# brown-ivl/manus

Hardware: AMD Instinct MI355X
Metric: train iters/sec (fwd+bwd) 300k Gaussians @1080p, 8 views; PSNR parity (higher is better)
Workload: dtype f32

## Files before the change

### include/manus_hip.h

```cpp
#ifndef MANUS_HIP_H
#define MANUS_HIP_H

#include <stddef.h>
#include <stdint.h>

#ifdef __cplusplus
extern "C" {
#endif

#define MGR_VERSION 100
#define MGR_CAM_FLOATS 40
#define MGR_TILE 16
#define MGR_MAX_BONES 32

enum {
    MGR_OK = 0,
    MGR_EINVAL = -1,
    MGR_ENOMEM = -2,
    MGR_EHIP = -3,
    MGR_EOVERFLOW = -4,
    MGR_ECUT = -6,
    MGR_ETIER = -7,
    MGR_ESTATE = -8
};

#define MGR_FWD_CHECK 1
#define MGR_FWD_NO_BLEND 2
#define MGR_FWD_BLEND_ONLY 4
#define MGR_FWD_DEPTH_CUT 8
#define MGR_FWD_SKIP_BOX_LARGE 16
#define MGR_FWD_SKIP_BOX_MID 32
#define MGR_FWD_SKIP_SORT_BEHIND 128
#define MGR_FWD_RANK_LARGE 256
#define MGR_FWD_IMAGE_KEPT 1024
#define MGR_FWD_REPAIR 2048
#define MGR_FWD_SPREAD 4096

#define MGR_BWD_CHECK 1
#define MGR_BWD_OUTPUTS_KEPT 512

#define MGR_OVF_PAIRS 1u
#define MGR_OVF_CUT 2u
#define MGR_OVF_TIER 4u
#define MGR_OVF_FLAGS_MASK 0xFFFF
#define MGR_OVF_REPAIRED_SHIFT 16

#define MGR_TIERS_BOX_LARGE 1
#define MGR_TIERS_BOX_MID 2
#define MGR_TIERS_WIDE_RECT 4
#define MGR_TIERS_NEAR_SMALL_SHIFT 8
#define MGR_TIERS_NEAR_LARGE_SHIFT 16
#define MGR_TIERS_NEAR_MASK 0xFF
#define MGR_TIERS_BEYOND_SMALL_SHIFT 24
#define MGR_TIERS_BEYOND_SMALL_MASK 0x7F

int mgr_version(void);
int mgr_build_variant(void);
int mgr_raster_repair_max_tiles(void);
const char* mgr_last_error(void);


size_t mgr_raster_workspace_bytes(int V, int N, int W, int H, int64_t pair_capacity);

int mgr_raster_forward(int V, int N, int W, int H, const float* cams, const float* bg,
                       const float* means3D, int64_t stride_means3D, const float* cov3D,
                       int64_t stride_cov3D, const float* colors, int64_t stride_colors,
                       const float* opacity, int64_t stride_opacity, float* out_color,
                       int32_t* radii, void* workspace, size_t workspace_bytes,
                       int64_t pair_capacity, int flags, void* stream);

int mgr_raster_backward(int V, int N, int W, int H, const float* cams, const float* bg,
                        const float* means3D, int64_t stride_means3D, const float* cov3D,
                        int64_t stride_cov3D, const float* colors, int64_t stride_colors,
                        const float* opacity, int64_t stride_opacity, const float* out_color,
                        const float* dL_dcolor, float* dL_dmeans3D, float* dL_dmeans2D, float* dL_dcolors,
                        float* dL_dopacity, float* dL_dcov3D, void* workspace,
                        size_t workspace_bytes, int64_t pair_capacity, int flags, void* stream);

int mgr_raster_blend_features(int V, int N, int C, int W, int H, const float* features, int64_t stride_features,
                              const float* bg_feat, int with_depth, float* out_feat, float* out_alpha,
                              const void* workspace, size_t workspace_bytes, int64_t pair_capacity, void* stream);

size_t mgr_raster_feat_backward_workspace_bytes(int V, int N, int C, int W, int H, int64_t pair_capacity);
int mgr_raster_blend_features_backward(int V, int N, int C, int W, int H, const float* cams, const float* means3D,
                                       int64_t stride_means3D, const float* cov3D, int64_t stride_cov3D, const float* features,
                                       int64_t stride_features, const float* bg_feat, int with_depth, const float* out_feat,
                                       const float* out_alpha, const float* dL_dout_feat, const float* dL_dalpha,
                                       float* dL_dmeans3D, float* dL_dmeans2D, float* dL_dopacity, float* dL_dcov3D,
                                       float* dL_dfeatures, const void* workspace, size_t workspace_bytes, int64_t pair_capacity,
                                       void* scratch, size_t scratch_bytes, int flags, void* stream);

int mgr_raster_forward_seq_sync(const void* workspace, uint32_t* seq, void* stream);

int mgr_views_forward(int V, int N, int B, int n_articulated, int sh_half, int W, int H, const float* cams, const float* bg,
                      const float* xyz, const float* log_scale, const float* rot,
                      const float* opacity_logit, const float* f_dc, const float* f_rest,
                      const float* skin_w, const float* transforms, float* out_color, int32_t* radii,
                      void* workspace, size_t workspace_bytes, int64_t pair_capacity, int flags,
                      void* stream);
int mgr_views_backward(int V, int N, int B, int n_articulated, int sh_half, int W, int H, const float* cams, const float* bg,
                       const float* xyz, const float* log_scale, const float* rot,
                       const float* opacity_logit, const float* f_dc, const float* f_rest,
                       const float* skin_w, const float* transforms, const int32_t* radii,
                       const float* out_color, const float* dL_dcolor, float grad2d_scale, float* d_xyz,
                       float* d_log_scale, float* d_rot, float* d_opacity_logit, float* d_f_dc,
                       float* d_f_rest, float* d_skin_w, float* stat_grad2d, float* stat_vis,
                       int32_t* stat_radii, void* workspace, size_t workspace_bytes,
                       int64_t pair_capacity, int flags, void* stream);



size_t mgr_views_pose_workspace_bytes(int V, int N, int B);
int mgr_views_backward_pose(int V, int N, int B, int n_articulated, int sh_half, int W, int H, const float* cams, const float* bg,
                            const float* xyz, const float* log_scale, const float* rot,
                            const float* opacity_logit, const float* f_dc, const float* f_rest,
                            const float* skin_w, const float* transforms, const int32_t* radii,
                            const float* out_color, const float* dL_dcolor, float grad2d_scale, float* d_xyz,
                            float* d_log_scale, float* d_rot, float* d_opacity_logit, float* d_f_dc,
                            float* d_f_rest, float* d_skin_w, float* stat_grad2d, float* stat_vis,
                            int32_t* stat_radii, void* workspace, size_t workspace_bytes,
                            int64_t pair_capacity, int flags, float* d_transforms, void* pose_workspace,
                            size_t pose_workspace_bytes, void* stream);

size_t mgr_views_maps_backward_workspace_bytes(int V, int N, int W, int H, int64_t pair_capacity);
int mgr_views_maps_backward(int V, int N, int B, int n_articulated, int W, int H, const float* cams, const float* xyz,
                            const float* log_scale, const float* rot, const float* opacity_logit, const float* skin_w,
                            const float* transforms, const float* out_alpha, const float* out_depth, const float* dL_dalpha,
                            const float* dL_ddepth, int accumulate, float* d_xyz, float* d_log_scale, float* d_rot,
                            float* d_opacity_logit, float* d_skin_w, const void* workspace, size_t workspace_bytes,
                            int64_t pair_capacity, void* scratch, size_t scratch_bytes, int flags, void* stream);

size_t mgr_views_maps_pose_workspace_bytes(int V, int N, int B);
int mgr_views_maps_backward_pose(int V, int N, int B, int n_articulated, int W, int H, const float* cams, const float* xyz,
                                 const float* log_scale, const float* rot, const float* opacity_logit, const float* skin_w,
                                 const float* transforms, const float* out_alpha, const float* out_depth, const float* dL_dalpha,
                                 const float* dL_ddepth, int accumulate, float* d_xyz, float* d_log_scale, float* d_rot,
                                 float* d_opacity_logit, float* d_skin_w, const void* workspace, size_t workspace_bytes,
                                 int64_t pair_capacity, void* scratch, size_t scratch_bytes, int flags, int accumulate_pose,
                                 float* d_transforms, void* pose_workspace, size_t pose_workspace_bytes, void* stream);

int mgr_views_active_list(void* workspace, int V, int N, int W, int H, int64_t pair_capacity, const uint32_t** list,
                          const uint32_t** count);

int mgr_views_backward_run_lists(int on);

int mgr_sh_to_half(int N, const float* f_rest, void* out_half, void* stream);

int mgr_raster_layout(int V, int N, int W, int H, int64_t pair_capacity, size_t* out, int n_out);
int mgr_raster_record_bytes(void);

int mgr_raster_set_cut_margin(float frac_entries, int min_entries, float depth_range_frac, float depth_rel, int interior_only);
int mgr_raster_set_cut_penalty(int forwards);
int mgr_raster_set_status_mirror(const void* workspace, void* host_words);
int mgr_raster_status_tiers_sync(const void* workspace, int64_t* num_pairs, int32_t* overflow, int32_t* tiers,
                                 void* stream);
int mgr_raster_status_sync(const void* workspace, int64_t* num_pairs, int32_t* overflow,
                           void* stream);

int mgr_raster_debug_binning_sync(const void* workspace, int V, int N, int W, int H,
                                  int64_t pair_capacity, int view, int32_t* tile_ranges_host,
                                  int32_t* point_list_host, int64_t max_pairs, void* stream);

int mgr_debug_pair_alpha(int n, const float* rec, const int32_t* px, const int32_t* py, float* alpha, int32_t* valid,
                         void* stream);


int mgr_skin_weights_fwd(int N, const float* xyz, const float* grid, int D, int H, int W, int B,
                         int grid_stride, const float* center3, const float* scale3, float* out_w,
                         void* stream);
int mgr_skin_weights_bwd(int N, const float* xyz, const float* grid, int D, int H, int W, int B,
                         int grid_stride, const float* center3, const float* scale3,
                         const float* dL_dw, float* dL_dxyz, int accumulate, void* stream);
int mgr_skin_weights_bwd_indexed(int N, const float* xyz, const float* grid, int D, int H, int W, int B,
                                 int grid_stride, const float* center3, const float* scale3, const float* dL_dw,
                                 float* dL_dxyz, const uint32_t* index, const uint32_t* index_count, int max_count,
                                 void* stream);

size_t mgr_skin_grid_bwd_workspace_bytes(int D, int H, int W, int max_count);
int mgr_skin_grid_bwd(int N, const float* xyz, const float* grid, int D, int H, int W, int B, int grid_stride,
                      const float* center3, const float* scale3, const float* dL_dw,
                      const uint32_t* index, const uint32_t* index_count, int max_count,
                      int32_t* out_voxel, float* out_grad, uint32_t* out_count, int capacity,
                      void* workspace, size_t workspace_bytes, void* stream);
int mgr_skin_grid_adam(const int32_t* voxel, const float* grad, const uint32_t* count, int capacity,
                       float* grid, int grid_stride, int B, float* exp_avg, float* exp_avg_sq,
                       double lr, double beta1, double beta2, double eps, int step, int clamp, float clamp_min,
                       void* stream);
int mgr_skin_rows_mask(int n, int B, const float* dL_dw, uint8_t* mask, void* stream);

int mgr_lbs_cov_fwd(int P, int N, int B, const float* xyz, const float* log_scale,
                    const float* rot, const float* skin_w, const float* transforms,
                    float* posed_xyz, float* posed_cov, float* tf, void* stream);
int mgr_lbs_cov_bwd(int P, int N, int B, const float* xyz, const float* log_scale,
                    const float* rot, const float* skin_w, const float* transforms,
                    const float* dL_dposed_xyz, const float* dL_dposed_cov, const float* dL_dtf,
                    float* dL_dxyz, float* dL_dlog_scale, float* dL_drot, float* dL_dw,
                    void* stream);

int mgr_sh_color_fwd(int V, int N, const float* sh, const float* xyz, int64_t stride_xyz,
                     const float* tf, int64_t stride_tf, const float* cams, float* colors,
                     void* stream);
int mgr_sh_color_bwd(int V, int N, const float* sh, const float* xyz, int64_t stride_xyz,
                     const float* tf, int64_t stride_tf, const float* cams,
                     const float* dL_dcolors, float* dL_dsh, float* dL_dxyz, float* dL_dtf,
                     void* stream);

int mgr_lbs_cov_fwd_rows(int P, int N, int B, const float* xyz, const float* log_scale,
                         const float* rot, const float* skin_w, const float* transforms,
                         float* posed_xyz, float* posed_cov, float* tf, int tf_row_floats, void* stream);
int mgr_lbs_cov_bwd_rows(int P, int N, int B, const float* xyz, const float* log_scale,
                         const float* rot, const float* skin_w, const float* transforms,
                         const float* dL_dposed_xyz, const float* dL_dposed_cov, const float* dL_dtf, int tf_row_floats,
                         float* dL_dxyz, float* dL_dlog_scale, float* dL_drot, float* dL_dw, void* stream);
size_t mgr_lbs_pose_workspace_bytes(int P, int N, int B);
int mgr_lbs_pose_bwd(int P, int N, int B, const float* xyz, const float* log_scale, const float* rot,
                     const float* skin_w, const float* transforms, const float* dL_dposed_xyz,
                     const float* dL_dposed_cov, const float* dL_dtf, int tf_row_floats, float* dL_dtransforms,
                     void* workspace, size_t workspace_bytes, void* stream);
int mgr_sh_color_fwd_rows(int V, int N, const float* sh, const float* xyz, int64_t stride_xyz,
                          const float* tf, int64_t stride_tf, int tf_row_floats, const float* cams, float* colors,
                          void* stream);
int mgr_sh_color_bwd_rows(int V, int N, const float* sh, const float* xyz, int64_t stride_xyz,
                          const float* tf, int64_t stride_tf, int tf_row_floats, const float* cams,
                          const float* dL_dcolors, float* dL_dsh, float* dL_dxyz, float* dL_dtf,
                          void* stream);

int mgr_pack_camera(float tanfovx, float tanfovy, const float* view16, const float* proj16, const float* campos3,
                    float* out40, void* stream);
int mgr_bone_transforms(int B, int background, const float* posed, const float* rest, float* out, void* stream);

int mgr_project_points(int N, const float* xyz, const float* K9, const float* E12, float* uv,
// ... 135 lines not shown
```

### manus_amd/_lib.py

```python
import ctypes
import os

import weakref

import torch

_HERE = os.path.dirname(os.path.abspath(__file__))
_VARIANT = os.environ.get("MANUS_HIP_VARIANT", "")
LIB_PATH = os.path.join(_HERE, "libmanus_hip%s.so" % ("_" + _VARIANT if _VARIANT else ""))
_LIB = None

MGR_CAM_FLOATS = 40
MGR_MAX_BONES = 32
MGR_FRAMES_MAX_VIEWS = 16

MGR_OK, MGR_EINVAL, MGR_ENOMEM, MGR_EHIP, MGR_EOVERFLOW, MGR_ECUT, MGR_ETIER, MGR_ESTATE = 0, -1, -2, -3, -4, -6, -7, -8
MGR_FWD_CHECK, MGR_FWD_NO_BLEND, MGR_FWD_BLEND_ONLY, MGR_FWD_DEPTH_CUT = 1, 2, 4, 8
MGR_FWD_SKIP_BOX_LARGE, MGR_FWD_SKIP_BOX_MID, MGR_FWD_SKIP_SORT_BEHIND, MGR_FWD_RANK_LARGE = 16, 32, 128, 256
MGR_FWD_IMAGE_KEPT, MGR_FWD_REPAIR, MGR_FWD_SPREAD = 1024, 2048, 4096
MGR_BWD_CHECK, MGR_BWD_OUTPUTS_KEPT = 1, 512
MGR_OVF_PAIRS, MGR_OVF_CUT, MGR_OVF_TIER, MGR_OVF_FLAGS_MASK, MGR_OVF_REPAIRED_SHIFT = 1, 2, 4, 0xFFFF, 16
MGR_TIERS_BOX_LARGE, MGR_TIERS_BOX_MID, MGR_TIERS_WIDE_RECT = 1, 2, 4
MGR_TIERS_NEAR_SMALL_SHIFT, MGR_TIERS_NEAR_LARGE_SHIFT, MGR_TIERS_NEAR_MASK = 8, 16, 0xFF
MGR_TIERS_BEYOND_SMALL_SHIFT, MGR_TIERS_BEYOND_SMALL_MASK = 24, 0x7F

c_int, c_i64, c_f32, c_vp, c_sz = ctypes.c_int, ctypes.c_int64, ctypes.c_float, ctypes.c_void_p, ctypes.c_size_t


class MgrFrameView(ctypes.Structure):
    _fields_ = [("offset", ctypes.c_int64), ("x0", ctypes.c_int32), ("y0", ctypes.c_int32), ("x1", ctypes.c_int32), ("y1", ctypes.c_int32),
                ("rx0", ctypes.c_int32), ("ry0", ctypes.c_int32), ("rx1", ctypes.c_int32), ("ry1", ctypes.c_int32),
                ("bg", ctypes.c_float * 3), ("slot", ctypes.c_int32)]


SIGNATURES = {
    "mgr_version": (c_int, []),
    "mgr_build_variant": (c_int, []),
    "mgr_raster_repair_max_tiles": (c_int, []),
    "mgr_last_error": (ctypes.c_char_p, []),
    "mgr_raster_workspace_bytes": (c_sz, [c_int, c_int, c_int, c_int, c_i64]),
    "mgr_raster_forward": (c_int, [c_int, c_int, c_int, c_int, c_vp, c_vp, c_vp, c_i64, c_vp, c_i64, c_vp,
                                   c_i64, c_vp, c_i64, c_vp, c_vp, c_vp, c_sz, c_i64, c_int, c_vp]),
    "mgr_raster_backward": (c_int, [c_int, c_int, c_int, c_int, c_vp, c_vp, c_vp, c_i64, c_vp, c_i64, c_vp,
                                    c_i64, c_vp, c_i64, c_vp, c_vp, c_vp, c_vp, c_vp, c_vp, c_vp, c_vp, c_sz,
                                    c_i64, c_int, c_vp]),
    "mgr_raster_blend_features": (c_int, [c_int, c_int, c_int, c_int, c_int, c_vp, c_i64, c_vp, c_int, c_vp, c_vp, c_vp, c_sz,
                                          c_i64, c_vp]),
    "mgr_raster_feat_backward_workspace_bytes": (c_sz, [c_int, c_int, c_int, c_int, c_int, c_i64]),
    "mgr_raster_blend_features_backward": (c_int, [c_int] * 5 + [c_vp, c_vp, c_i64, c_vp, c_i64, c_vp, c_i64, c_vp, c_int] + [c_vp] * 9
                                           + [c_vp, c_sz, c_i64, c_vp, c_sz, c_int, c_vp]),
    "mgr_raster_forward_seq_sync": (c_int, [c_vp, ctypes.POINTER(ctypes.c_uint32), c_vp]),
    "mgr_sh_to_half": (c_int, [c_int, c_vp, c_vp, c_vp]),
    "mgr_views_forward": (c_int, [c_int] * 7 + [c_vp] * 12 + [c_vp, c_sz, c_i64, c_int, c_vp]),
    "mgr_views_backward": (c_int, [c_int] * 7 + [c_vp] * 13 + [c_f32] + [c_vp] * 10 + [c_vp, c_sz, c_i64, c_int, c_vp]),
    "mgr_views_pose_workspace_bytes": (c_sz, [c_int, c_int, c_int]),
    "mgr_views_backward_pose": (c_int, [c_int] * 7 + [c_vp] * 13 + [c_f32] + [c_vp] * 10 + [c_vp, c_sz, c_i64, c_int, c_vp, c_vp, c_sz,
                                        c_vp]),
    "mgr_views_maps_backward_workspace_bytes": (c_sz, [c_int, c_int, c_int, c_int, c_i64]),
    "mgr_views_maps_backward": (c_int, [c_int] * 6 + [c_vp] * 11 + [c_int] + [c_vp] * 5 + [c_vp, c_sz, c_i64, c_vp, c_sz, c_int, c_vp]),
    "mgr_views_maps_pose_workspace_bytes": (c_sz, [c_int, c_int, c_int]),
    "mgr_views_maps_backward_pose": (c_int, [c_int] * 6 + [c_vp] * 11 + [c_int] + [c_vp] * 5 + [c_vp, c_sz, c_i64, c_vp, c_sz, c_int] +
                                     [c_int, c_vp, c_vp, c_sz, c_vp]),
    "mgr_raster_record_bytes": (c_int, []),
    "mgr_raster_layout": (c_int, [c_int, c_int, c_int, c_int, c_i64, ctypes.POINTER(c_sz), c_int]),
    "mgr_raster_status_sync": (c_int, [c_vp, ctypes.POINTER(c_i64), ctypes.POINTER(ctypes.c_int32), c_vp]),
    "mgr_raster_set_status_mirror": (c_int, [c_vp, c_vp]),
    "mgr_raster_set_cut_margin": (c_int, [c_f32, c_int, c_f32, c_f32, c_int]),
    "mgr_raster_set_cut_penalty": (c_int, [c_int]),
    "mgr_raster_status_tiers_sync": (c_int, [c_vp, ctypes.POINTER(c_i64), ctypes.POINTER(ctypes.c_int32),
                                             ctypes.POINTER(ctypes.c_int32), c_vp]),
    "mgr_debug_pair_alpha": (c_int, [c_int, c_vp, c_vp, c_vp, c_vp, c_vp, c_vp]),
    "mgr_raster_debug_binning_sync": (c_int, [c_vp, c_int, c_int, c_int, c_int, c_i64, c_int, c_vp, c_vp,
                                              c_i64, c_vp]),
    "mgr_skin_weights_fwd": (c_int, [c_int, c_vp, c_vp, c_int, c_int, c_int, c_int, c_int, c_vp, c_vp, c_vp,
                                     c_vp]),
    "mgr_skin_weights_bwd": (c_int, [c_int, c_vp, c_vp, c_int, c_int, c_int, c_int, c_int, c_vp, c_vp, c_vp,
                                     c_vp, c_int, c_vp]),
    "mgr_skin_weights_bwd_indexed": (c_int, [c_int, c_vp, c_vp, c_int, c_int, c_int, c_int, c_int, c_vp, c_vp, c_vp,
                                             c_vp, c_vp, c_vp, c_int, c_vp]),
    "mgr_skin_grid_bwd_workspace_bytes": (c_sz, [c_int, c_int, c_int, c_int]),
    "mgr_skin_grid_bwd": (c_int, [c_int, c_vp, c_vp, c_int, c_int, c_int, c_int, c_int, c_vp, c_vp, c_vp, c_vp, c_vp, c_int,
                                  c_vp, c_vp, c_vp, c_int, c_vp, c_sz, c_vp]),
    "mgr_skin_grid_adam": (c_int, [c_vp, c_vp, c_vp, c_int, c_vp, c_int, c_int, c_vp, c_vp, ctypes.c_double, ctypes.c_double, ctypes.c_double,
                                   ctypes.c_double, c_int, c_int, c_f32, c_vp]),
    "mgr_skin_rows_mask": (c_int, [c_int, c_int, c_vp, c_vp, c_vp]),
    "mgr_views_backward_run_lists": (c_int, [c_int]),
    "mgr_views_active_list": (c_int, [c_vp, c_int, c_int, c_int, c_int, c_i64, ctypes.POINTER(c_vp), ctypes.POINTER(c_vp)]),
    "mgr_lbs_cov_fwd": (c_int, [c_int, c_int, c_int, c_vp, c_vp, c_vp, c_vp, c_vp, c_vp, c_vp, c_vp, c_vp]),
    "mgr_lbs_cov_bwd": (c_int, [c_int, c_int, c_int, c_vp, c_vp, c_vp, c_vp, c_vp, c_vp, c_vp, c_vp, c_vp,
                                c_vp, c_vp, c_vp, c_vp]),
    "mgr_lbs_cov_fwd_rows": (c_int, [c_int, c_int, c_int, c_vp, c_vp, c_vp, c_vp, c_vp, c_vp, c_vp, c_vp, c_int, c_vp]),
    "mgr_lbs_cov_bwd_rows": (c_int, [c_int, c_int, c_int, c_vp, c_vp, c_vp, c_vp, c_vp, c_vp, c_vp, c_vp, c_int, c_vp,
                                     c_vp, c_vp, c_vp, c_vp]),
    "mgr_lbs_pose_workspace_bytes": (c_sz, [c_int, c_int, c_int]),
    "mgr_lbs_pose_bwd": (c_int, [c_int, c_int, c_int, c_vp, c_vp, c_vp, c_vp, c_vp, c_vp, c_vp, c_vp, c_int, c_vp, c_vp, c_sz, c_vp]),
    "mgr_sh_color_fwd_rows": (c_int, [c_int, c_int, c_vp, c_vp, c_i64, c_vp, c_i64, c_int, c_vp, c_vp, c_vp]),
    "mgr_sh_color_bwd_rows": (c_int, [c_int, c_int, c_vp, c_vp, c_i64, c_vp, c_i64, c_int, c_vp, c_vp, c_vp, c_vp, c_vp,
                                      c_vp]),
    "mgr_sh_color_fwd": (c_int, [c_int, c_int, c_vp, c_vp, c_i64, c_vp, c_i64, c_vp, c_vp, c_vp]),
    "mgr_sh_color_bwd": (c_int, [c_int, c_int, c_vp, c_vp, c_i64, c_vp, c_i64, c_vp, c_vp, c_vp, c_vp, c_vp,
                                 c_vp]),
    "mgr_pack_camera": (c_int, [c_f32, c_f32, c_vp, c_vp, c_vp, c_vp, c_vp]),
    "mgr_bone_transforms": (c_int, [c_int, c_int, c_vp, c_vp, c_vp, c_vp]),
    "mgr_project_points": (c_int, [c_int, c_vp, c_vp, c_vp, c_vp, c_vp]),
    "mgr_dilate_mask": (c_int, [c_int, c_int, c_int, c_vp, c_vp, c_vp, c_vp]),
    "mgr_points_outside_mask": (c_int, [c_int, c_vp, c_vp, c_vp, c_int, c_int, c_vp, c_int, c_vp, c_vp, c_vp]),
    "mgr_keypoint_far_mask": (c_int, [c_int, c_vp, c_int, c_vp, c_f32, c_vp, c_vp]),
    "mgr_knn3_workspace_bytes": (c_sz, [c_int]),
    "mgr_knn3_mean_dist2": (c_int, [c_int, c_vp, c_vp, c_vp, c_sz, c_vp]),
    "mgr_exchange_mask": (c_int, [c_int, c_vp, c_int, ctypes.POINTER(c_i64), ctypes.POINTER(c_int), c_i64, c_vp, c_vp, c_vp, c_vp]),
    "mgr_exchange_index_workspace_bytes": (c_sz, [c_int]),
    "mgr_exchange_index": (c_int, [c_int, c_vp, c_vp, c_vp, c_vp, c_sz, c_vp]),
    "mgr_exchange_pack": (c_int, [c_int, c_int, c_vp, c_vp, c_int, ctypes.POINTER(c_i64), ctypes.POINTER(c_int), c_i64, c_vp, c_vp]),
    "mgr_exchange_unpack": (c_int, [c_int, c_int, c_vp, c_vp, c_int, ctypes.POINTER(c_i64), ctypes.POINTER(c_int), c_i64, c_vp, c_vp,
                                    c_i64, c_vp]),
    "mgr_exchange_pack_rows": (c_int, [c_int, c_int, c_vp, c_vp, c_vp, c_int, ctypes.POINTER(c_i64), ctypes.POINTER(c_int), c_i64, c_vp, c_vp]),
    "mgr_exchange_unpack_rows": (c_int, [c_int, c_int, c_vp, c_vp, c_vp, c_int, ctypes.POINTER(c_i64), ctypes.POINTER(c_int), c_i64, c_vp, c_vp,
                                         c_i64, c_vp]),
    "mgr_l1_loss_grad": (c_int, [c_i64, c_vp, c_vp, c_f32, c_vp, c_vp, c_vp]),
    "mgr_image_loss_workspace_bytes": (c_sz, [c_int, c_int, c_int]),
    "mgr_image_loss": (c_int, [c_int, c_int, c_int, c_vp, c_vp, c_f32, c_f32, c_f32, c_f32, c_vp, c_vp, c_vp, c_sz, c_vp]),
    "mgr_image_loss_tiles": (c_int, [c_int, c_int, c_int, c_vp, c_vp, c_vp, c_vp, c_f32, c_f32, c_f32, c_f32, c_vp, c_vp, c_vp, c_sz,
                                     c_vp]),
    "mgr_image_loss_target_map_words": (c_sz, [c_int, c_int, c_int]),
    "mgr_image_loss_target_map": (c_int, [c_int, c_int, c_int, c_vp, c_vp, c_vp, c_vp]),
    "mgr_image_loss_tiles_list_mapped": (c_int, [c_int, c_int, c_int, c_vp, c_vp, c_vp, c_vp, c_sz, c_int, c_vp]),
    "mgr_views_forward_attach_loss_list": (c_int, [c_vp, c_int, c_int, c_int, c_vp, c_vp, c_sz]),
    "mgr_image_loss_tiles_list": (c_int, [c_int, c_int, c_int, c_vp, c_vp, c_vp, c_vp, c_sz, c_vp]),
    "mgr_image_loss_tiles_finish": (c_int, [c_int, c_int, c_int, c_vp, c_vp, c_f32, c_f32, c_f32, c_f32, c_vp, c_vp, c_vp, c_sz,
                                            c_vp]),
    "mgr_map_loss_workspace_bytes": (c_sz, [c_int, c_int, c_int]),
    "mgr_map_loss": (c_int, [c_int, c_int, c_int, c_vp, c_vp, c_vp, c_vp, c_f32, c_f32, c_f32, c_vp, c_vp, c_vp, c_vp, c_sz, c_vp]),
    "mgr_frames_decode": (c_int, [c_int, c_int, c_int, c_int, c_vp, c_i64, ctypes.POINTER(MgrFrameView), c_vp, c_vp, c_i64, c_vp]),
    "mgr_eval_workspace_bytes": (c_sz, [c_int, c_int, c_int]),
    "mgr_eval_views": (c_int, [c_int, c_int, c_int, c_vp, c_vp, c_vp, c_vp, c_vp, c_vp, c_vp, c_vp, c_sz, c_vp]),
    "mgr_eval_triptych": (c_int, [c_int, c_int, c_int, c_vp, c_vp, c_vp, c_vp, c_vp, c_vp]),
    "mgr_ceval_workspace_bytes": (c_sz, [c_int, c_int, c_int]),
    "mgr_ceval_masks": (c_int, [c_int, c_int, c_int, c_vp, c_int, c_vp, c_vp, c_vp, c_vp, c_vp, c_vp, c_vp]),
    "mgr_ceval_labels": (c_int, [c_int, c_int, c_int, c_vp, c_int, c_vp, c_vp, c_vp, c_sz, c_vp]),
    "mgr_ceval_fill": (c_int, [c_int, c_int, c_int, c_vp, c_vp, c_vp, c_sz, c_vp]),
    "mgr_ceval_counts": (c_int, [c_int, c_int, c_int, c_vp, c_vp, c_vp, c_vp, c_vp, c_sz, c_vp]),
    "mgr_ceval_collage": (c_int, [c_int, c_int, c_int, c_int, c_vp, c_vp, c_vp, c_vp, c_vp]),
    "mgr_adam_step": (c_int, [c_int, c_vp, c_vp, c_vp, c_vp, c_vp, c_vp, c_i64, ctypes.c_double, ctypes.c_double,
                               ctypes.c_double, c_vp]),
    "mgr_reset_opacity": (c_int, [c_int, c_vp, c_vp, c_vp, c_vp]),
    "mgr_add_densification_stats": (c_int, [c_int, c_vp, c_vp, c_vp, c_vp, c_vp, c_vp, c_vp]),
# ... 145 lines not shown
```

### manus_amd/csrc/instance_math.h

```cpp
#pragma once
#include <hip/hip_fp16.h>

#include "mgr_common.h"

#ifdef __HIPCC__

struct GaussCano {
    float x, y, z;
    float q[4], nrm, R[9], s[3];
};

__device__ __forceinline__ void quat_rot(const float q[4], float R[9]) {
#pragma clang fp contract(off)
    const float r = q[0], x = q[1], y = q[2], z = q[3];
    R[0] = 1.f - 2.f * (y * y + z * z); R[1] = 2.f * (x * y - r * z); R[2] = 2.f * (x * z + r * y);
    R[3] = 2.f * (x * y + r * z); R[4] = 1.f - 2.f * (x * x + z * z); R[5] = 2.f * (y * z - r * x);
    R[6] = 2.f * (x * z - r * y); R[7] = 2.f * (y * z + r * x); R[8] = 1.f - 2.f * (x * x + y * y);
}

typedef float mgr_f4u __attribute__((ext_vector_type(4), aligned(4)));
typedef float mgr_f3u __attribute__((ext_vector_type(3), aligned(4)));

__device__ __forceinline__ void cano_load(const float* __restrict__ xyz, const float* __restrict__ log_scale,
                                          const float* __restrict__ rot, int i, GaussCano& g) {
// ... 297 lines not shown
    const float b = M0[0] * S1[0] + M0[1] * S1[1] + M0[2] * S1[2];
    const float c = M1[0] * S1[0] + M1[1] * S1[1] + M1[2] * S1[2] + 0.3f;
    const float dA = acc[2], dB = acc[3], dC = acc[4];
    const float den = a * c - b * b;
    const float k2 = 1.0f / (den * den + 0.0000001f);
    float da = 0.f, db = 0.f, dc = 0.f;
#pragma unroll
    for (int j = 0; j < 6; ++j) dc6[j] = 0.f;
    if (k2 != 0.0f) {
        da = k2 * (-c * c * dA + 2.0f * b * c * dB + (den - a * c) * dC);
        dc = k2 * (-a * a * dC + 2.0f * a * b * dB + (den - a * c) * dA);
        db = k2 * 2.0f * (b * c * dA - (den + 2.0f * b * b) * dB + a * b * dC);
        dc6[0] = M0[0] * M0[0] * da + M0[0] * M1[0] * db + M1[0] * M1[0] * dc;
        dc6[3] = M0[1] * M0[1] * da + M0[1] * M1[1] * db + M1[1] * M1[1] * dc;
        dc6[5] = M0[2] * M0[2] * da + M0[2] * M1[2] * db + M1[2] * M1[2] * dc;
        dc6[1] = 2.0f * M0[0] * M0[1] * da + (M0[0] * M1[1] + M0[1] * M1[0]) * db + 2.0f * M1[0] * M1[1] * dc;
        dc6[2] = 2.0f * M0[0] * M0[2] * da + (M0[0] * M1[2] + M0[2] * M1[0]) * db + 2.0f * M1[0] * M1[2] * dc;
        dc6[4] = 2.0f * M0[2] * M0[1] * da + (M0[1] * M1[2] + M0[2] * M1[1]) * db + 2.0f * M1[1] * M1[2] * dc;
    }
    float dM0[3], dM1[3];
#pragma unroll
    for (int j = 0; j < 3; ++j) {
        dM0[j] = 2.0f * S0[j] * da + S1[j] * db;
        dM1[j] = 2.0f * S1[j] * dc + S0[j] * db;
    }
    const float dJ00 = vm[0] * dM0[0] + vm[4] * dM0[1] + vm[8] * dM0[2];
    const float dJ02 = vm[2] * dM0[0] + vm[6] * dM0[1] + vm[10] * dM0[2];
    const float dJ11 = vm[1] * dM1[0] + vm[5] * dM1[1] + vm[9] * dM1[2];
    const float dJ12 = vm[2] * dM1[0] + vm[6] * dM1[1] + vm[10] * dM1[2];
    const float tz = 1.0f / t[2], tz2 = tz * tz, tz3 = tz2 * tz;
    const float dtx = xm * -fx * tz2 * dJ02;
    const float dty = ym * -fy * tz2 * dJ12;
    const float dtz = -fx * tz2 * dJ00 - fy * tz2 * dJ11 + (2.0f * fx * t[0]) * tz3 * dJ02 +
                      (2.0f * fy * t[1]) * tz3 * dJ12;
    dm[0] = vm[0] * dtx + vm[1] * dty + vm[2] * dtz;
    dm[1] = vm[4] * dtx + vm[5] * dty + vm[6] * dtz;
    dm[2] = vm[8] * dtx + vm[9] * dty + vm[10] * dtz;
    const float* pm = cam.proj;
    const float hw = pm[3] * p[0] + pm[7] * p[1] + pm[11] * p[2] + pm[15];
    const float mw = 1.0f / (hw + 0.0000001f);
    const float mul1 = (pm[0] * p[0] + pm[4] * p[1] + pm[8] * p[2] + pm[12]) * mw * mw;
    const float mul2 = (pm[1] * p[0] + pm[5] * p[1] + pm[9] * p[2] + pm[13]) * mw * mw;
    const float gx2 = acc[0], gy2 = acc[1];
    dm[0] += (pm[0] * mw - pm[3] * mul1) * gx2 + (pm[1] * mw - pm[3] * mul2) * gy2;
    dm[1] += (pm[4] * mw - pm[7] * mul1) * gx2 + (pm[5] * mw - pm[7] * mul2) * gy2;
    dm[2] += (pm[8] * mw - pm[11] * mul1) * gx2 + (pm[9] * mw - pm[11] * mul2) * gy2;
}

typedef uint32_t mgr_u4u __attribute__((ext_vector_type(4), aligned(4)));

__device__ __forceinline__ void gather_pair_grads(uint32_t off, uint32_t cnt, const uint32_t* __restrict__ pair_tag,
                                                  const float4* __restrict__ pair_grad, uint32_t cap, uint32_t epoch,
                                                  float acc[9]) {
#pragma unroll
    for (int k = 0; k < 9; ++k) acc[k] = 0.f;
    if (off >= cap) return;
    cnt = min(cnt, cap - off);
    for (uint32_t base = 0; base < cnt; base += 64) {
        const uint32_t n = min(64u, cnt - base);
        unsigned long long hit = 0ull;
        for (uint32_t k = 0; k < n; k += 16) {
            const mgr_u4u* tp = (const mgr_u4u*)(pair_tag + off + base + k);
            const mgr_u4u t0 = tp[0], t1 = tp[1], t2 = tp[2], t3 = tp[3];
            const uint32_t tg[16] = {t0.x, t0.y, t0.z, t0.w, t1.x, t1.y, t1.z, t1.w,
                                     t2.x, t2.y, t2.z, t2.w, t3.x, t3.y, t3.z, t3.w};
            uint32_t m16 = 0;
#pragma unroll
            for (int j = 0; j < 16; ++j) m16 |= (tg[j] == epoch ? 1u : 0u) << j;
            hit |= (unsigned long long)m16 << k;
        }
        if (n < 64) hit &= (1ull << n) - 1ull;
        while (hit) {
            const int j = __builtin_ctzll(hit);
            hit &= hit - 1;
            const float4* r = pair_grad + (size_t)(off + base + (uint32_t)j) * 3;
            const float4 a = r[0], b = r[1], c = r[2];
            acc[0] += a.x; acc[1] += a.y; acc[2] += a.z; acc[3] += a.w;
            acc[4] += b.x; acc[5] += b.y; acc[6] += b.z; acc[7] += b.w;
            acc[8] += c.x;
        }
    }
}

#define MGR_POSE_REC 13
#define MGR_POSE_MAX_WG 1024

__device__ __forceinline__ int pose_segments(int NT, int nvb) {
    int s = 1;
    while (s < 8 && 2 * s * nvb <= NT) s *= 2;
    return s;
}

template <int NT>
__device__ __forceinline__ void pose_wg_lists(int tid, int NV, int pv, unsigned char* s_lst, int* s_cnt, int* s_wc) {
    static_assert(NT <= 256 && NT % 64 == 0, "lane ids are kept in a byte");
    constexpr int NW = NT / 64;
    const int lane = tid & 63, wv = tid >> 6;
    int rank = 0;
    for (int v = 0; v < NV; ++v) {
        const unsigned long long m = __ballot(pv == v);
        if (pv == v) rank = __popcll(m & ((1ull << lane) - 1ull));
        if (lane == 0) s_wc[v * NW + wv] = __popcll(m);
    }
    __syncthreads();
    if (pv >= 0) {
        int base = 0;
        for (int w = 0; w < wv; ++w) base += s_wc[pv * NW + w];
        s_lst[pv * NT + base + rank] = (unsigned char)tid;
    }
    if (tid < NV) {
        int c = 0;
        for (int w = 0; w < NW; ++w) c += s_wc[tid * NW + w];
        s_cnt[tid] = c;
    }
    __syncthreads();
}

template <int NT>
__device__ __forceinline__ void pose_wg_accumulate(int tid, int NV, int B, const float* s_rec, const unsigned char* s_lst,
                                                   const int* s_cnt, const float* __restrict__ skin_w, float pacc[12]) {
    const int nvb = NV * B, S = pose_segments(NT, nvb);
    const int seg = tid / nvb, o = tid - seg * nvb;
    if (seg >= S) return;
    const int v = o / B, b = o - v * B;
    const int cnt = s_cnt[v], per = (cnt + S - 1) / S;
    const int j1 = min(cnt, (seg + 1) * per);
    const unsigned char* lst = s_lst + v * NT;
#pragma unroll 4
    for (int j = seg * per; j < j1; ++j) {
        const float* r = s_rec + (int)lst[j] * MGR_POSE_REC;
        const float w = skin_w[(size_t)__float_as_int(r[12]) * B + b];
#pragma unroll
        for (int k = 0; k < 12; ++k) pacc[k] = __builtin_fmaf(w, r[k], pacc[k]);
    }
}

template <int NT>
__device__ __forceinline__ void pose_wg_store(int tid, int NV, int B, float* s_scratch, const float pacc[12],
                                              float* __restrict__ slot) {
    const int nvb = NV * B, S = pose_segments(NT, nvb);
    const int seg = tid / nvb, o = tid - seg * nvb;
    if (S > 1) {
        __syncthreads();
        if (seg > 0 && seg < S) {
#pragma unroll
            for (int k = 0; k < 12; ++k) s_scratch[(seg * nvb + o) * 12 + k] = pacc[k];
        }
        __syncthreads();
    }
    if (seg != 0) return;
    float a[12];
#pragma unroll
    for (int k = 0; k < 12; ++k) a[k] = pacc[k];
    for (int s = 1; s < S; ++s) {
#pragma unroll
        for (int k = 0; k < 12; ++k) a[k] += s_scratch[(s * nvb + o) * 12 + k];
    }
#pragma unroll
    for (int k = 0; k < 12; ++k) slot[o * 12 + k] = a[k];
}

#endif

int mgr_pose_fold(int v_first, int v_count, int NV, int B, const float* part, int n_slots, float* d_transforms,
                  hipStream_t stream);
int mgr_pose_fold_acc(int v_first, int v_count, int NV, int B, const float* part, int n_slots, int accumulate, float* d_transforms,
// ... 2 lines not shown
```

### manus_amd/csrc/mgr_common.h

```cpp
#pragma once
#include <hip/hip_runtime.h>
#include <stdint.h>
#include <stdio.h>
#include <string.h>

#include "../../include/manus_hip.h"

#define MGR_WAVE 64

extern thread_local char g_mgr_err[512];

static inline int mgr_fail(int code, const char* fmt, const char* a = "", const char* b = "") {
    snprintf(g_mgr_err, sizeof(g_mgr_err), fmt, a, b);
    return code;
}

#define MGR_HIP(call)                                                                      \
    do {                                                                                   \
        hipError_t e_ = (call);                                                            \
        if (e_ != hipSuccess) return mgr_fail(MGR_EHIP, "%s: %s", #call, hipGetErrorString(e_)); \
    } while (0)

#define MGR_LAUNCH_CHECK(name, stream, debug)                                              \
    do {                                                                                   \
// ... 30 lines not shown
#define MGR_REP_CAND 8192
#define MGR_REP_TARGET 3072
#define MGR_REP_VIEW_TILES 256
#define MGR_REP_MAX_TILES 65536
struct __attribute__((aligned(16))) MgrRepUnit {
    uint32_t vt, quad, nlist, start;
    uint32_t ck0, done_lo, done_hi, ntail;
    uint32_t ov_start, ov_ck0, p0, ck_first;
    uint32_t beyond;
    uint32_t pad[3];
};
struct __attribute__((aligned(16))) MgrRepTile {
    uint32_t tile, unit, zc, zw;
};
struct MgrRepView {
    uint32_t n, x0, y0, x1, y1, pad[3];
    MgrRepTile t[MGR_REP_VIEW_TILES];
};
struct MgrRep {
    MgrRepUnit* unit;
    float4* state;
    uint32_t* last;
    uint32_t* cnt;
    uint32_t* tile_rep;
    unsigned long long* cand;
    MgrRepView* view;
    uint32_t max_units, list_cap, ck_cap, list_base, ck_base;
};
struct MgrHeader {
    uint32_t total_pairs;
    uint32_t overflow;
    uint32_t epoch;
    uint32_t queue_len;
    uint32_t queue_head;
    uint32_t queue_head2;
    uint32_t n_items;
    uint32_t item_head;
    uint32_t queue_small;
    uint32_t queue_head3;
    uint32_t n_active;
    uint32_t queue_len_i;
    uint32_t acc_pairs, acc_flags;
    uint32_t tiers;
    uint32_t sort_big;
    uint32_t n_runs[4];
    uint32_t bwd_seq, rows_seq, rows_pending;
    uint32_t rows_owner[2];
    uint32_t fwd_seq, img_seq, img_owner[2], img_bg[3];
    uint32_t n_rep_units, rep_list_used, rep_ck_used;
    uint32_t rep_why;
    MgrRep rep;
    uint32_t sort_huge;
    uint32_t sort_large;
    uint32_t sort_near_large;
    uint32_t feat_seq, feat_dims[5], feat_flags;
    uint32_t spare[45 - 7 - sizeof(MgrRep) / 4];
    uint32_t queue_giant;
    uint32_t n_groups;
    uint32_t split_head, group_head;
    uint32_t pad2[56 - 8 - 68 + 64 - 4];
    uint32_t qctr[16 * 64];
    uint32_t qctr_f[16 * 64];
};
#define MGR_NCTR 16
#define MGR_HOLE 0xFFFFFFFEu
#define MGR_FEAT_CUT 1u
struct MgrFeatStamp {
    uint32_t dims[5], flags;
};
#define MGR_SKIP_BOX_LARGE 1
#define MGR_SKIP_BOX_MID 2
#define MGR_SKIP_SORT_BEHIND 4
#define MGR_SKIP_RANK_LARGE 8

#ifndef MGR_GREC_BYTES
#define MGR_GREC_BYTES 64
#endif
struct __attribute__((aligned(MGR_GREC_BYTES == 64 ? 64 : 16))) MgrGRec {
    float x, y, ca, cb;
    float cc, op, r, g;
    float b;
    int32_t slot_base;
    int32_t rect_w;
    int32_t pad;
#if MGR_GREC_BYTES == 64
    int32_t pad64[4];
#endif
};

#define MGR_CHUNK 64

static inline uint32_t mgr_rep_units(int64_t cap) { int64_t u = cap / 16384; return (uint32_t)(u < 64 ? 64 : (u > 1024 ? 1024 : u)); }
static inline uint32_t mgr_rep_list(int64_t cap) { int64_t n = cap / 8; return (uint32_t)(n < (1 << 16) ? (1 << 16) : (n > (2 << 20) ? (2 << 20) : n)); }
static inline uint32_t mgr_rep_ck(int64_t cap) { return mgr_rep_list(cap) / MGR_CHUNK + mgr_rep_units(cap); }

struct MgrLayout {
    size_t header, scan_part, scan_cls, scan_box, grec, depth, rect, alive, pair_off, tile_count, tile_start, tile_cursor, tile_done, tile_qdone,
        tile_zcut, tile_zused, tile_qend, tile_bgok, tile_queue, tile_qrec, chunk_start, items, ckpt, keys, keys2, groups, sorted_gid, final_T, n_contrib, pair_tag, pair_grad, inst_grad, inst_tag,
        db_count, db_cursor, db_start, db_nvis, db_bbox, db_keys, db_order, db_rec, bin_mat, tile_rep, rep_unit, rep_state, rep_last, rep_cnt, rep_cand, rep_view, tile_zwin, db_zrange, db_item, total;
};

#ifndef MGR_DB_BUCKETS
#define MGR_DB_BUCKETS 1024
#endif
#ifndef MGR_DB_ITEM
#define MGR_DB_ITEM 768
#endif
#define MGR_DB_RANK_MAX 2048
#define MGR_DB_RANK_LARGE 3072
#ifndef MGR_BIN_BLOCK
#define MGR_BIN_BLOCK 1024
#endif
static inline int mgr_bin_block(int V, int N) { return (long long)V * (long long)N >= 500000ll ? MGR_BIN_BLOCK : 256; }

static inline size_t mgr_align(size_t x) { return (x + 255) & ~(size_t)255; }

static inline MgrLayout mgr_layout(int V, int N, int W, int H, int64_t cap) {
    MgrLayout L;
    size_t VN = (size_t)V * (size_t)(N > 0 ? N : 1);
    size_t gx = (W + MGR_TILE - 1) / MGR_TILE, gy = (H + MGR_TILE - 1) / MGR_TILE;
    size_t VT = (size_t)V * gx * gy, VP = (size_t)V * W * H;
    size_t c = (size_t)(cap > 0 ? cap : 1);
    size_t o = 0;
    L.header = o;      o += mgr_align(sizeof(MgrHeader));
    const size_t scan_blocks = (size_t)V * ((gx * gy + 1023) / 1024);
    L.scan_part = o;   o += mgr_align((scan_blocks + 1) * 8);
    L.scan_cls = o;    o += mgr_align(scan_blocks * 34 * 4);
    L.scan_box = o;    o += mgr_align(scan_blocks * 16);
    L.grec = o;        o += mgr_align(VN * sizeof(MgrGRec));
    L.depth = o;       o += mgr_align(VN * 4);
    L.rect = o;        o += mgr_align(VN * 8);
    L.alive = o;       o += mgr_align(VN * 8);
    L.pair_off = o;    o += mgr_align(VN * 4);
    L.tile_count = o;  o += mgr_align(VT * 4);
    L.tile_start = o;  o += mgr_align((VT + 1) * 4);
    L.tile_cursor = o; o += mgr_align(VT * 4);
    L.tile_done = o;   o += mgr_align(VT * 4);
    L.tile_qdone = o;  o += mgr_align(VT * 16);
    L.tile_zcut = o;   o += mgr_align(VT * 4);
    L.tile_zused = o;  o += mgr_align(VT * 4);
    L.tile_qend = o;   o += mgr_align(VT * 4);
    L.tile_queue = o;  o += mgr_align(VT * 4);
    L.tile_qrec = o;   o += mgr_align(VT * 16);
    L.chunk_start = o; o += mgr_align((VT + 1) * 4);
    const size_t rep_u = mgr_rep_units(cap), rep_l = mgr_rep_list(cap), rep_c = mgr_rep_ck(cap);
    L.items = o;       o += mgr_align((c / MGR_CHUNK + VT + 1 + rep_c) * 32);
    L.ckpt = o;        o += mgr_align((c / MGR_CHUNK + 1 + rep_c) * 256 * 16);
    L.keys = o;        o += mgr_align(c * 8);
    L.keys2 = o;       o += mgr_align(c * 8);
    L.groups = o;      o += mgr_align((c / 4096 + 64) * 16);
    L.sorted_gid = o;  o += mgr_align((c + rep_l) * 4);
    L.final_T = o;     o += mgr_align(VP * 4);
    L.n_contrib = o;   o += mgr_align(VP * 4);
    L.pair_tag = o;    o += mgr_align(c * 4 + 64);
    L.pair_grad = o;   o += mgr_align(c * 48);
    L.inst_tag = o;    o += mgr_align(VN * 4);
    L.inst_grad = o;   o += mgr_align(VN * 128);
    {
        const size_t VB = (size_t)V * MGR_DB_BUCKETS, bb = (size_t)mgr_bin_block(V, N), nblk = ((size_t)(N > 0 ? N : 1) + bb - 1) / bb;
        L.db_count = o;  o += mgr_align(VB * 4);
        L.db_cursor = o; o += mgr_align(VB * 4);
        L.db_start = o;  o += mgr_align((VB + 1) * 4);
        L.db_nvis = o;   o += mgr_align((size_t)V * 4);
        L.db_bbox = o;   o += mgr_align((size_t)V * 8);
        L.db_keys = o;   o += mgr_align(VN * 8);
        L.db_order = o;  o += mgr_align(VN * 4);
        L.db_rec = o;    o += mgr_align(VN * 16);
        L.bin_mat = o;   o += mgr_align((size_t)V * nblk * gx * gy * 4);
    }
    L.tile_bgok = o; o += mgr_align((size_t)V * gx * gy);
    L.tile_rep = o;  o += mgr_align(VT * 4);
    L.rep_unit = o;  o += mgr_align(rep_u * sizeof(MgrRepUnit));
    L.rep_state = o; o += mgr_align(rep_u * 64 * 16);
    L.rep_last = o;  o += mgr_align(rep_u * 64 * 4);
    L.rep_cnt = o;   o += mgr_align(rep_u * 4);
    L.rep_cand = o;  o += mgr_align(rep_u * (size_t)MGR_REP_CAND * 8);
    L.rep_view = o;  o += mgr_align((size_t)V * sizeof(MgrRepView));
    L.tile_zwin = o; o += mgr_align(VT * 4);
    L.db_zrange = o; o += mgr_align((size_t)V * (((size_t)(N > 0 ? N : 1) + 511) / 512) * 2 * 4);
    L.db_item = o;   o += mgr_align((size_t)V * (((size_t)(N > 0 ? N : 1) + MGR_DB_ITEM - 1) / MGR_DB_ITEM + 1) * 2 * 4);
    L.total = o;
    return L;
}

#ifdef __HIPCC__

struct MgrCam {
    float tanfovx, tanfovy;
    float view[16], proj[16];
    float campos[3];
};

__device__ __forceinline__ void mgr_load_cam(const float* __restrict__ cams, int v, MgrCam& c) {
    const float* p = cams + (size_t)v * MGR_CAM_FLOATS;
    c.tanfovx = p[0];
    c.tanfovy = p[1];
#pragma unroll
    for (int i = 0; i < 16; ++i) {
        c.view[i] = p[2 + i];
        c.proj[i] = p[18 + i];
    }
    c.campos[0] = p[34];
    c.campos[1] = p[35];
    c.campos[2] = p[36];
}

template <int CTRL, int ROW_MASK = 0xf, int BANK_MASK = 0xf>
__device__ __forceinline__ float mgr_dpp(float v) {
    return __builtin_bit_cast(
        float, __builtin_amdgcn_update_dpp(0, __builtin_bit_cast(int, v), CTRL, ROW_MASK, BANK_MASK, false));
}

template <int CTRL, int ROW_MASK = 0xf>
__device__ __forceinline__ uint32_t mgr_dpp_u(uint32_t v) {
    return (uint32_t)__builtin_amdgcn_update_dpp(0, (int)v, CTRL, ROW_MASK, 0xf, false);
}
__device__ __forceinline__ uint32_t mgr_wave_incl_scan_u32(uint32_t v) {
    v += mgr_dpp_u<0x111>(v);
    v += mgr_dpp_u<0x112>(v);
    v += mgr_dpp_u<0x114>(v);
    v += mgr_dpp_u<0x118>(v);
    v += mgr_dpp_u<0x142, 0xa>(v);
    v += mgr_dpp_u<0x143, 0xc>(v);
    return v;
}

__device__ __forceinline__ uint32_t mgr_wave_max_u32(uint32_t v) {
    v = max(v, mgr_dpp_u<0xb1>(v));
    v = max(v, mgr_dpp_u<0x4e>(v));
    v = max(v, mgr_dpp_u<0x141>(v));
    v = max(v, mgr_dpp_u<0x140>(v));
    const uint32_t a = (uint32_t)__builtin_amdgcn_readlane((int)v, 0), b = (uint32_t)__builtin_amdgcn_readlane((int)v, 16),
                   c = (uint32_t)__builtin_amdgcn_readlane((int)v, 32), d = (uint32_t)__builtin_amdgcn_readlane((int)v, 48);
    return max(max(a, b), max(c, d));
}

__device__ __forceinline__ float mgr_wave_sum63(float v) {
    v += mgr_dpp<0xb1>(v);
    v += mgr_dpp<0x4e>(v);
    v += mgr_dpp<0x114>(v);
    v += mgr_dpp<0x118>(v);
    v += mgr_dpp<0x142, 0xa>(v);
    v += mgr_dpp<0x143, 0xc>(v);
    return v;
}

#define MGR_DPP9(ctrl)                                                                              \
    asm volatile("s_nop 1\n"                                                                        \
                 "v_add_f32_dpp %0, %0, %0 " ctrl "\n v_add_f32_dpp %1, %1, %1 " ctrl "\n"          \
                 "v_add_f32_dpp %2, %2, %2 " ctrl "\n v_add_f32_dpp %3, %3, %3 " ctrl "\n"          \
                 "v_add_f32_dpp %4, %4, %4 " ctrl "\n v_add_f32_dpp %5, %5, %5 " ctrl "\n"          \
                 "v_add_f32_dpp %6, %6, %6 " ctrl "\n v_add_f32_dpp %7, %7, %7 " ctrl "\n"          \
                 "v_add_f32_dpp %8, %8, %8 " ctrl "\n"                                              \
                 : "+v"(a0), "+v"(a1), "+v"(a2), "+v"(a3), "+v"(a4), "+v"(a5), "+v"(a6), "+v"(a7), "+v"(a8))

__device__ __forceinline__ void mgr_wave_sum63_x9(float& a0, float& a1, float& a2, float& a3, float& a4,
                                                  float& a5, float& a6, float& a7, float& a8) {
    MGR_DPP9("quad_perm:[1,0,3,2] row_mask:0xf bank_mask:0xf");
    MGR_DPP9("quad_perm:[2,3,0,1] row_mask:0xf bank_mask:0xf");
    MGR_DPP9("row_shr:4 row_mask:0xf bank_mask:0xf");
    MGR_DPP9("row_shr:8 row_mask:0xf bank_mask:0xf");
    MGR_DPP9("row_bcast:15 row_mask:0xa bank_mask:0xf");
    MGR_DPP9("row_bcast:31 row_mask:0xc bank_mask:0xf");
// ... 241 lines not shown
```

### manus_amd/csrc/raster_bwd.hip

```cpp
#include <atomic>

#include "instance_math.h"

#ifdef MGR_STATS
__device__ unsigned long long g_stats[16];
extern "C" int mgr_debug_stats(unsigned long long* dst) {
    return (int)hipMemcpyFromSymbol(dst, HIP_SYMBOL(g_stats), sizeof(unsigned long long) * 16);
}
__device__ unsigned long long g_bhist[3][65];
extern "C" int mgr_debug_bhist(unsigned long long* dst) {
    return (int)hipMemcpyFromSymbol(dst, HIP_SYMBOL(g_bhist), sizeof(unsigned long long) * 3 * 65);
}
#define BH(r, c, v) do { const int c_ = (c); const unsigned long long v_ = (unsigned long long)(v); if (lane == 0) atomicAdd(&g_bhist[r][c_], v_); } while (0)
#define MGR_STAT(i, v) do { const unsigned long long v_ = (unsigned long long)(v); if (lane == 0) atomicAdd(&g_stats[i], v_); } while (0)
#else
#define MGR_STAT(i, v)
#endif

#ifdef BWD_PROF
__device__ unsigned long long g_bprof[8];
extern "C" int mgr_debug_bprof(unsigned long long* dst) {
    return (int)hipMemcpyFromSymbol(dst, HIP_SYMBOL(g_bprof), sizeof(unsigned long long) * 8);
}
#define BP(k) { const long long now_ = wall_clock64(); acc_[k] += now_ - tp_; tp_ = now_; }
#else
#define BP(k)
#endif

__device__ __forceinline__ uint32_t mgr_any64(unsigned long long m) {
    uint32_t r;
    asm("s_cmp_lg_u64 %1, 0\n\ts_cselect_b32 %0, 1, 0" : "=s"(r) : "s"(m) : "scc");
    return r;
}

#define BWD_BATCH MGR_CHUNK
#ifndef BWD_KO
#define BWD_KO 0
#endif
int mgr_bwd_variant_bits(void) {
    int bits = 0;
    if (BWD_KO != 0) bits |= 1;
#if defined(MGR_STATS) || defined(BWD_PROF)
    bits |= 2;
#endif
#ifdef BWD_WLAST_REDUCE
    bits |= 4;
#endif
#if defined(MGR_GATHER_PRELOAD)
    if (MGR_GATHER_PRELOAD != 1) bits |= 4;
#endif
    return bits;
}
#define MGR_LDS_VOLATILE_F32 volatile const __attribute__((address_space(3))) float*
#define BWD_ROW 288
#define BWD_PLANE_W 64
#define BWD_PLANE_B 128
#ifndef BWD_WAVES
#define BWD_WAVES 4
#endif

__global__ __launch_bounds__(256) __attribute__((amdgpu_waves_per_eu(BWD_WAVES, BWD_WAVES))) void k_blend_bwd(
    int N, int W, int H, int gx, int gy, const uint32_t* __restrict__ sorted_gid, const MgrGRec* __restrict__ grec,
    const uint32_t* __restrict__ n_contrib, const float4* __restrict__ ckpt, const uint4* __restrict__ items,
    MgrHeader* hdr, const float* __restrict__ out_color, const float* __restrict__ dL_dpix,
    uint32_t* __restrict__ pair_tag, float4* __restrict__ pair_grad, uint32_t* __restrict__ inst_tag, uint32_t cap,
    uint32_t epoch) {
    __shared__ __align__(16) float s_pair[4][32][MGR_PAIR_FLOATS];
    __shared__ __align__(16) float s_xch[4][4 * BWD_ROW];
    __shared__ float s_acc[4][BWD_BATCH][9];
    __shared__ uint32_t s_flag[4][BWD_BATCH];

    const int tid = threadIdx.x, wave = tid >> 6, lane = tid & 63;
    const int T = gx * gy;
    const uint32_t n_items = hdr->n_items;
    if (blockIdx.x == 0 && tid < 4) (tid == 3 ? hdr->n_active : hdr->n_runs[tid]) = 0;
    if (blockIdx.x == 0 && tid == 4) hdr->bwd_seq += 1u;
    const size_t P = (size_t)W * H;
    const unsigned long long lt = (1ull << lane) - 1ull;
    float* const slab = &s_pair[wave][0][0];
    float* const xch = &s_xch[wave][0];
    float* const acc = &s_acc[wave][0][0];
    uint32_t* const flag = &s_flag[wave][0];
    const int e2 = lane >> 3, pc = lane & 7;
#ifdef BWD_PROF
    long long acc_[6] = {0, 0, 0, 0, 0, 0}, tp_ = wall_clock64(), nit_ = 0;
#endif

    MgrQueue queue;
    queue.init(hdr->qctr, n_items, (int)blockIdx.x);
    uint32_t item = queue.resolve(queue.issue(lane), lane);
    while (item != 0xFFFFFFFFu) {
        const uint32_t next_raw = queue.issue(lane);
        const uint4 recA = items[2 * (size_t)item], recB = items[2 * (size_t)item + 1];
        const uint32_t vt = recA.x, chunk = recA.y;
        const uint32_t mxq[4] = {recB.x, recB.y, recB.z, recB.w};
        const int v = (int)(vt / (uint32_t)T), t = (int)(vt % (uint32_t)T);
        const int bx = t % gx, by = t / gx;
        const uint32_t first = chunk * BWD_BATCH;
        const uint32_t tmax = max(max(mxq[0], mxq[1]), max(mxq[2], mxq[3]));
        const int cnt = (int)min((uint32_t)BWD_BATCH, tmax - first);
        const MgrGRec* const gv = grec + (size_t)v * N;
#ifdef BWD_PROF
        ++nit_;
#endif
        BP(0);
#if BWD_KO & 1024
        const uint32_t gid = sorted_gid[recA.z] + 0u * (uint32_t)lane;
#else
        const uint32_t gid = sorted_gid[recA.z + (uint32_t)min(lane, cnt - 1)];
#endif
        float4 ra, rb, rcz;
        {
            const MgrGRec* r = gv + gid;
            ra = *(const float4*)r;
            rb = *((const float4*)r + 1);
            rcz = *((const float4*)r + 2);
        }
#pragma unroll
        for (int k = 0; k < 9; ++k) acc[k * 64 + lane] = 0.f;
        flag[lane] = 0u;
        const int32_t slot = __float_as_int(rcz.y) + by * __float_as_int(rcz.z) + bx;
        const float qmax_e = mgr_qmax(rb.y);
        BP(1);

        uint32_t qmask = (mxq[0] > first ? 1u : 0u) | (mxq[1] > first ? 2u : 0u) | (mxq[2] > first ? 4u : 0u) | (mxq[3] > first ? 8u : 0u);
        struct PxState {
            uint32_t nc;
            float t0, t1, t2, o0, o1, o2;
            float4 ck;
        };
        auto load_px = [&](int quad, PxState& q) {
            const int px = bx * 16 + (quad & 1) * 8 + (lane & 7);
            const int py = by * 16 + (quad >> 1) * 8 + (lane >> 3);
            const size_t pixc = (size_t)min(py, H - 1) * W + min(px, W - 1);
#if BWD_KO & 512
            q.nc = tmax; q.t0 = 0.001f * (float)pixc; q.t1 = 0.5f; q.t2 = 0.25f; q.o0 = 0.3f; q.o1 = 0.2f; q.o2 = 0.1f;
            q.ck = make_float4(0.1f, 0.1f, 0.1f, 0.5f);
#else
            q.nc = n_contrib[(size_t)v * P + pixc];
            const float* gp = dL_dpix + (size_t)v * 3 * P + pixc;
            const float* op = out_color + (size_t)v * 3 * P + pixc;
            q.t0 = gp[0]; q.t1 = gp[P]; q.t2 = gp[2 * P];
            q.o0 = op[0]; q.o1 = op[P]; q.o2 = op[2 * P];
            q.ck = ckpt[(size_t)recA.w * 256 + ((quad << 6) | lane)];
#endif
        };
        PxState pxn;
        load_px(qmask ? __builtin_ctz(qmask) : 0, pxn);
#pragma unroll 1
// ... 156 lines not shown
                    const float xe = pbs[0 + h], ye = pbs[2 + h];
                    const uint32_t pos = __float_as_uint(*(MGR_LDS_VOLATILE_F32)(pbs + 18 + h));
                    const float dxc = xe - fx_col, dy0 = ye - qy0;
                    const float* src = xch + (e2 >> 1) * BWD_ROW + h * BWD_PLANE_B + 4 * pc;
#if !(BWD_KO & 128)
                    const bool on2 = (tmask >> e2) & 1u;
                    float* const accp = acc + (on2 ? (int)((pos - 1u - first) & 63u) : 0) * 9;
                    const float old_t = *(MGR_LDS_VOLATILE_F32)(accp + pc), old_9 = *(MGR_LDS_VOLATILE_F32)(accp + 8);
#endif
                    mgr_v2f DY = {dy0, dy0 - 1.0f};
                    mgr_v2f B0 = {0.f, 0.f}, B1 = {0.f, 0.f}, B2 = {0.f, 0.f}, Cr = {0.f, 0.f}, Cg = {0.f, 0.f}, Cb = {0.f, 0.f};
#pragma unroll
                    for (int j = 0; j < 2; ++j) {
                        const float4 v4 = *(const float4*)(src + 32 * j), w4 = *(const float4*)(src + BWD_PLANE_W + 32 * j);
#pragma unroll
                        for (int q = 0; q < 2; ++q) {
                            const int k = 2 * j + q;
                            const mgr_v2f vv = q ? mgr_v2f{v4.z, v4.w} : mgr_v2f{v4.x, v4.y};
                            const mgr_v2f ww = q ? mgr_v2f{w4.z, w4.w} : mgr_v2f{w4.x, w4.y};
                            const mgr_v2f t1 = vv * DY;
                            B0 += vv;
                            B1 += t1;
                            B2 += t1 * DY;
                            Cr += ww * gr0[k];
                            Cg += ww * gr1[k];
                            Cb += ww * gr2[k];
                            DY -= 2.0f;
                        }
                    }
                    const float A0 = B0.x + B0.y, A1 = B1.x + B1.y, A2 = B2.x + B2.y;
                    const float sr = Cr.x + Cr.y, sgn = Cg.x + Cg.y, sb = Cb.x + Cb.y;
                    const float Sx = dxc * A0;
                    const float x8[8] = {Sx, A1, Sx * dxc, dxc * A1, A2, A0, sr, sgn};
                    const float tot = grp8_reduce_scatter(x8, pc);
                    const float b9 = grp_sum<8>(sb);
                    if ((tmask >> e2) & 1u) {
                        const int ja = (int)(pos - 1u - first);
#if BWD_KO & 8
                        acc[ja * 9 + pc] = tot;
                        if (pc == 0) {
                            acc[ja * 9 + 8] = b9;
                            flag[ja] = 1u;
                        }
#elif BWD_KO & 128
                        __hip_atomic_fetch_add(acc + ja * 9 + pc, tot, __ATOMIC_RELAXED, __HIP_MEMORY_SCOPE_WAVEFRONT);
                        if (pc == 0) {
                            __hip_atomic_fetch_add(acc + ja * 9 + 8, b9, __ATOMIC_RELAXED, __HIP_MEMORY_SCOPE_WAVEFRONT);
                            flag[ja] = 1u;
                        }
#else
                        accp[pc] = old_t + tot;
                        if (pc == 0) {
                            accp[8] = old_9 + b9;
                            flag[ja] = 1u;
                        }
#endif
                    }
                }
                __builtin_amdgcn_wave_barrier();
            }
#ifdef MGR_STATS
            MGR_STAT(10, (max(max(nblk_[0], nblk_[1]), max(nblk_[2], nblk_[3])) + 1u) >> 1);
            MGR_STAT(11, (nblk_[0] + nblk_[1] + nblk_[2] + nblk_[3] + 7u) >> 3);
#endif
            BP(3);
        }
        __builtin_amdgcn_wave_barrier();
        if (lane < cnt && flag[lane] != 0u && slot >= 0 && (uint32_t)slot < cap) {
            float r[9];
#pragma unroll
            for (int c = 0; c < 9; ++c) r[c] = acc[lane * 9 + c];
#pragma unroll
            for (int c = 0; c < 5; ++c) r[c] *= rb.y;
            const float cA = ra.z, cB = ra.w, cC = rb.x;
            const float mx = (-0.5f * (float)W) * (cA * r[0] + cB * r[1]);
            const float my = (-0.5f * (float)H) * (cC * r[1] + cB * r[0]);
#if BWD_KO & 256
            if (mx + my + r[2] + r[3] + r[4] + r[5] + r[6] + r[7] + r[8] == 12345.678f) pair_tag[slot] = epoch;
#else
            float4* o = pair_grad + (size_t)slot * 3;
            o[0] = make_float4(mx, my, -0.5f * r[2], -0.5f * r[3]);
            o[1] = make_float4(-0.5f * r[4], r[5], r[6], r[7]);
            o[2] = make_float4(r[8], 0.f, 0.f, 0.f);
            pair_tag[slot] = epoch;
            inst_tag[(size_t)v * N + gid] = epoch;
#endif
        }
        __builtin_amdgcn_wave_barrier();
        BP(5);
        item = queue.resolve(next_raw, lane);
    }
#ifdef BWD_PROF
    if (lane == 0) {
        for (int k = 0; k < 6; ++k) atomicAdd(&g_bprof[k], (unsigned long long)acc_[k]);
        atomicAdd(&g_bprof[6], (unsigned long long)nit_);
        atomicAdd(&g_bprof[7], 1ull);
    }
#endif
}

__global__ __launch_bounds__(256) void k_preprocess_bwd(
    int N, int W, int H, const float* __restrict__ cams, const float* __restrict__ means3D,
    int64_t s_means, const float* __restrict__ cov3D, int64_t s_cov,
    const int32_t* __restrict__ radii_ws, const ushort4* __restrict__ rect,
    const uint32_t* __restrict__ pair_off, const uint32_t* __restrict__ pair_tag,
    const float4* __restrict__ pair_grad, float* __restrict__ dL_dmeans3D,
    float* __restrict__ dL_dmeans2D, float* __restrict__ dL_dcolors,
    float* __restrict__ dL_dopacity, float* __restrict__ dL_dcov3D, const uint32_t* __restrict__ inst_tag,
    uint32_t cap, uint32_t epoch, MgrHeader* hdr) {
    if (blockIdx.x == 0 && blockIdx.y == 0 && threadIdx.x < MGR_NCTR) hdr->qctr[threadIdx.x * 64] = 0u;
    const int v = blockIdx.y;
    const int i = blockIdx.x * 256 + threadIdx.x;
    if (i >= N) return;
    const size_t vi = (size_t)v * N + i;
    const ushort4 rc = rect[vi];
    const uint32_t cnt = (uint32_t)((rc.z - rc.x) * (rc.w - rc.y));
    float acc[9] = {0.f, 0.f, 0.f, 0.f, 0.f, 0.f, 0.f, 0.f, 0.f};
    float dm[3] = {0.f, 0.f, 0.f}, dc6[6] = {0.f, 0.f, 0.f, 0.f, 0.f, 0.f};
    if (cnt > 0 && inst_tag[vi] == epoch) {
        gather_pair_grads(pair_off[vi], cnt, pair_tag, pair_grad, cap, epoch, acc);
        MgrCam cam;
        mgr_load_cam(cams, v, cam);
        const float* mp = means3D + (size_t)v * s_means + (size_t)i * 3;
        const float p[3] = {mp[0], mp[1], mp[2]};
        const float* cp = cov3D + (size_t)v * s_cov + (size_t)i * 6;
        const float c6[6] = {cp[0], cp[1], cp[2], cp[3], cp[4], cp[5]};
        project_backward(cam, W, H, p, c6, acc, dm, dc6);
    }
    float* o3 = dL_dmeans3D + vi * 3;
    o3[0] = dm[0]; o3[1] = dm[1]; o3[2] = dm[2];
    float* o2 = dL_dmeans2D + vi * 3;
    o2[0] = acc[0]; o2[1] = acc[1]; o2[2] = 0.f;
    float* oc = dL_dcolors + vi * 3;
    oc[0] = acc[6]; oc[1] = acc[7]; oc[2] = acc[8];
    dL_dopacity[vi] = acc[5];
    float* ov = dL_dcov3D + vi * 6;
#pragma unroll
    for (int j = 0; j < 6; ++j) ov[j] = dc6[j];
}


typedef float mgr_f2u __attribute__((ext_vector_type(2), aligned(4)));
template <int G>
__device__ __forceinline__ void grp_store_span(const float t[8], int vl, bool ok, float* __restrict__ dst, int n, bool accumulate) {
    constexpr int PER = 8 / G;
    float mine[PER];
#pragma unroll
    for (int j = 0; j < PER; ++j) {
        mine[j] = t[j];
#pragma unroll
        for (int r = 1; r < G; ++r) mine[j] = vl == r ? t[r * PER + j] : mine[j];
    }
    const int e0 = vl * PER;
    if (!ok || e0 >= n) return;
    float* d = dst + e0;
    if (e0 + PER <= n) {
        if (PER == 2) {
            mgr_f2u v = {mine[0], mine[1]};
            if (accumulate) v += *(const mgr_f2u*)d;
            *(mgr_f2u*)d = v;
        } else if (PER == 4) {
            mgr_f4u v = {mine[0], mine[1], mine[2], mine[3]};
            if (accumulate) v += *(const mgr_f4u*)d;
            *(mgr_f4u*)d = v;
        } else {
#pragma unroll
            for (int h = 0; h < PER / 4; ++h) {
                mgr_f4u v = {mine[4 * h], mine[4 * h + 1], mine[4 * h + 2], mine[4 * h + 3]};
                if (accumulate) v += *(const mgr_f4u*)(d + 4 * h);
                *(mgr_f4u*)(d + 4 * h) = v;
            }
        }
    } else {
#pragma unroll
        for (int j = 0; j < PER; ++j)
            if (e0 + j < n) d[j] = accumulate ? d[j] + mine[j] : mine[j];
    }
}

template <int G>
__device__ __forceinline__ void grp_store8(const float x[8], int vl, bool ok, float* __restrict__ dst, int n,
                                           bool accumulate) {
    if (G == 8) {
        const float t = grp8_reduce_scatter(x, vl);
        if (ok && vl < n) dst[vl] = accumulate ? dst[vl] + t : t;
    } else {
        float t[8];
#pragma unroll
        for (int k = 0; k < 8; ++k) t[k] = grp_sum<G>(x[k]);
        grp_store_span<G>(t, vl, ok, dst, n, accumulate);
    }
}

#ifndef IB_THREADS
#define IB_THREADS 256
#endif
#ifndef MGR_IB_WAVES
#define MGR_IB_WAVES 2
#endif
#ifndef IG_ROUNDS
#define IG_ROUNDS 8
#endif
#define IB_TSTRIDE(B) ((B) * 16 + 4)

template <int G>
__global__ __launch_bounds__(256) void k_inst_gather(
    int v_first, int v_count, int N, int B, int n_art, const int32_t* __restrict__ radii, const ushort4* __restrict__ rect,
    const uint32_t* __restrict__ pair_off, const uint32_t* __restrict__ pair_tag,
    const float4* __restrict__ pair_grad, const uint32_t* __restrict__ inst_tag, uint32_t cap, uint32_t epoch,
    int accumulate, int rounds, float4* __restrict__ iacc,
    uint32_t* __restrict__ active_list, MgrHeader* hdr, float* __restrict__ d_xyz, float* __restrict__ d_ls,
    float* __restrict__ d_rot, float* __restrict__ d_op, float* __restrict__ d_fdc, float* __restrict__ d_frest,
    float* __restrict__ d_w, float* __restrict__ st_grad2d, float* __restrict__ st_vis,
    int32_t* __restrict__ st_radii, uint32_t* __restrict__ run_list) {
    constexpr int IPB = 256 / G;
    __shared__ uint32_t s_list[IPB * IG_ROUNDS];
    __shared__ uint32_t s_cnt, s_base;
    constexpr int RL = G == 8 ? IPB * IG_ROUNDS : 1;
    __shared__ uint32_t s_rl[3][RL];
    __shared__ uint32_t s_rc[3], s_rb[3];
    const bool runs = G == 8 && run_list != nullptr;
    const int tid = threadIdx.x, vl = tid & (G - 1), il = tid / G, lane = tid & 63;
    if (blockIdx.x == 0 && tid < MGR_NCTR && v_first == 0) hdr->qctr[tid * 64] = 0u;
    if (tid == 0) s_cnt = 0;
    if (tid < 3) s_rc[tid] = 0;
    __syncthreads();
    const bool acc_out = accumulate != 0;
#pragma unroll 1
    for (int rnd = 0; rnd < rounds; ++rnd) {
        const int i_raw = (blockIdx.x * rounds + rnd) * IPB + il;
        const int i = min(i_raw, N - 1);
        const bool ok = i_raw < N, mine = ok && vl < v_count;
        const int v = v_first + vl;
        float acc[9];
#pragma unroll
        for (int k = 0; k < 9; ++k) acc[k] = 0.f;
        int rad = 0;
        bool any = false;
        {
            const size_t vi = (size_t)min(v, v_first + v_count - 1) * N + i;
            const int rd = radii[vi];
            const uint32_t tg = inst_tag[vi];
            const ushort4 rc = rect[vi];
            const uint32_t po = pair_off[vi];
            rad = mine ? rd : 0;
            if (rad > 0 && tg == epoch) {
                gather_pair_grads(po, (uint32_t)((rc.z - rc.x) * (rc.w - rc.y)), pair_tag, pair_grad, cap, epoch, acc);
#pragma unroll
                for (int k = 0; k < 9; ++k) any = any || (acc[k] != 0.f);
            }
        }
        const bool grp_any = grp_sum<G>(any ? 1.0f : 0.0f) > 0.0f;
        const float vis = grp_sum<G>(rad > 0 ? 1.0f : 0.0f);
        int maxrad = rad;
        if (G >= 2) maxrad = max(maxrad, __builtin_amdgcn_update_dpp(0, maxrad, 0xb1, 0xf, 0xf, false));
        if (G >= 4) maxrad = max(maxrad, __builtin_amdgcn_update_dpp(0, maxrad, 0x4e, 0xf, 0xf, false));
        if (G >= 8) maxrad = max(maxrad, __builtin_amdgcn_update_dpp(0, maxrad, 0x141, 0xf, 0xf, false));
        if (runs) {
            const uint32_t m8 = (uint32_t)(__ballot(any) >> (lane & 56)) & 0xFFu;
            if (ok && vl == 0 && m8) {
                const int nv = __popc(m8), c = nv > 4 ? 0 : nv > 2 ? 1 : 2;
                s_rl[c][atomicAdd(&s_rc[c], 1u)] = (uint32_t)i | (m8 << 24);
            }
        }
        if (ok && (runs ? any : grp_any)) {
            float4* o = iacc + ((size_t)i * G + vl) * 3;
            o[0] = make_float4(acc[0], acc[1], acc[2], acc[3]);
            o[1] = make_float4(acc[4], acc[5], acc[6], acc[7]);
            o[2] = make_float4(acc[8], 0.f, 0.f, 0.f);
        }
        {
            const bool lead = ok && grp_any && vl == 0;
            const unsigned long long m = __ballot(lead);
            if (m) {
                const int first = __builtin_ctzll(m);
                uint32_t base = 0;
                if (lane == first) base = atomicAdd(&s_cnt, (uint32_t)__popcll(m));
                base = (uint32_t)__shfl((int)base, first, 64);
                if (lead) s_list[base + (uint32_t)__popcll(m & ((1ull << lane) - 1ull))] = (uint32_t)i;
            }
        }
        if (ok && vl == 0) {
            if (st_vis) st_vis[i] = acc_out ? st_vis[i] + vis : vis;
            if (st_radii) st_radii[i] = acc_out ? max(st_radii[i], maxrad) : maxrad;
        }
    }
    if (!acc_out) {
        const size_t i_lo = (size_t)blockIdx.x * rounds * IPB;
        const size_t i_hi = min((size_t)N, i_lo + (size_t)rounds * IPB);
        if (i_hi > i_lo) {
            const size_t n = i_hi - i_lo;
            for (size_t k = tid; k < n * 3; k += 256) { d_xyz[i_lo * 3 + k] = 0.f; d_ls[i_lo * 3 + k] = 0.f; d_fdc[i_lo * 3 + k] = 0.f; }
            for (size_t k = tid; k < n * 4; k += 256) d_rot[i_lo * 4 + k] = 0.f;
            for (size_t k = tid; k < n * 45; k += 256) d_frest[i_lo * 45 + k] = 0.f;
            if (d_w && i_lo < (size_t)n_art) {
                const size_t na = min(i_hi, (size_t)n_art) - i_lo;
                for (size_t k = tid; k < na * (size_t)B; k += 256) d_w[i_lo * B + k] = 0.f;
            }
            for (size_t k = tid; k < n; k += 256) {
                d_op[i_lo + k] = 0.f;
                if (st_grad2d) st_grad2d[i_lo + k] = 0.f;
            }
        }
    }
    __syncthreads();
    const uint32_t cnt = s_cnt;
    if (tid == 0 && cnt) s_base = atomicAdd(&hdr->n_active, cnt);
    __syncthreads();
    for (uint32_t k = tid; k < cnt; k += 256) active_list[s_base + k] = s_list[k];
    if (runs) {
        if (tid < 3) s_rb[tid] = s_rc[tid] ? atomicAdd(&hdr->n_runs[tid], s_rc[tid]) : 0u;
        __syncthreads();
#pragma unroll
        for (int c = 0; c < 3; ++c)
            for (uint32_t k = tid; k < s_rc[c]; k += 256) run_list[(size_t)c * N + s_rb[c] + k] = s_rl[c][k];
    }
}

template <int G>
__global__ __launch_bounds__(256) void k_inst_gather_runs(
    int v_first, int v_count, int N, int B, int n_art, const int32_t* __restrict__ radii, const ushort4* __restrict__ rect,
    const uint32_t* __restrict__ pair_off, const uint32_t* __restrict__ pair_tag,
    const float4* __restrict__ pair_grad, const uint32_t* __restrict__ inst_tag, uint32_t cap, uint32_t epoch,
    int accumulate, int rounds, float4* __restrict__ iacc,
    uint32_t* __restrict__ active_list, MgrHeader* hdr, float* __restrict__ d_xyz, float* __restrict__ d_ls,
    float* __restrict__ d_rot, float* __restrict__ d_op, float* __restrict__ d_fdc, float* __restrict__ d_frest,
    float* __restrict__ d_w, float* __restrict__ st_grad2d, float* __restrict__ st_vis,
    int32_t* __restrict__ st_radii, uint32_t* __restrict__ run_list, unsigned char* __restrict__ row_state, int kept) {
    constexpr int IPB = 256 / G, NG = 256;
    __shared__ uint32_t s_wi[NG * G], s_wo[NG * G], s_wc[NG * G];
    __shared__ uint32_t s_mask[NG];
    __shared__ uint32_t s_list[NG], s_rl[3][NG];
    __shared__ uint32_t s_nw, s_cnt, s_base, s_rc[3], s_rb[3];
    const int tid = threadIdx.x, vl = tid & (G - 1), il = tid / G, lane = tid & 63;
    if (blockIdx.x == 0 && tid < MGR_NCTR && v_first == 0) hdr->qctr[tid * 64] = 0u;
    if (tid == 0) { s_nw = 0; s_cnt = 0; }
    if (tid < 3) s_rc[tid] = 0;
    s_mask[tid] = 0u;
    __syncthreads();
    const bool acc_out = accumulate != 0;
    const int i_base = blockIdx.x * rounds * IPB;
    const unsigned long long owner = (unsigned long long)(uintptr_t)d_xyz;
    const bool kept_ok = kept && row_state && hdr->rows_seq != 0u && hdr->rows_seq + 1u == hdr->bwd_seq &&
                         hdr->rows_owner[0] == (uint32_t)owner && hdr->rows_owner[1] == (uint32_t)(owner >> 32);
    int rd_r[G];
    uint32_t tg_r[G], po_r[G];
    ushort4 rc_r[G];
#ifndef MGR_GATHER_PRELOAD
#define MGR_GATHER_PRELOAD 1
#endif
#if MGR_GATHER_PRELOAD
#pragma unroll
    for (int rnd = 0; rnd < G; ++rnd) {
        const int i = min(i_base + min(rnd, rounds - 1) * IPB + il, N - 1);
        const size_t vi = (size_t)min(v_first + vl, v_first + v_count - 1) * N + i;
        rd_r[rnd] = radii[vi];
        tg_r[rnd] = inst_tag[vi];
        rc_r[rnd] = rect[vi];
        po_r[rnd] = pair_off[vi];
    }
#pragma unroll
#else
#pragma unroll 1
#endif
    for (int rnd = 0; rnd < G; ++rnd) {
        if (rnd >= rounds) break;
        const int i_raw = i_base + rnd * IPB + il;
        const int i = min(i_raw, N - 1);
        const bool ok = i_raw < N, mine = ok && vl < v_count;
#if MGR_GATHER_PRELOAD
        const int rd = rd_r[rnd];
        const uint32_t tg = tg_r[rnd];
        const ushort4 rc = rc_r[rnd];
        const uint32_t po = po_r[rnd];
#else
        const size_t vi = (size_t)min(v_first + vl, v_first + v_count - 1) * N + i;
        const int rd = radii[vi];
        const uint32_t tg = inst_tag[vi];
        const ushort4 rc = rect[vi];
        const uint32_t po = pair_off[vi];
        (void)rd_r; (void)tg_r; (void)rc_r; (void)po_r;
#endif
        const int rad = mine ? rd : 0;
        const bool act = rad > 0 && tg == epoch;
        const float vis = grp_sum<G>(rad > 0 ? 1.0f : 0.0f);
        int maxrad = rad;
        if (G >= 2) maxrad = max(maxrad, __builtin_amdgcn_update_dpp(0, maxrad, 0xb1, 0xf, 0xf, false));
        if (G >= 4) maxrad = max(maxrad, __builtin_amdgcn_update_dpp(0, maxrad, 0x4e, 0xf, 0xf, false));
        if (G >= 8) maxrad = max(maxrad, __builtin_amdgcn_update_dpp(0, maxrad, 0x141, 0xf, 0xf, false));
        const unsigned long long m = __ballot(act);
        if (m) {
            const int first = __builtin_ctzll(m);
            uint32_t base = 0;
            if (lane == first) base = atomicAdd(&s_nw, (uint32_t)__popcll(m));
            base = (uint32_t)__shfl((int)base, first, 64);
            if (act) {
                const uint32_t pos = base + (uint32_t)__popcll(m & ((1ull << lane) - 1ull));
                s_wi[pos] = ((uint32_t)(rnd * IPB + il) << 3) | (uint32_t)vl;
                s_wo[pos] = po;
                s_wc[pos] = (uint32_t)((rc.z - rc.x) * (rc.w - rc.y));
            }
        }
        if (ok && vl == 0) {
            if (st_vis) st_vis[i] = acc_out ? st_vis[i] + vis : vis;
            if (st_radii) st_radii[i] = acc_out ? max(st_radii[i], maxrad) : maxrad;
        }
    }
    __syncthreads();
    const uint32_t n_work = s_nw;
    for (uint32_t k = (uint32_t)tid; k < n_work; k += 256u) {
        const uint32_t w = s_wi[k];
        float acc[9];
        gather_pair_grads(s_wo[k], s_wc[k], pair_tag, pair_grad, cap, epoch, acc);
        bool any = false;
#pragma unroll
        for (int q = 0; q < 9; ++q) any = any || (acc[q] != 0.f);
        {
            float4* o = iacc + ((size_t)(i_base + (int)(w >> 3)) * G + (w & 7u)) * 3;
            o[0] = make_float4(acc[0], acc[1], acc[2], acc[3]);
            o[1] = make_float4(acc[4], acc[5], acc[6], acc[7]);
            o[2] = make_float4(acc[8], 0.f, 0.f, 0.f);
        }
        if (any) atomicOr(&s_mask[w >> 3], 1u << (w & 7u));
    }
    if (!acc_out && !kept_ok) {
        const size_t i_lo = (size_t)i_base;
        const size_t i_hi = min((size_t)N, i_lo + (size_t)rounds * IPB);
        if (i_hi > i_lo) {
            const size_t n = i_hi - i_lo;
            for (size_t k = tid; k < n * 3; k += 256) { d_xyz[i_lo * 3 + k] = 0.f; d_ls[i_lo * 3 + k] = 0.f; d_fdc[i_lo * 3 + k] = 0.f; }
            for (size_t k = tid; k < n * 4; k += 256) d_rot[i_lo * 4 + k] = 0.f;
            for (size_t k = tid; k < n * 45; k += 256) d_frest[i_lo * 45 + k] = 0.f;
            if (d_w && i_lo < (size_t)n_art) {
                const size_t na = min(i_hi, (size_t)n_art) - i_lo;
                for (size_t k = tid; k < na * (size_t)B; k += 256) d_w[i_lo * B + k] = 0.f;
            }
            for (size_t k = tid; k < n; k += 256) {
                d_op[i_lo + k] = 0.f;
                if (st_grad2d) st_grad2d[i_lo + k] = 0.f;
            }
        }
    }
    __syncthreads();
    if (row_state && tid < rounds * IPB && i_base + tid < N) {
        const int i = i_base + tid;
        if (kept_ok && row_state[i] && s_mask[tid] == 0u) {
            for (int k = 0; k < 3; ++k) { d_xyz[3 * i + k] = 0.f; d_ls[3 * i + k] = 0.f; d_fdc[3 * i + k] = 0.f; }
            for (int k = 0; k < 4; ++k) d_rot[4 * i + k] = 0.f;
            for (int k = 0; k < 45; ++k) d_frest[(size_t)i * 45 + k] = 0.f;
            if (d_w && i < n_art)
                for (int k = 0; k < B; ++k) d_w[(size_t)i * B + k] = 0.f;
            d_op[i] = 0.f;
            if (st_grad2d) st_grad2d[i] = 0.f;
        }
        row_state[i] = s_mask[tid] != 0u ? 1 : 0;
    }
    if (blockIdx.x == 0 && tid == 0) hdr->rows_pending = row_state ? hdr->bwd_seq : 0u;
    {
        const uint32_t m8 = tid < rounds * IPB ? s_mask[tid] : 0u;
        if (m8) {
            const uint32_t i = (uint32_t)(i_base + tid);
            s_list[atomicAdd(&s_cnt, 1u)] = i;
            if (G >= 2) {
                const int nv = __popc(m8), c = nv > 4 ? 0 : nv > 2 ? 1 : 2;
                s_rl[c][atomicAdd(&s_rc[c], 1u)] = i | (m8 << 24);
            }
        }
    }
    __syncthreads();
    const uint32_t cnt = s_cnt;
    if (tid == 0 && cnt) s_base = atomicAdd(&hdr->n_active, cnt);
    if (G >= 2 && tid < 3) s_rb[tid] = s_rc[tid] ? atomicAdd(&hdr->n_runs[tid], s_rc[tid]) : 0u;
    __syncthreads();
    for (uint32_t k = tid; k < cnt; k += 256) active_list[s_base + k] = s_list[k];
    if (G >= 2) {
#pragma unroll
        for (int c = 0; c < 3; ++c)
            for (uint32_t k = tid; k < s_rc[c]; k += 256) run_list[(size_t)c * N + s_rb[c] + k] = s_rl[c][k];
    }
}

template <int G, int BMAX, bool MIXED, bool SH_HALF, bool RUNS, int NVV = 8, bool POSE = false>
__device__ __forceinline__ void inst_bwd_body(
    int blk, int n_active, const uint32_t* __restrict__ active_list,
    int v_first, int v_count, int N, int B, int n_art, int W, int H, const float* __restrict__ cams,
    const float* __restrict__ xyz, const float* __restrict__ log_scale, const float* __restrict__ rot,
    const float* __restrict__ op_logit, const float* __restrict__ f_dc, const float* __restrict__ f_rest,
    const float* __restrict__ skin_w, const float* __restrict__ transforms, const float4* __restrict__ iacc,
    float grad2d_scale, int accumulate,
    float* __restrict__ d_xyz, float* __restrict__ d_ls, float* __restrict__ d_rot, float* __restrict__ d_op,
    float* __restrict__ d_fdc, float* __restrict__ d_frest, float* __restrict__ d_w, float* __restrict__ st_grad2d,
    unsigned char* __restrict__ pose_valid = nullptr) {
    constexpr int IPB = IB_THREADS / G;
    constexpr int NV = RUNS ? NVV : G;
    extern __shared__ __align__(16) float s_view[];
    if (blk * IPB >= n_active) return;
// ... 193 lines not shown
        h->rows_seq = hdr->bwd_seq;
        h->rows_owner[0] = (uint32_t)owner;
        h->rows_owner[1] = (uint32_t)(owner >> 32);
    }
    const int b8 = (n8 + IB_THREADS / 8 - 1) / (IB_THREADS / 8), b4 = (n4 + IB_THREADS / 4 - 1) / (IB_THREADS / 4);
    if constexpr (NVV >= 8) {
        if (blk < b8) { inst_bwd_body<8, BMAX, MIXED, SH_HALF, true, NVV, POSE>(blk, n8, active_list, MGR_IB_ARGS, pose_valid); return; }
    }
    blk -= b8;
    if constexpr (NVV >= 4) {
        if (blk < b4) { inst_bwd_body<4, BMAX, MIXED, SH_HALF, true, NVV, POSE>(blk, n4, active_list + (size_t)N, MGR_IB_ARGS, pose_valid); return; }
    }
    blk -= b4;
    inst_bwd_body<2, BMAX, MIXED, SH_HALF, true, NVV, POSE>(blk, n2, active_list + 2 * (size_t)N, MGR_IB_ARGS, pose_valid);
}
template <int NVV, int BMAX, bool MIXED, bool SH_HALF>
__global__ __launch_bounds__(IB_THREADS) __attribute__((amdgpu_waves_per_eu(MGR_IB_WAVES, MGR_IB_WAVES))) void k_inst_bwd_runs(MGR_IB_PARAMS) {
    inst_bwd_runs<NVV, BMAX, MIXED, SH_HALF, false>(MGR_IB_ALL, nullptr);
}

template <int G, int BMAX, bool MIXED, bool SH_HALF>
__global__ __launch_bounds__(IB_THREADS) __attribute__((amdgpu_waves_per_eu(MGR_IB_WAVES, MGR_IB_WAVES))) void k_inst_bwd_pose(MGR_IB_PARAMS, unsigned char* __restrict__ pose_valid) {
    inst_bwd_body<G, BMAX, MIXED, SH_HALF, false, 8, true>((int)blockIdx.x, (int)hdr->n_active, active_list, MGR_IB_ARGS, pose_valid);
}
template <int NVV, int BMAX, bool MIXED, bool SH_HALF>
__global__ __launch_bounds__(IB_THREADS) __attribute__((amdgpu_waves_per_eu(MGR_IB_WAVES, MGR_IB_WAVES))) void k_inst_bwd_runs_pose(MGR_IB_PARAMS, unsigned char* __restrict__ pose_valid) {
    inst_bwd_runs<NVV, BMAX, MIXED, SH_HALF, true>(MGR_IB_ALL, pose_valid);
}

template <int NV>
__global__ __launch_bounds__(256) void k_pose_part_views(int n_art, int B, int n_chunks, const float4* __restrict__ iacc,
                                                         const unsigned char* __restrict__ valid,
                                                         const float* __restrict__ skin_w, float* __restrict__ part) {
    constexpr int IPB = 256 / NV;
    __shared__ float s_rec[256 * MGR_POSE_REC];
    __shared__ unsigned char s_lst[NV * 256];
    __shared__ int s_cnt[8], s_wc[8 * 4];
    const int tid = threadIdx.x, vl = tid & (NV - 1), il = tid / NV;
    float pacc[12];
#pragma unroll
    for (int k = 0; k < 12; ++k) pacc[k] = 0.f;
    for (int c = blockIdx.x; c < n_chunks; c += gridDim.x) {
        const int i = c * IPB + il;
        const bool on = i < n_art && valid[(size_t)i * NV + vl] != 0;
        if (on) {
            const float4* o = iacc + ((size_t)i * NV + vl) * 3;
            const float4 a = o[0], b = o[1], d = o[2];
            float* r = s_rec + tid * MGR_POSE_REC;
            r[0] = a.x; r[1] = a.y; r[2] = a.z; r[3] = a.w; r[4] = b.x; r[5] = b.y; r[6] = b.z; r[7] = b.w;
            r[8] = d.x; r[9] = d.y; r[10] = d.z; r[11] = d.w;
            r[12] = __int_as_float(i);
        }
        pose_wg_lists<256>(tid, NV, on ? vl : -1, s_lst, s_cnt, s_wc);
        pose_wg_accumulate<256>(tid, NV, B, s_rec, s_lst, s_cnt, skin_w, pacc);
        __syncthreads();
    }
    pose_wg_store<256>(tid, NV, B, s_rec, pacc, part + (size_t)blockIdx.x * NV * B * 12);
}

static std::atomic<int> g_inst_runs{[] { const char* e = getenv("MANUS_INST_RUNS"); return e ? atoi(e) : 1; }()};
extern "C" int mgr_views_backward_run_lists(int on) { return g_inst_runs.exchange(on); }

struct CanonGrads {
    int B, n_art, sh_half;
    const float *xyz, *log_scale, *rot, *op_logit, *f_dc, *f_rest, *skin_w, *transforms;
    const int32_t* radii;
    float grad2d_scale;
    float *d_xyz, *d_ls, *d_rot, *d_op, *d_fdc, *d_frest, *d_w, *st_grad2d, *st_vis;
    int32_t* st_radii;
    float *d_T, *pose_part;
};

static int pose_view_slots(int n_art, int Gv) {
    const int ipb = 256 / Gv, chunks = (n_art + ipb - 1) / ipb;
    return chunks < MGR_POSE_MAX_WG ? chunks : MGR_POSE_MAX_WG;
}
static size_t pose_part_bytes(int N, int B, int Gv) { return ((size_t)pose_view_slots(N, Gv) * Gv * B * 12 * sizeof(float) + 255) & ~(size_t)255; }
extern "C" size_t mgr_views_pose_workspace_bytes(int V, int N, int B) {
    if (V <= 0 || N <= 0 || B <= 0) return 0;
    const int Gv = V <= 1 ? 1 : V <= 2 ? 2 : V <= 4 ? 4 : 8;
    return pose_part_bytes(N, B, Gv) + (size_t)N * Gv;
}

static int raster_backward_impl(int V, int N, int W, int H, const float* cams, const float* bg,
                                   const float* means3D, int64_t s_means, const float* cov3D,
                                   int64_t s_cov, const float* colors, int64_t s_col,
                                   const float* opacity, int64_t s_op, const float* out_color,
                                   const float* dL_dcolor, float* dL_dmeans3D, float* dL_dmeans2D, float* dL_dcolors,
                                   float* dL_dopacity, float* dL_dcov3D, const CanonGrads* canon, void* workspace,
                                   size_t workspace_bytes, int64_t cap, int flags, void* stream_) {
    (void)colors; (void)s_col; (void)opacity; (void)s_op;
    hipStream_t stream = (hipStream_t)stream_;
    if (V <= 0 || N < 0 || W <= 0 || H <= 0 || cap < 0)
        return mgr_fail(MGR_EINVAL, "mgr_raster_backward: bad sizes");
    if (!cams || !bg || !dL_dcolor || !out_color || !workspace)
        return mgr_fail(MGR_EINVAL, "mgr_raster_backward: null pointer");
    if (N == 0) return MGR_OK;
    if (!canon && (!means3D || !cov3D || !dL_dmeans3D || !dL_dmeans2D || !dL_dcolors || !dL_dopacity || !dL_dcov3D))
        return mgr_fail(MGR_EINVAL, "mgr_raster_backward: null pointer");
    const int gx = (W + 15) / 16, gy = (H + 15) / 16;
    const MgrLayout L = mgr_layout(V, N, W, H, cap);
    if (workspace_bytes < L.total) return mgr_fail(MGR_ENOMEM, "mgr_raster_backward: workspace too small");
    char* ws = (char*)workspace;
    MgrHeader* hdr = (MgrHeader*)(ws + L.header);
    static std::atomic<uint32_t> g_epoch{0};
    uint32_t epoch = g_epoch.fetch_add(1) + 1;
    if (epoch == 0) epoch = g_epoch.fetch_add(1) + 1;

    { MGR_PROF("k_blend_bwd", stream); hipLaunchKernelGGL(k_blend_bwd, dim3(256 * BWD_WAVES), dim3(256), 0, stream, N, W, H, gx, gy,
                       (const uint32_t*)(ws + L.sorted_gid), (const MgrGRec*)(ws + L.grec), (const uint32_t*)(ws + L.n_contrib),
                       (const float4*)(ws + L.ckpt), (const uint4*)(ws + L.items), hdr, out_color,
                       dL_dcolor, (uint32_t*)(ws + L.pair_tag), (float4*)(ws + L.pair_grad),
                       (uint32_t*)(ws + L.inst_tag), (uint32_t)cap, epoch); }
    MGR_LAUNCH_CHECK("k_blend_bwd", stream, flags & MGR_BWD_CHECK);
    if (canon) {
        const int Gv = V <= 1 ? 1 : V <= 2 ? 2 : V <= 4 ? 4 : 8;
        const int ipb = 256 / Gv;
        const size_t lds = (size_t)Gv * (MGR_CAM_FLOATS + (canon->skin_w ? IB_TSTRIDE(canon->B) : 0)) * sizeof(float);
        float4* iacc = (float4*)(ws + L.inst_grad);
        uint32_t* alist = (uint32_t*)(ws + L.inst_grad + (size_t)N * Gv * 48);
        const int ipb2 = IB_THREADS / Gv;
        const bool mixed = canon->skin_w && canon->n_art < N;
        int rounds = (int)((long long)N / ((long long)ipb * 1024));
        rounds = rounds < 1 ? 1 : (rounds > IG_ROUNDS ? IG_ROUNDS : rounds);
        const dim3 grid((N + ipb2 - 1) / ipb2), grid_g((N + ipb * rounds - 1) / (ipb * rounds));
        for (int v0 = 0; v0 < V; v0 += Gv) {
            const int vc = V - v0 < Gv ? V - v0 : Gv;
            const int accm = v0 > 0 ? 1 : 0;
            if (v0 > 0) {
                MGR_HIP(hipMemsetAsync(&hdr->n_active, 0, 4, stream));
                MGR_HIP(hipMemsetAsync(&hdr->n_runs[0], 0, 12, stream));
            }
            const bool runs = g_inst_runs.load(std::memory_order_relaxed) != 0 && Gv >= 4 && canon->B <= 24 && N < (1 << 24);
            const int rounds_r = rounds < Gv ? rounds : Gv;
            const dim3 grid_gr((N + ipb * rounds_r - 1) / (ipb * rounds_r));
            uint32_t* rlist = alist + (size_t)N;
            unsigned char* row_state = V <= Gv ? (unsigned char*)(rlist + 3 * (size_t)N) : nullptr;
            const int kept = (flags & MGR_BWD_OUTPUTS_KEPT) && V <= Gv ? 1 : 0;
#define MGR_IG_LAUNCH(GG)                                                                                             \
    hipLaunchKernelGGL((k_inst_gather<GG>), grid_g, dim3(256), 0, stream, v0, vc, N, canon->B, canon->n_art, canon->radii, \
                       (const ushort4*)(ws + L.rect), (const uint32_t*)(ws + L.pair_off),                             \
                       (const uint32_t*)(ws + L.pair_tag), (const float4*)(ws + L.pair_grad),                        \
                       (const uint32_t*)(ws + L.inst_tag), (uint32_t)cap, epoch, accm, rounds, iacc, alist, hdr, canon->d_xyz, canon->d_ls, canon->d_rot, canon->d_op, canon->d_fdc,    \
                       canon->d_frest, canon->d_w, canon->st_grad2d, canon->st_vis, canon->st_radii, runs && GG == 8 ? rlist : (uint32_t*)nullptr)
#define MGR_IB_LAUNCH(GG, BB)                                                                                         \
    if (mixed && canon->sh_half) MGR_IB_LAUNCH2(GG, BB, true, true);                                                  \
    else if (mixed) MGR_IB_LAUNCH2(GG, BB, true, false);                                                              \
    else if (canon->sh_half) MGR_IB_LAUNCH2(GG, BB, false, true);                                                     \
    else MGR_IB_LAUNCH2(GG, BB, false, false)
#define MGR_IB_LAUNCH2(GG, BB, MX, HF)                                                                                \
    hipLaunchKernelGGL((k_inst_bwd<GG, BB, MX, HF>), grid, dim3(IB_THREADS), lds, stream, v0, vc, N, canon->B, canon->n_art, W, H, cams, canon->xyz, \
                       canon->log_scale, canon->rot, canon->op_logit, canon->f_dc, canon->f_rest, canon->skin_w,      \
                       canon->transforms, (const float4*)iacc, (const uint32_t*)alist, (const MgrHeader*)hdr,         \
                       canon->grad2d_scale, accm, canon->d_xyz, canon->d_ls, canon->d_rot, canon->d_op, canon->d_fdc, \
                       canon->d_frest, canon->d_w, canon->st_grad2d)
            {
                MGR_PROF("k_inst_gather", stream);
#define MGR_IGR_LAUNCH(GG)                                                                                            \
    hipLaunchKernelGGL((k_inst_gather_runs<GG>), grid_gr, dim3(256), 0, stream, v0, vc, N, canon->B, canon->n_art, canon->radii, \
                       (const ushort4*)(ws + L.rect), (const uint32_t*)(ws + L.pair_off),                             \
                       (const uint32_t*)(ws + L.pair_tag), (const float4*)(ws + L.pair_grad),                        \
                       (const uint32_t*)(ws + L.inst_tag), (uint32_t)cap, epoch, accm, rounds_r, iacc, alist, hdr, canon->d_xyz, canon->d_ls, canon->d_rot, canon->d_op, canon->d_fdc, \
                       canon->d_frest, canon->d_w, canon->st_grad2d, canon->st_vis, canon->st_radii, rlist, row_state, kept)
                const bool old_gather = g_inst_runs.load(std::memory_order_relaxed) == 2 && Gv == 8;
                if (runs && !old_gather) {
                    if (Gv == 8) MGR_IGR_LAUNCH(8);
                    else if (Gv == 4) MGR_IGR_LAUNCH(4);
                    else if (Gv == 2) MGR_IGR_LAUNCH(2);
                    else MGR_IGR_LAUNCH(1);
                }
#undef MGR_IGR_LAUNCH
                else if (Gv == 8) MGR_IG_LAUNCH(8);
                else if (Gv == 4) MGR_IG_LAUNCH(4);
                else if (Gv == 2) MGR_IG_LAUNCH(2);
                else MGR_IG_LAUNCH(1);
            }
            MgrProfScope prof_ib(canon->d_T ? "k_inst_bwd_pose" : "k_inst_bwd", stream);
#define MGR_IBR_LAUNCH(MX, HF)                                                                                        \
    if (Gv == 8) MGR_IBR_LAUNCH2(8, MX, HF); else if (Gv == 4) MGR_IBR_LAUNCH2(4, MX, HF); else MGR_IBR_LAUNCH2(2, MX, HF)
#define MGR_IBR_LAUNCH2(NN, MX, HF)                                                                                   \
    hipLaunchKernelGGL((k_inst_bwd_runs<NN, 24, MX, HF>), dim3(grid.x + 3), dim3(IB_THREADS), lds, stream, v0, vc, N, canon->B, canon->n_art, W, H, cams, canon->xyz, \
                       canon->log_scale, canon->rot, canon->op_logit, canon->f_dc, canon->f_rest, canon->skin_w,      \
                       canon->transforms, (const float4*)iacc, (const uint32_t*)rlist, (const MgrHeader*)hdr,         \
                       canon->grad2d_scale, accm, canon->d_xyz, canon->d_ls, canon->d_rot, canon->d_op, canon->d_fdc, \
                       canon->d_frest, canon->d_w, canon->st_grad2d)
            if (canon->d_T) {
                const int slots = pose_view_slots(canon->n_art, Gv);
                unsigned char* pvalid = (unsigned char*)canon->pose_part + pose_part_bytes(N, canon->B, Gv);
                MGR_HIP(hipMemsetAsync(pvalid, 0, (size_t)canon->n_art * Gv, stream));
#define MGR_IP_ARGS                                                                                                   \
    v0, vc, N, canon->B, canon->n_art, W, H, cams, canon->xyz, canon->log_scale, canon->rot, canon->op_logit, canon->f_dc,  \
        canon->f_rest, canon->skin_w, canon->transforms, (const float4*)iacc, (const uint32_t*)(runs && Gv >= 2 ? rlist : alist), \
        (const MgrHeader*)hdr, canon->grad2d_scale, accm, canon->d_xyz, canon->d_ls, canon->d_rot, canon->d_op,          \
        canon->d_fdc, canon->d_frest, canon->d_w, canon->st_grad2d, pvalid
#define MGR_IP_LAUNCH(KERNEL) hipLaunchKernelGGL(KERNEL, dim3(runs && Gv >= 2 ? grid.x + 3 : grid.x), dim3(IB_THREADS), lds, stream, MGR_IP_ARGS)
#define MGR_IP_FLAGS(K, GG, BB)                                                                                       \
    if (mixed && canon->sh_half) MGR_IP_LAUNCH((K<GG, BB, true, true>));                                               \
    else if (mixed) MGR_IP_LAUNCH((K<GG, BB, true, false>));                                                           \
    else if (canon->sh_half) MGR_IP_LAUNCH((K<GG, BB, false, true>));                                                  \
    else MGR_IP_LAUNCH((K<GG, BB, false, false>))
#define MGR_IP_VIEWS(K, BB)                                                                                           \
    if (Gv == 8) { MGR_IP_FLAGS(K, 8, BB); } else if (Gv == 4) { MGR_IP_FLAGS(K, 4, BB); } else if (Gv == 2) { MGR_IP_FLAGS(K, 2, BB); }
                if (runs && Gv >= 2) { MGR_IP_VIEWS(k_inst_bwd_runs_pose, 24) }
                else if (canon->B <= 24) { MGR_IP_VIEWS(k_inst_bwd_pose, 24) else { MGR_IP_FLAGS(k_inst_bwd_pose, 1, 24); } }
                else { MGR_IP_VIEWS(k_inst_bwd_pose, MGR_MAX_BONES) else { MGR_IP_FLAGS(k_inst_bwd_pose, 1, MGR_MAX_BONES); } }
#undef MGR_IP_VIEWS
#undef MGR_IP_FLAGS
#undef MGR_IP_LAUNCH
#undef MGR_IP_ARGS
                MGR_LAUNCH_CHECK("k_inst_bwd_pose", stream, flags & MGR_BWD_CHECK);
                if (prof_ib.on) { mgr_prof_end(stream); prof_ib.on = false; }
                {
                    MGR_PROF("k_pose_part_views", stream);
                    const int n_chunks = (canon->n_art + 256 / Gv - 1) / (256 / Gv);
#define MGR_PP_LAUNCH(NN) hipLaunchKernelGGL((k_pose_part_views<NN>), dim3(slots), dim3(256), 0, stream, canon->n_art, canon->B, n_chunks, \
                                             (const float4*)iacc, (const unsigned char*)pvalid, canon->skin_w, canon->pose_part)
                    if (Gv == 8) MGR_PP_LAUNCH(8); else if (Gv == 4) MGR_PP_LAUNCH(4); else if (Gv == 2) MGR_PP_LAUNCH(2); else MGR_PP_LAUNCH(1);
#undef MGR_PP_LAUNCH
                    MGR_LAUNCH_CHECK("k_pose_part_views", stream, flags & MGR_BWD_CHECK);
                }
                const int rc = mgr_pose_fold(v0, vc, Gv, canon->B, canon->pose_part, slots, canon->d_T, stream);
                if (rc != MGR_OK) return rc;
            } else
            if (runs && Gv >= 2) {
                if (mixed && canon->sh_half) MGR_IBR_LAUNCH(true, true);
                else if (mixed) MGR_IBR_LAUNCH(true, false);
                else if (canon->sh_half) MGR_IBR_LAUNCH(false, true);
                else MGR_IBR_LAUNCH(false, false);
            } else
#undef MGR_IBR_LAUNCH
#undef MGR_IBR_LAUNCH2
            if (canon->B <= 24) {
                if (Gv == 8) MGR_IB_LAUNCH(8, 24);
                else if (Gv == 4) MGR_IB_LAUNCH(4, 24);
                else if (Gv == 2) MGR_IB_LAUNCH(2, 24);
                else MGR_IB_LAUNCH(1, 24);
            } else {
                if (Gv == 8) MGR_IB_LAUNCH(8, MGR_MAX_BONES);
                else if (Gv == 4) MGR_IB_LAUNCH(4, MGR_MAX_BONES);
                else if (Gv == 2) MGR_IB_LAUNCH(2, MGR_MAX_BONES);
                else MGR_IB_LAUNCH(1, MGR_MAX_BONES);
            }
#undef MGR_IB_LAUNCH
#undef MGR_IB_LAUNCH2
#undef MGR_IG_LAUNCH
        }
    } else
    { MGR_PROF("k_preprocess_bwd", stream); hipLaunchKernelGGL(k_preprocess_bwd, dim3((N + 255) / 256, V), dim3(256), 0, stream, N, W, H, cams,
                       means3D, s_means, cov3D, s_cov, (const int32_t*)nullptr,
                       (const ushort4*)(ws + L.rect), (const uint32_t*)(ws + L.pair_off),
                       (const uint32_t*)(ws + L.pair_tag), (const float4*)(ws + L.pair_grad),
                       dL_dmeans3D, dL_dmeans2D, dL_dcolors, dL_dopacity, dL_dcov3D,
                       (const uint32_t*)(ws + L.inst_tag), (uint32_t)cap, epoch, hdr); }
    MGR_LAUNCH_CHECK("k_preprocess_bwd", stream, flags & MGR_BWD_CHECK);
    return MGR_OK;
}

extern "C" int mgr_views_active_list(void* workspace, int V, int N, int W, int H, int64_t cap, const uint32_t** list,
                                     const uint32_t** count) {
    if (!workspace || !list || !count || V <= 0 || N <= 0) return mgr_fail(MGR_EINVAL, "mgr_views_active_list: bad arguments");
    if (V > 8) return mgr_fail(MGR_EINVAL, "mgr_views_active_list: only defined for up to 8 views (one lane group)");
    const MgrLayout L = mgr_layout(V, N, W, H, cap);
    const int Gv = V <= 1 ? 1 : V <= 2 ? 2 : V <= 4 ? 4 : 8;
    char* ws = (char*)workspace;
    *list = (const uint32_t*)(ws + L.inst_grad + (size_t)N * Gv * 48);
    *count = &((const MgrHeader*)(ws + L.header))->n_active;
    return MGR_OK;
}

extern "C" int mgr_raster_backward(int V, int N, int W, int H, const float* cams, const float* bg,
                                   const float* means3D, int64_t s_means, const float* cov3D,
                                   int64_t s_cov, const float* colors, int64_t s_col,
                                   const float* opacity, int64_t s_op, const float* out_color,
                                   const float* dL_dcolor, float* dL_dmeans3D, float* dL_dmeans2D, float* dL_dcolors,
                                   float* dL_dopacity, float* dL_dcov3D, void* workspace,
                                   size_t workspace_bytes, int64_t cap, int flags, void* stream_) {
    return raster_backward_impl(V, N, W, H, cams, bg, means3D, s_means, cov3D, s_cov, colors, s_col, opacity, s_op,
                                out_color, dL_dcolor, dL_dmeans3D, dL_dmeans2D, dL_dcolors, dL_dopacity, dL_dcov3D,
                                nullptr, workspace, workspace_bytes, cap, flags, stream_);
}

extern "C" int mgr_views_backward(int V, int N, int B, int n_articulated, int sh_half, int W, int H, const float* cams, const float* bg,
                                  const float* xyz, const float* log_scale, const float* rot,
                                  const float* opacity_logit, const float* f_dc, const float* f_rest,
                                  const float* skin_w, const float* transforms, const int32_t* radii,
                                  const float* out_color, const float* dL_dcolor, float grad2d_scale,
                                  float* d_xyz, float* d_log_scale, float* d_rot, float* d_opacity_logit,
                                  float* d_f_dc, float* d_f_rest, float* d_skin_w, float* stat_grad2d,
                                  float* stat_vis, int32_t* stat_radii, void* workspace, size_t workspace_bytes,
                                  int64_t cap, int flags, void* stream_) {
    if (N > 0 && (!xyz || !log_scale || !rot || !opacity_logit || !f_dc || !f_rest || !radii || !d_xyz ||
                  !d_log_scale || !d_rot || !d_opacity_logit || !d_f_dc || !d_f_rest ||
                  (skin_w && (!transforms || !d_skin_w))))
        return mgr_fail(MGR_EINVAL, "mgr_views_backward: null pointer");
    if (skin_w && (B <= 0 || B > MGR_MAX_BONES)) return mgr_fail(MGR_EINVAL, "mgr_views_backward: bad B");
    if (skin_w && (n_articulated < 0 || n_articulated > N)) return mgr_fail(MGR_EINVAL, "mgr_views_backward: bad n_articulated");
    const CanonGrads cg = {B, skin_w ? n_articulated : 0, sh_half ? 1 : 0, xyz, log_scale, rot, opacity_logit, f_dc, f_rest, skin_w, transforms, radii,
                           grad2d_scale, d_xyz, d_log_scale, d_rot, d_opacity_logit, d_f_dc, d_f_rest, d_skin_w,
                           stat_grad2d, stat_vis, stat_radii};
    return raster_backward_impl(V, N, W, H, cams, bg, nullptr, 0, nullptr, 0, nullptr, 0, nullptr, 0, out_color,
                                dL_dcolor, nullptr, nullptr, nullptr, nullptr, nullptr, &cg, workspace, workspace_bytes,
                                cap, flags, stream_);
}

extern "C" int mgr_views_backward_pose(int V, int N, int B, int n_articulated, int sh_half, int W, int H, const float* cams, const float* bg,
                                       const float* xyz, const float* log_scale, const float* rot,
                                       const float* opacity_logit, const float* f_dc, const float* f_rest,
                                       const float* skin_w, const float* transforms, const int32_t* radii,
                                       const float* out_color, const float* dL_dcolor, float grad2d_scale,
                                       float* d_xyz, float* d_log_scale, float* d_rot, float* d_opacity_logit,
                                       float* d_f_dc, float* d_f_rest, float* d_skin_w, float* stat_grad2d,
                                       float* stat_vis, int32_t* stat_radii, void* workspace, size_t workspace_bytes,
                                       int64_t cap, int flags, float* d_transforms, void* pose_workspace,
                                       size_t pose_workspace_bytes, void* stream_) {
    if (!skin_w || !transforms || n_articulated <= 0)
        return mgr_fail(MGR_EINVAL, "mgr_views_backward_pose: no articulated Gaussians (a static object has no transforms)");
    if (B <= 0 || B > MGR_MAX_BONES || V <= 0 || N <= 0 || n_articulated > N) return mgr_fail(MGR_EINVAL, "mgr_views_backward_pose: bad sizes");
    if (!xyz || !log_scale || !rot || !opacity_logit || !f_dc || !f_rest || !radii || !d_xyz || !d_log_scale || !d_rot ||
        !d_opacity_logit || !d_f_dc || !d_f_rest || !d_skin_w || !d_transforms)
        return mgr_fail(MGR_EINVAL, "mgr_views_backward_pose: null pointer");
    if (!pose_workspace || pose_workspace_bytes < mgr_views_pose_workspace_bytes(V, N, B))
        return mgr_fail(MGR_ENOMEM, "mgr_views_backward_pose: pose workspace too small");
    const CanonGrads cg = {B, n_articulated, sh_half ? 1 : 0, xyz, log_scale, rot, opacity_logit, f_dc, f_rest, skin_w, transforms, radii,
                           grad2d_scale, d_xyz, d_log_scale, d_rot, d_opacity_logit, d_f_dc, d_f_rest, d_skin_w,
                           stat_grad2d, stat_vis, stat_radii, d_transforms, (float*)pose_workspace};
    return raster_backward_impl(V, N, W, H, cams, bg, nullptr, 0, nullptr, 0, nullptr, 0, nullptr, 0, out_color,
                                dL_dcolor, nullptr, nullptr, nullptr, nullptr, nullptr, &cg, workspace, workspace_bytes,
                                cap, flags, stream_);
}
```

### manus_amd/csrc/raster_fwd.hip

```cpp
#include <atomic>
#include <mutex>

#include "instance_math.h"
#include "il_list.h"

#include <cstdlib>
#include <cstring>
#include <map>
#include <string>
#include <vector>

thread_local char g_mgr_err[512] = {0};

int g_mgr_prof_on = 0;
namespace {
struct ProfRec { const char* name; hipEvent_t a, b; };
std::vector<ProfRec> g_prof_recs;
std::vector<hipEvent_t> g_prof_pool;
hipEvent_t prof_event() {
    if (!g_prof_pool.empty()) { hipEvent_t e = g_prof_pool.back(); g_prof_pool.pop_back(); return e; }
    hipEvent_t e;
    if (hipEventCreate(&e) != hipSuccess) return nullptr;
    return e;
}
// ... 129 lines not shown
    r.zmin = __uint_as_float(~lo_c);
    const float ext = __uint_as_float(hi) - r.zmin;
    r.scale = (hi != 0u && ext > 0.0f) ? (float)(MGR_DB_BUCKETS - 1) / ext : 0.0f;
    return r;
}
__device__ __forceinline__ uint32_t db_bucket(float z, const DbRange r) {
    const float f = (z - r.zmin) * r.scale;
    return f > 0.0f ? min((uint32_t)f, (uint32_t)MGR_DB_BUCKETS - 1u) : 0u;
}
__device__ __forceinline__ bool db_takes_part(int radius, ushort4 rc, unsigned long long am) {
    const uint32_t tiles = (uint32_t)((rc.z - rc.x) * (rc.w - rc.y));
    return radius > 0 && tiles > 0u && (tiles > 64u || am != 0ull);
}

__device__ __forceinline__ void pre_tail(int N, int gx, int gy, int v, int i, const ProjOut& po, float op_i,
                                         const float col[3], uint32_t* s_scan, uint32_t* s_hist, int lds_hist,
                                         MgrGRec* __restrict__ grec, float* __restrict__ depth,
                                         ushort4* __restrict__ rect, unsigned long long* __restrict__ alive,
                                         uint32_t* __restrict__ pair_off, uint32_t* __restrict__ tile_count,
                                         int32_t* __restrict__ radii, MgrHeader* hdr, uint32_t* __restrict__ zr_slot,
                                         const uint32_t* __restrict__ zcut_v = nullptr) {
    const int tid = threadIdx.x, T = gx * gy;
    const int radius = po.radius, x0 = po.x0, y0 = po.y0, x1 = po.x1, y1 = po.y1;
    const uint32_t tiles = (uint32_t)((x1 - x0) * (y1 - y0));
    {
        const uint32_t zb = (radius > 0 && tiles > 0u) ? __float_as_uint(po.zv) : 0u;
        const uint32_t wmax = mgr_wave_max_u32(zb), wminc = mgr_wave_max_u32(zb ? ~zb : 0u);
        if ((tid & 63) == 0 && wmax) { atomicMax(&s_scan[23], wmax); atomicMax(&s_scan[22], wminc); }
    }
    unsigned long long amask = ~0ull;
    if (radius > 0 && !(zcut_v && tiles <= 64)) {
        const bool small = tiles <= 64;
        const MgrCull cull = mgr_cull_init(po.px, po.py, po.ca, po.cb, po.cc, mgr_qmax(op_i));
        if (small) amask = 0ull;
        int k = 0;
        for (int y = y0; y < y1; ++y) {
            float dy_lo, dy_hi, dxo;
            mgr_cull_row(cull, 16.0f * y, 16.0f * y + 15.0f, dy_lo, dy_hi, dxo);
            for (int x = x0; x < x1; ++x, ++k) {
                if (small) {
                    if (mgr_cull_dead(cull, dy_lo, dy_hi, dxo, 16.0f * x, 16.0f * x + 15.0f)) continue;
                    amask |= 1ull << k;
                }
                if (lds_hist) atomicAdd(&s_hist[y * gx + x], 1u);
                else atomicAdd(&tile_count[(size_t)v * T + y * gx + x], 1u);
            }
        }
    } else if (radius > 0) {
        const MgrCull cull = mgr_cull_init(po.px, po.py, po.ca, po.cb, po.cc, mgr_qmax(op_i));
        const uint32_t zbits = __float_as_uint(po.zv);
        amask = 0ull;
        int k = 0;
        uint32_t zc = tiles ? zcut_v[y0 * gx + x0] : 0u;
        for (int y = y0; y < y1; ++y) {
            float dy_lo, dy_hi, dxo;
            mgr_cull_row(cull, 16.0f * y, 16.0f * y + 15.0f, dy_lo, dy_hi, dxo);
            for (int x = x0; x < x1; ++x, ++k) {
                const bool wrap = x + 1 == x1;
                const int nx = wrap ? x0 : x + 1, ny = wrap ? y + 1 : y;
                const uint32_t zn = zcut_v[min(ny, y1 - 1) * gx + nx];
                const bool dead = mgr_cull_dead(cull, dy_lo, dy_hi, dxo, 16.0f * x, 16.0f * x + 15.0f);
                if (!dead && zbits <= ~zc) {
                    amask |= 1ull << k;
                    if (lds_hist) atomicAdd(&s_hist[y * gx + x], 1u);
                    else atomicAdd(&tile_count[(size_t)v * T + y * gx + x], 1u);
                }
                zc = zn;
            }
        }
    }
    uint32_t block_total;
    const uint32_t local = block_excl_scan(tiles, s_scan, block_total);
    if (tid == 0) s_scan[20] = block_total ? atomicAdd(&hdr->acc_pairs, block_total) : 0u;
    __syncthreads();
    const uint32_t off = s_scan[20] + local;
    if (i < N) {
        const size_t vi = (size_t)v * N + i;
        MgrGRec r;
        r.x = po.px; r.y = po.py; r.ca = po.ca; r.cb = po.cb; r.cc = po.cc;
        r.op = op_i;
        r.r = col[0]; r.g = col[1]; r.b = col[2];
        r.rect_w = x1 - x0;
        r.slot_base = (int32_t)off - y0 * (x1 - x0) - x0;
        r.pad = 0;
        grec[vi] = r;
        depth[vi] = po.zv;
        rect[vi] = make_ushort4((unsigned short)x0, (unsigned short)y0, (unsigned short)x1, (unsigned short)y1);
        alive[vi] = amask;
        pair_off[vi] = off;
        radii[vi] = radius;
    }
    if (lds_hist) {
        __syncthreads();
        for (int k = tid; k < T; k += PRE_THREADS) {
            const uint32_t c = s_hist[k];
            if (c) atomicAdd(&tile_count[(size_t)v * T + k], c);
        }
    }
    if (tid == 0) { zr_slot[0] = s_scan[22]; zr_slot[1] = s_scan[23]; }
}

__global__ __launch_bounds__(PRE_THREADS) void k_preprocess(
    int N, int W, int H, int gx, int gy, const float* __restrict__ cams,
    const float* __restrict__ means3D, int64_t s_means, const float* __restrict__ cov3D,
    int64_t s_cov, const float* __restrict__ colors, int64_t s_col,
    const float* __restrict__ opacity, int64_t s_op, MgrGRec* __restrict__ grec,
    float* __restrict__ depth, ushort4* __restrict__ rect, unsigned long long* __restrict__ alive,
    uint32_t* __restrict__ pair_off, uint32_t* __restrict__ tile_count, int32_t* __restrict__ radii,
    MgrHeader* hdr, int lds_hist, uint32_t* __restrict__ db_zrange) {
    extern __shared__ uint32_t s_mem[];
    uint32_t* s_scan = s_mem;
    uint32_t* s_hist = s_mem + 32;
    const int v = blockIdx.y, tid = threadIdx.x;
    const int i = blockIdx.x * PRE_THREADS + tid;
    const int T = gx * gy;
    if (lds_hist) {
        for (int k = tid; k < T; k += PRE_THREADS) s_hist[k] = 0;
    }
    if (tid < 2) s_scan[22 + tid] = 0u;
    __syncthreads();

    MgrCam cam;
    mgr_load_cam(cams, v, cam);

    ProjOut po;
    po.radius = 0; po.x0 = po.y0 = po.x1 = po.y1 = 0;
    po.px = po.py = po.ca = po.cb = po.cc = po.zv = 0.f;
    if (i < N) {
        const float* mp = means3D + (size_t)v * s_means + (size_t)i * 3;
        const float p[3] = {mp[0], mp[1], mp[2]};
        const float* cp = cov3D + (size_t)v * s_cov + (size_t)i * 6;
        const float c6[6] = {cp[0], cp[1], cp[2], cp[3], cp[4], cp[5]};
        project_gaussian(cam, W, H, gx, gy, p, c6, po);
    }
    const float op_i = (i < N) ? opacity[(size_t)v * s_op + i] : 0.0f;
    float col[3] = {0.f, 0.f, 0.f};
    if (i < N) {
        const float* cp = colors + (size_t)v * s_col + (size_t)i * 3;
        col[0] = cp[0]; col[1] = cp[1]; col[2] = cp[2];
    }
    pre_tail(N, gx, gy, v, i, po, op_i, col, s_scan, s_hist, lds_hist, grec, depth, rect, alive, pair_off, tile_count,
             radii, hdr, db_zrange + 2 * ((size_t)v * gridDim.x + blockIdx.x));
}

template <bool MIXED, bool SH_HALF>
__global__ __launch_bounds__(PRE_THREADS) void k_inst_fwd(
    int N, int B, int n_art, int W, int H, int gx, int gy, const float* __restrict__ cams,
    const float* __restrict__ xyz, const float* __restrict__ log_scale, const float* __restrict__ rot,
    const float* __restrict__ op_logit, const float* __restrict__ f_dc, const float* __restrict__ f_rest,
    const float* __restrict__ skin_w, const float* __restrict__ transforms, MgrGRec* __restrict__ grec,
    float* __restrict__ depth, ushort4* __restrict__ rect, unsigned long long* __restrict__ alive,
    uint32_t* __restrict__ pair_off, uint32_t* __restrict__ tile_count, int32_t* __restrict__ radii,
    MgrHeader* hdr, int lds_hist, int V, const uint32_t* __restrict__ tile_zcut, uint32_t* __restrict__ db_zrange) {
    extern __shared__ uint32_t s_mem[];
    uint32_t* s_scan = s_mem;
    uint32_t* s_hist = s_mem + 32;
    const int tid = threadIdx.x;
    const int nrange = (N + PRE_THREADS - 1) / PRE_THREADS;
    const int xcd = blockIdx.x & 7, k = blockIdx.x >> 3;
    const int range = (k / V) * 8 + xcd, v = k % V;
    if (range >= nrange) return;
    const int i = range * PRE_THREADS + tid;
    const int T = gx * gy;
    if (lds_hist) {
        for (int k2 = tid; k2 < T; k2 += PRE_THREADS) s_hist[k2] = 0;
    }
    if (tid < 2) s_scan[22 + tid] = 0u;
// ... 2322 lines not shown

struct MgrSideStream {
    hipStream_t stream = nullptr;
    hipEvent_t fork = nullptr, join = nullptr;
    hipError_t init() {
        if (stream) return hipSuccess;
        hipError_t e = hipStreamCreateWithFlags(&stream, hipStreamNonBlocking);
        if (e != hipSuccess) return e;
        e = hipEventCreateWithFlags(&fork, hipEventDisableTiming);
        if (e != hipSuccess) return e;
        return hipEventCreateWithFlags(&join, hipEventDisableTiming);
    }
};
#define MGR_MAX_DEVICES 64
static MgrSideStream& mgr_side_stream(int device) {
    static thread_local MgrSideStream s[MGR_MAX_DEVICES];
    return s[device];
}

static std::mutex g_slot_mu;
template <typename T>
struct MgrSlots {
    struct { const void* ws; T v; } slot[64];
    bool set(const void* workspace, const T* v) {
        std::lock_guard<std::mutex> lk(g_slot_mu);
        int k_free = -1;
        for (int k = 0; k < 64; ++k) {
            if (slot[k].ws == workspace) { k_free = k; break; }
            if (!slot[k].ws && k_free < 0) k_free = k;
        }
        if (k_free < 0) return false;
        if (v) { slot[k_free].ws = workspace; slot[k_free].v = *v; }
        else if (slot[k_free].ws == workspace) slot[k_free].ws = nullptr;
        return true;
    }
    T take(const void* workspace) {
        std::lock_guard<std::mutex> lk(g_slot_mu);
        for (auto& m : slot)
            if (m.ws == workspace) { m.ws = nullptr; return m.v; }
        return T();
    }
};
static MgrSlots<uint32_t*> g_mirror;
static MgrSlots<IlListArgs> g_loss_list;

extern "C" int mgr_views_forward_attach_loss_list(const void* workspace, int V, int H, int W, const uint32_t* target_map,
                                                  void* loss_workspace, size_t loss_workspace_bytes) {
    if (!workspace) return mgr_fail(MGR_EINVAL, "mgr_views_forward_attach_loss_list: null workspace");
    if (!target_map) { g_loss_list.set(workspace, nullptr); return MGR_OK; }
    if (V <= 0 || H <= 0 || W <= 0 || W > ILS_MAXW || !loss_workspace) return mgr_fail(MGR_EINVAL, "mgr_views_forward_attach_loss_list: bad arguments");
    if (loss_workspace_bytes < (size_t)il_blocks(V, H, W) * 12 + 256) return mgr_fail(MGR_ENOMEM, "mgr_views_forward_attach_loss_list: loss workspace too small");
    const IlListArgs a = il_list_args(V, H, W, target_map, nullptr, loss_workspace);
    if (!g_loss_list.set(workspace, &a)) return mgr_fail(MGR_ENOMEM, "mgr_views_forward_attach_loss_list: too many pending lists");
    return MGR_OK;
}

extern "C" int mgr_raster_set_status_mirror(const void* workspace, void* host_words) {
    if (!workspace) return mgr_fail(MGR_EINVAL, "mgr_raster_set_status_mirror: null workspace");
    void* dev = nullptr;
    if (host_words) MGR_HIP(hipHostGetDevicePointer(&dev, host_words, 0));
    uint32_t* const words = (uint32_t*)dev;
    if (!g_mirror.set(workspace, host_words ? &words : nullptr))
        return mgr_fail(MGR_EINVAL, "mgr_raster_set_status_mirror: too many workspaces with a pending mirror");
    return MGR_OK;
}

static int raster_forward_impl(int V, int N, int W, int H, const float* cams, const float* bg,
                               const float* means3D, int64_t s_means, const float* cov3D,
                               int64_t s_cov, const float* colors, int64_t s_col,
                               const float* opacity, int64_t s_op, const CanonInputs* canon, float* out_color,
                               int32_t* radii, void* workspace, size_t workspace_bytes,
                               int64_t cap, int flags, void* stream_) {
    hipStream_t stream = (hipStream_t)stream_;
    const bool do_bin = !(flags & MGR_FWD_BLEND_ONLY), do_blend = !(flags & MGR_FWD_NO_BLEND), use_cut = (flags & MGR_FWD_DEPTH_CUT) && canon != nullptr;
    static const bool bg_fill_on = [] { const char* e = getenv("MANUS_BG_FILL"); return !(e && e[0] == 'b'); }();
    bool bg_filled = false;
    const int skip_tiers = ((flags & MGR_FWD_SKIP_BOX_LARGE) ? MGR_SKIP_BOX_LARGE : 0) | ((flags & MGR_FWD_SKIP_BOX_MID) ? MGR_SKIP_BOX_MID : 0) |
                           ((flags & MGR_FWD_SKIP_SORT_BEHIND) ? MGR_SKIP_SORT_BEHIND : 0) | ((flags & MGR_FWD_RANK_LARGE) ? MGR_SKIP_RANK_LARGE : 0);
    const int img_kept = (flags & MGR_FWD_IMAGE_KEPT) ? 1 : 0;
    const bool spread = (flags & MGR_FWD_SPREAD) != 0;
    const bool repair = use_cut && (flags & MGR_FWD_REPAIR) && W < 65536 && H < 65536 &&
                        (int64_t)((W + 15) / 16) * ((H + 15) / 16) <= (int64_t)MGR_REP_MAX_TILES;
    const int debug = flags & MGR_FWD_CHECK;
    if (V <= 0 || N < 0 || W <= 0 || H <= 0 || cap < 0 || cap > 0xFFFFFFF0ll)
        return mgr_fail(MGR_EINVAL, "mgr_raster_forward: bad sizes");
    if (!cams || !bg || !out_color || !workspace ||
        (N > 0 && !canon && (!means3D || !cov3D || !colors || !opacity)) || (N > 0 && !radii))
        return mgr_fail(MGR_EINVAL, "mgr_raster_forward: null pointer");
    const int gx = (W + 15) / 16, gy = (H + 15) / 16, T = gx * gy;
    if (gx > 65535 || gy > 65535) return mgr_fail(MGR_EINVAL, "mgr_raster_forward: image too large");
    const MgrLayout L = mgr_layout(V, N, W, H, cap);
    if (workspace_bytes < L.total) return mgr_fail(MGR_ENOMEM, "mgr_raster_forward: workspace too small");
    char* ws = (char*)workspace;
    MgrHeader* hdr = (MgrHeader*)(ws + L.header);
    uint32_t* tile_count = (uint32_t*)(ws + L.tile_count);
    uint32_t* tile_start = (uint32_t*)(ws + L.tile_start);
    const int VT = V * T;
    MgrRep rep_all;
    rep_all.unit = (MgrRepUnit*)(ws + L.rep_unit); rep_all.state = (float4*)(ws + L.rep_state); rep_all.last = (uint32_t*)(ws + L.rep_last);
    rep_all.cnt = (uint32_t*)(ws + L.rep_cnt); rep_all.tile_rep = (uint32_t*)(ws + L.tile_rep); rep_all.cand = (unsigned long long*)(ws + L.rep_cand);
    rep_all.view = (MgrRepView*)(ws + L.rep_view);
    rep_all.max_units = repair ? mgr_rep_units(cap) : 0u;
    rep_all.list_cap = mgr_rep_list(cap); rep_all.ck_cap = mgr_rep_ck(cap);
    rep_all.list_base = (uint32_t)cap; rep_all.ck_base = (uint32_t)(cap / MGR_CHUNK + 1);

    static std::atomic<bool> attr_set[MGR_MAX_DEVICES];
    int device = 0;
    MGR_HIP(hipGetDevice(&device));
    if (device < 0 || device >= MGR_MAX_DEVICES) return mgr_fail(MGR_EINVAL, "mgr_raster_forward: device index out of range");
    if (!attr_set[device].load(std::memory_order_acquire)) {
        MGR_HIP(hipFuncSetAttribute((const void*)k_tile_sort, hipFuncAttributeMaxDynamicSharedMemorySize,
                                    SORT_LDS_KEYS * 8 + RS_WAVES * 256 * 4 + 256));
        MGR_HIP(hipFuncSetAttribute((const void*)k_preprocess, hipFuncAttributeMaxDynamicSharedMemorySize,
                                    152 * 1024));
        MGR_HIP(hipFuncSetAttribute((const void*)k_emit, hipFuncAttributeMaxDynamicSharedMemorySize,
                                    152 * 1024));
        MGR_HIP(hipFuncSetAttribute((const void*)k_inst_fwd<false, false>, hipFuncAttributeMaxDynamicSharedMemorySize, 152 * 1024));
        MGR_HIP(hipFuncSetAttribute((const void*)k_inst_fwd<true, false>, hipFuncAttributeMaxDynamicSharedMemorySize, 152 * 1024));
        MGR_HIP(hipFuncSetAttribute((const void*)k_inst_fwd<false, true>, hipFuncAttributeMaxDynamicSharedMemorySize, 152 * 1024));
        MGR_HIP(hipFuncSetAttribute((const void*)k_inst_fwd<true, true>, hipFuncAttributeMaxDynamicSharedMemorySize, 152 * 1024));
        MGR_HIP(hipFuncSetAttribute((const void*)k_dbin_sort<SORT_LDS_KEYS>, hipFuncAttributeMaxDynamicSharedMemorySize,
                                    SORT_LDS_KEYS * 8 + RS_WAVES * 256 * 4 + 256));
        MGR_HIP(hipFuncSetAttribute((const void*)k_bin_count<false>, hipFuncAttributeMaxDynamicSharedMemorySize, 152 * 1024));
        MGR_HIP(hipFuncSetAttribute((const void*)k_bin_scatter<0, false>, hipFuncAttributeMaxDynamicSharedMemorySize, 152 * 1024));
        MGR_HIP(hipFuncSetAttribute((const void*)k_bin_scatter<0, true>, hipFuncAttributeMaxDynamicSharedMemorySize, 152 * 1024));
        MGR_HIP(hipFuncSetAttribute((const void*)k_repair_blend, hipFuncAttributeMaxDynamicSharedMemorySize, REP_BLEND_LDS));
        attr_set[device].store(true, std::memory_order_release);
    }

    const int lds_hist = ((size_t)T * 4 + 128 <= 150 * 1024) ? 1 : 0;
    const char* binning_env = getenv("MGR_BINNING");
    const bool ordered_env = !(binning_env && strcmp(binning_env, "sorted") == 0);
    const bool ordered = ordered_env && lds_hist && T <= 65535 && (size_t)T * 4 + BIN_SC_FIXED_BYTES <= 150 * 1024;
    const size_t hist_bytes = lds_hist ? (size_t)T * 4 : 0;
    if (do_bin) {

    if (N > 0) {
        dim3 grid((N + PRE_THREADS - 1) / PRE_THREADS, V);
        if (canon) {
            MGR_PROF("k_inst_fwd", stream);
            const bool mixed = canon->skin_w && canon->n_art < N;
#define MGR_IF_LAUNCH(MX, HF)                                                                                           \
    hipLaunchKernelGGL((k_inst_fwd<MX, HF>), dim3(8 * ((grid.x + 7) / 8) * V), dim3(PRE_THREADS), 128 + hist_bytes, stream, N, canon->B, canon->n_art, W, H, \
                       gx, gy, cams, canon->xyz, canon->log_scale, canon->rot, canon->op_logit, canon->f_dc,            \
                       canon->f_rest, canon->skin_w, canon->transforms, (MgrGRec*)(ws + L.grec),                        \
                       (float*)(ws + L.depth), (ushort4*)(ws + L.rect), (unsigned long long*)(ws + L.alive),            \
                       (uint32_t*)(ws + L.pair_off), tile_count, radii, hdr, lds_hist, V,                                  \
                       use_cut ? (const uint32_t*)(ws + L.tile_zcut) : (const uint32_t*)nullptr, (uint32_t*)(ws + L.db_zrange))
            if (mixed && canon->sh_half) MGR_IF_LAUNCH(true, true);
            else if (mixed) MGR_IF_LAUNCH(true, false);
            else if (canon->sh_half) MGR_IF_LAUNCH(false, true);
            else MGR_IF_LAUNCH(false, false);
#undef MGR_IF_LAUNCH
        } else
        { MGR_PROF("k_preprocess", stream); hipLaunchKernelGGL(k_preprocess, grid, dim3(PRE_THREADS), 128 + hist_bytes, stream, N, W, H, gx,
                           gy, cams, means3D, s_means, cov3D, s_cov, colors, s_col, opacity, s_op,
                           (MgrGRec*)(ws + L.grec), (float*)(ws + L.depth), (ushort4*)(ws + L.rect),
                           (unsigned long long*)(ws + L.alive), (uint32_t*)(ws + L.pair_off), tile_count, radii,
                           hdr, lds_hist, (uint32_t*)(ws + L.db_zrange)); }
        MGR_LAUNCH_CHECK("k_preprocess", stream, debug);
    }
    {
        const int nbT = (T + 1023) / 1024, nblk = V * nbT;
        uint2* part = (uint2*)(ws + L.scan_part);
        uint32_t* blk_cls = (uint32_t*)(ws + L.scan_cls);
        const int use_hint = ordered ? 1 : 0;
        const bool dbin = ordered && N > 0;
        const int n_bx = (N + 1024 * DB_PER - 1) / (1024 * DB_PER);
// ... 96 lines not shown
                           tile_start, (const uint32_t*)(ws + L.tile_queue), (unsigned long long*)(ws + L.keys),
                           (unsigned long long*)(ws + L.keys2), (uint4*)(ws + L.groups),
                           (uint32_t*)(ws + L.sorted_gid), hdr, (uint32_t)cap); }
        { MGR_PROF("k_tile_sort_small", side.stream); hipLaunchKernelGGL(k_tile_sort_small, dim3(256 * 8), dim3(256), 0, side.stream,
                           tile_start, (const uint32_t*)(ws + L.tile_queue),
                           (const unsigned long long*)(ws + L.keys), (uint32_t*)(ws + L.sorted_gid), hdr,
                           (uint32_t)cap); }
        MGR_HIP(hipEventRecord(side.join, side.stream));
        { MGR_PROF("k_tile_sort", stream); hipLaunchKernelGGL(k_tile_sort, dim3(512), dim3(RS_THREADS), SORT_LDS_KEYS * 8 + RS_WAVES * 256 * 4 + 256, stream,
                           tile_start, (const uint32_t*)(ws + L.tile_queue),
                           (const unsigned long long*)(ws + L.keys), (const unsigned long long*)(ws + L.keys2),
                           (const uint4*)(ws + L.groups), (uint32_t*)(ws + L.sorted_gid), hdr, (uint32_t)cap); }
        MGR_HIP(hipStreamWaitEvent(stream, side.join, 0));
        MGR_LAUNCH_CHECK("k_tile_sort", stream, debug);
    }
    }
    if (!do_blend) return MGR_OK;
    { MGR_PROF("k_blend_fwd", stream); hipLaunchKernelGGL(k_blend_fwd, dim3(MGR_FWD_GRID), dim3(256), 0, stream, N, W, H, gx, gy, VT, bg,
                       (const uint32_t*)(ws + L.tile_queue), (const uint4*)(ws + L.tile_qrec), (const uint32_t*)(ws + L.sorted_gid), (const MgrGRec*)(ws + L.grec), out_color,
                       (uint32_t*)(ws + L.n_contrib), (uint32_t*)(ws + L.tile_done), (uint32_t*)(ws + L.tile_qdone),
                       (float4*)(ws + L.ckpt), hdr, (const uint32_t*)(ws + L.tile_zused), (uint32_t*)(ws + L.tile_qend), bg_filled ? 1 : 0); }
    if (repair && N > 0) {
        { MGR_PROF("k_repair_scan", stream);
          hipLaunchKernelGGL(k_repair_prep, dim3(V), dim3(256), 0, stream, T, gx, hdr, rep_all, (const uint32_t*)(ws + L.tile_zused),
                             (const uint32_t*)(ws + L.tile_zwin));
          hipLaunchKernelGGL(k_repair_scan, dim3(REP_SCAN_SEGS, V), dim3(REP_SCAN_THREADS), 0, stream, N, T, gx, hdr, rep_all, (const int32_t*)radii,
                             (const ushort4*)(ws + L.rect), (const float*)(ws + L.depth), (const MgrGRec*)(ws + L.grec)); }
        { MGR_PROF("k_repair_blend", stream);
          hipLaunchKernelGGL(k_repair_blend, dim3(128), dim3(RS_THREADS), REP_BLEND_LDS, stream, N, W, H, gx, T, hdr, rep_all, bg,
                             (uint32_t*)(ws + L.sorted_gid), (const MgrGRec*)(ws + L.grec), out_color, (uint32_t*)(ws + L.n_contrib),
                             (uint32_t*)(ws + L.tile_qdone), (float4*)(ws + L.ckpt)); }
        MGR_LAUNCH_CHECK("k_repair_blend", stream, debug);
    }
    IlListArgs ll = g_loss_list.take(workspace);
    if (ll.nbx) {
        if (ll.H != H || ll.W != W || ll.list_views != V) return mgr_fail(MGR_EINVAL, "attached loss list: views or image size differ from the forward's");
        ll.tile_start = tile_start;
    }
    const int n_item_blocks = (VT + 255) / 256;
    const MgrFeatStamp stamp = {{(uint32_t)V, (uint32_t)N, (uint32_t)W, (uint32_t)H, (uint32_t)cap}, use_cut ? MGR_FEAT_CUT : 0u};
    { MGR_PROF("k_fwd_items", stream); hipLaunchKernelGGL(k_fwd_items, dim3((unsigned)(n_item_blocks + ll.nbx * V)), dim3(256), 0, stream, (const uint4*)(ws + L.tile_qrec),
                       (const uint32_t*)(ws + L.tile_qdone), (uint32_t*)(ws + L.tile_done), (uint4*)(ws + L.items), hdr,
                       N, T, (const uint32_t*)(ws + L.sorted_gid), (const float*)(ws + L.depth), (const uint32_t*)(ws + L.tile_zused),
                       (const uint32_t*)(ws + L.tile_qend), (uint32_t*)(ws + L.tile_zcut), g_mirror.take(workspace),
                       g_cut_frac, (uint32_t)g_cut_min, g_cut_range, g_cut_rel, gx, g_cut_interior,
                       (const uint32_t*)(ws + L.tile_queue), VT, (unsigned char*)(ws + L.tile_bgok), (const float*)out_color, bg, rep_all,
                       (uint32_t)g_cut_penalty, (uint32_t*)(ws + L.tile_zwin), ll, n_item_blocks, stamp); }
    MGR_LAUNCH_CHECK("k_blend_fwd", stream, debug);
    return MGR_OK;
}

extern "C" int mgr_raster_forward(int V, int N, int W, int H, const float* cams, const float* bg,
                                  const float* means3D, int64_t s_means, const float* cov3D,
                                  int64_t s_cov, const float* colors, int64_t s_col,
                                  const float* opacity, int64_t s_op, float* out_color,
                                  int32_t* radii, void* workspace, size_t workspace_bytes,
                                  int64_t cap, int flags, void* stream_) {
    return raster_forward_impl(V, N, W, H, cams, bg, means3D, s_means, cov3D, s_cov, colors, s_col, opacity, s_op,
                               nullptr, out_color, radii, workspace, workspace_bytes, cap, flags, stream_);
}

extern "C" int mgr_views_forward(int V, int N, int B, int n_articulated, int sh_half, int W, int H, const float* cams, const float* bg,
                                 const float* xyz, const float* log_scale, const float* rot,
                                 const float* opacity_logit, const float* f_dc, const float* f_rest,
                                 const float* skin_w, const float* transforms, float* out_color,
                                 int32_t* radii, void* workspace, size_t workspace_bytes, int64_t cap,
                                 int flags, void* stream_) {
    if (N > 0 && (!xyz || !log_scale || !rot || !opacity_logit || !f_dc || !f_rest || (skin_w && !transforms)))
        return mgr_fail(MGR_EINVAL, "mgr_views_forward: null pointer");
    if (skin_w && (B <= 0 || B > MGR_MAX_BONES)) return mgr_fail(MGR_EINVAL, "mgr_views_forward: bad B");
    if (skin_w && (n_articulated < 0 || n_articulated > N)) return mgr_fail(MGR_EINVAL, "mgr_views_forward: bad n_articulated");
    if (sh_half && ((uintptr_t)f_rest & 15)) return mgr_fail(MGR_EINVAL, "mgr_views_forward: fp16 f_rest must be 16-byte aligned");
    const CanonInputs ci = {B, skin_w ? n_articulated : 0, sh_half ? 1 : 0, xyz, log_scale, rot, opacity_logit, f_dc, f_rest, skin_w, transforms};
    return raster_forward_impl(V, N, W, H, cams, bg, nullptr, 0, nullptr, 0, nullptr, 0, nullptr, 0, &ci, out_color,
                               radii, workspace, workspace_bytes, cap, flags, stream_);
}

#ifdef BIN_PROF
extern "C" int mgr_binprof(unsigned long long* out) {
    MGR_HIP(hipMemcpyFromSymbol(out, HIP_SYMBOL(g_binprof), 8 * 8 * 4096));
    return 0;
}
#endif
extern "C" int mgr_raster_layout(int V, int N, int W, int H, int64_t cap, size_t* out, int n_out) {
    const MgrLayout L = mgr_layout(V, N, W, H, cap);
    const size_t v[] = {L.header, L.grec, L.depth, L.rect, L.alive, L.pair_off, L.tile_count, L.tile_start,
                        L.tile_cursor, L.tile_done, L.tile_queue, L.chunk_start, L.items, L.ckpt, L.keys,
                        L.sorted_gid, L.final_T, L.n_contrib, L.pair_tag, L.pair_grad, L.total, L.inst_grad, L.inst_tag,
                        L.db_nvis, L.db_bbox, L.db_order, L.tile_zcut, L.tile_zused, L.tile_qend, L.tile_rep, L.rep_unit, L.rep_cnt, L.tile_zwin};
    const int n = (int)(sizeof(v) / sizeof(v[0]));
    for (int i = 0; i < n && i < n_out; ++i) out[i] = v[i];
    return n;
}

__global__ void k_debug_pair_alpha(int n, const float* __restrict__ rec, const int32_t* __restrict__ px,
                                   const int32_t* __restrict__ py, float* __restrict__ alpha, int32_t* __restrict__ valid) {
    const int i = blockIdx.x * blockDim.x + threadIdx.x;
    if (i >= n) return;
    float pb[MGR_PAIR_FLOATS];
    const float* r = rec + (size_t)i * 6;
    mgr_pair_store(pb, 0, r[0], r[1], r[2], r[3], r[4], r[5], 0.f, 0.f, 0.f, 1u);
    mgr_pair_pad(pb);
    const float4 R0 = make_float4(pb[0], pb[1], pb[2], pb[3]), R1 = make_float4(pb[4], pb[5], pb[6], pb[7]),
                 R2 = make_float4(pb[8], pb[9], pb[10], pb[11]);
    const mgr_v2f fpx2 = {(float)px[i], (float)px[i]}, fpy2 = {(float)py[i], (float)py[i]};
    mgr_v2f dx, dy, G, al;
    bool va, vb;
    mgr_pair_alpha(R0, R1, R2, fpx2, fpy2, dx, dy, G, al, va, vb);
    alpha[i] = al.x;
    valid[i] = va ? 1 : 0;
}

extern "C" int mgr_debug_pair_alpha(int n, const float* rec, const int32_t* px, const int32_t* py, float* alpha,
                                    int32_t* valid, void* stream_) {
    if (n < 0 || (n > 0 && (!rec || !px || !py || !alpha || !valid))) return mgr_fail(MGR_EINVAL, "mgr_debug_pair_alpha: bad arguments");
    if (n == 0) return MGR_OK;
    hipStream_t stream = (hipStream_t)stream_;
    hipLaunchKernelGGL(k_debug_pair_alpha, dim3((n + 255) / 256), dim3(256), 0, stream, n, rec, px, py, alpha, valid);
    MGR_LAUNCH_CHECK("k_debug_pair_alpha", stream, 0);
    return MGR_OK;
}

static int mgr_overflow_code(uint32_t ovf) {
    if (ovf & MGR_OVF_PAIRS) return mgr_fail(MGR_EOVERFLOW, "pair capacity exceeded");
    if (ovf & MGR_OVF_CUT) return mgr_fail(MGR_ECUT, "depth cut violated: run the forward again without MGR_FWD_DEPTH_CUT");
    if (ovf & MGR_OVF_TIER) return mgr_fail(MGR_ETIER, "a skipped binning launch was needed: run the forward again without MGR_FWD_SKIP_*");
    return MGR_OK;
}

extern "C" int mgr_raster_status_sync(const void* workspace, int64_t* num_pairs, int32_t* overflow,
                                      void* stream_) {
    hipStream_t stream = (hipStream_t)stream_;
    uint32_t h[2] = {0, 0};
    MGR_HIP(hipMemcpyAsync(h, workspace, 8, hipMemcpyDeviceToHost, stream));
    MGR_HIP(hipStreamSynchronize(stream));
    if (num_pairs) *num_pairs = h[0];
    if (overflow) *overflow = (int32_t)h[1];
    return mgr_overflow_code(h[1]);
}

extern "C" int mgr_raster_status_tiers_sync(const void* workspace, int64_t* num_pairs, int32_t* overflow, int32_t* tiers,
                                            void* stream_) {
    hipStream_t stream = (hipStream_t)stream_;
    uint32_t h[64];
    static_assert(offsetof(MgrHeader, sort_near_large) / 4 < 64, "status words beyond the copied part of the header");
    MGR_HIP(hipMemcpyAsync(h, workspace, sizeof(h), hipMemcpyDeviceToHost, stream));
    MGR_HIP(hipStreamSynchronize(stream));
    if (num_pairs) *num_pairs = h[0];
    if (overflow) *overflow = (int32_t)h[1];
    if (tiers) {
        const uint32_t sb = h[offsetof(MgrHeader, sort_big) / 4], sn = h[offsetof(MgrHeader, sort_near_large) / 4], sl = h[offsetof(MgrHeader, sort_large) / 4];
        const uint32_t near_max = MGR_TIERS_NEAR_MASK, beyond_max = MGR_TIERS_BEYOND_SMALL_MASK;
        *tiers = (int32_t)(h[offsetof(MgrHeader, tiers) / 4] | ((sb < near_max ? sb : near_max) << MGR_TIERS_NEAR_SMALL_SHIFT) |
                           ((sn < near_max ? sn : near_max) << MGR_TIERS_NEAR_LARGE_SHIFT) | ((sl < beyond_max ? sl : beyond_max) << MGR_TIERS_BEYOND_SMALL_SHIFT));
    }
    return mgr_overflow_code(h[1]);
}

extern "C" int mgr_raster_debug_binning_sync(const void* workspace, int V, int N, int W, int H,
                                             int64_t cap, int view, int32_t* tile_ranges_host,
                                             int32_t* point_list_host, int64_t max_pairs,
                                             void* stream_) {
    hipStream_t stream = (hipStream_t)stream_;
    const int gx = (W + 15) / 16, gy = (H + 15) / 16, T = gx * gy;
    if (view < 0 || view >= V) return mgr_fail(MGR_EINVAL, "bad view");
    const MgrLayout L = mgr_layout(V, N, W, H, cap);
// ... 21 lines not shown
```

### manus_amd/engine.py

```python
import ctypes
import functools
import os

import torch
import torch.distributed as dist

from . import fused as fused_mod, losses, ops, rasterizer
from . import _lib
from ._lib import ManusHipError, check, lib, ptr, stream

GRAD_LAYOUT = (("_xyz", 3), ("_features_dc", 3), ("_features_rest", 45), ("_opacity", 1),
               ("_scaling", 3), ("_rotation", 4))
GRAD_WIDTH = sum(w for _, w in GRAD_LAYOUT)
FLAT_TAIL = 2

LAYOUT_TILE_START, LAYOUT_TILE_DONE = 7, 9
LAYOUT_FINAL_T, LAYOUT_N_CONTRIB, LAYOUT_INST_TAG = 16, 17, 22
LAYOUT_TILE_ZCUT, LAYOUT_TILE_ZUSED, LAYOUT_TILE_QEND = 26, 27, 28
LAYOUT_TILE_REP, LAYOUT_REP_UNIT, LAYOUT_REP_CNT, LAYOUT_TILE_ZWIN = 29, 30, 31, 32


def flat_size(N):
    return N * (GRAD_WIDTH + 2) + FLAT_TAIL

# ... 759 lines not shown
        tgt, bg = sel["targets"], self.s["bg"]
        if route is None:
            if g_img is not None:
                return (out * g_img).sum(), g_img.contiguous()
            return self._image_loss(out, tgt, scale, tiles=(bg, self._tile_start_ptr(ws, V, N, W, H)))
        if route == "mapped":
            lws, tmap, nbytes = loss_list
            if not self.attach_list:
                check(lib().mgr_image_loss_tiles_list_mapped(V, H, W, ptr(tmap), ptr(bg), ctypes.c_void_p(self._tile_start_ptr(ws, V, N, W, H)),
                                                             ptr(lws), nbytes, 1, stream()), "mgr_image_loss_tiles_list_mapped")
        else:
            nbytes = int(lib().mgr_image_loss_workspace_bytes(V, H, W))
            lws = torch.empty(nbytes, dtype=torch.uint8, device=self.device)
            cur = torch.cuda.current_stream(self.device)
            if self._side is None:
                self._side = torch.cuda.Stream(device=self.device)
            self._side.wait_stream(cur)
            with torch.cuda.stream(self._side):
                check(lib().mgr_image_loss_tiles_list(V, H, W, ptr(tgt), ptr(bg), ctypes.c_void_p(self._tile_start_ptr(ws, V, N, W, H)),
                                                      ptr(lws), nbytes, stream()), "mgr_image_loss_tiles_list")
            self._views_forward(ws, fwd, _lib.MGR_FWD_BLEND_ONLY)
            if ctx.fenced(self.sync_check):
                ctx.fence(ws)
            cur.wait_stream(self._side)
            lws.record_stream(self._side)
        k, const = self._loss_scales(out, scale)
        g_img = torch.empty_like(out)
        sums = torch.empty(3, dtype=torch.float32, device=self.device)
        check(lib().mgr_image_loss_tiles_finish(V, H, W, ptr(out), ptr(tgt), self.w_rgb, self.w_ssim, k, const, ptr(g_img),
                                                ptr(sums), ptr(lws), nbytes, stream()), "mgr_image_loss_tiles_finish")
        return sums[2], g_img

    def _map_chain(self, ws, head, sel, view_ids, scale, map_on, grads, d_w, d_T=None):
        V, N, B, na, _, W, H = head[:7]
        cams, xyz, ls, rot, op, w, T = head[7], head[9], head[10], head[11], head[12], head[15], head[16]
        dev, L = self.device, lib()
        masks, depths = self._map_sel(sel, view_ids, map_on[1])
        key = (V, N, W, H, ws.cap, bool(map_on[1]))
        mb = self._map_bufs.get(key)
        if mb is None:
            e = functools.partial(torch.empty, dtype=torch.float32, device=dev)
            n_loss, n_scr = int(L.mgr_map_loss_workspace_bytes(V, H, W)), int(L.mgr_views_maps_backward_workspace_bytes(V, N, W, H, ws.cap))
            mb = dict(alpha=e((V, H, W)), g_alpha=e((V, H, W)), depth=e((V, 1, H, W)) if map_on[1] else None,
                      g_depth=e((V, 1, H, W)) if map_on[1] else None,
                      loss_ws=torch.empty(n_loss, dtype=torch.uint8, device=dev), scratch=torch.empty(n_scr, dtype=torch.uint8, device=dev))
            self._map_bufs = {key: mb}
        sums = torch.empty(3, dtype=torch.float32, device=dev)
        rc = L.mgr_raster_blend_features(V, N, 0, W, H, None, 0, None, int(map_on[1]), ptr(mb["depth"]), ptr(mb["alpha"]), ptr(ws.buf),
                                         ws.nbytes, ws.cap, stream())
        if rc == _lib.MGR_ESTATE and int(ws.buf[4:8].view(torch.int32).item()) != 0:
            z = torch.zeros((), dtype=torch.float32, device=dev)
            return z, z, z
        check(rc, "mgr_raster_blend_features")
        k = scale * V
        check(L.mgr_map_loss(V, H, W, ptr(mb["alpha"]), ptr(masks), ptr(mb["depth"]), ptr(depths), self.w_mask,
                             self.w_depth if map_on[1] else 0.0, k, ptr(mb["g_alpha"]), ptr(mb["g_depth"]), ptr(sums), ptr(mb["loss_ws"]),
                             mb["loss_ws"].numel(), stream()), "mgr_map_loss")
        args = (V, N, B, na, W, H, cams, xyz, ls, rot, op, w, T, ptr(mb["alpha"]), ptr(mb["depth"]), ptr(mb["g_alpha"]), ptr(mb["g_depth"]), 1,
                ptr(grads["_xyz"]), ptr(grads["_scaling"]), ptr(grads["_rotation"]), ptr(grads["_opacity"]), ptr(d_w), ptr(ws.buf),
                ws.nbytes, ws.cap, ptr(mb["scratch"]), mb["scratch"].numel(), 0)
        if d_T is not None:
            nbytes = int(L.mgr_views_maps_pose_workspace_bytes(V, N, B))
            if self._map_pose_ws is None or self._map_pose_ws.numel() < nbytes:
                self._map_pose_ws = torch.empty(nbytes, dtype=torch.uint8, device=dev)
            check(L.mgr_views_maps_backward_pose(*args, 1, ptr(d_T), ptr(self._map_pose_ws), self._map_pose_ws.numel(), stream()),
                  "mgr_views_maps_backward_pose")
        else:
            check(L.mgr_views_maps_backward(*args, stream()), "mgr_views_maps_backward")
        return sums[2] * k, sums[0] * k, sums[1] * k

    def _backward(self, ws, fwd, g_img, scale, full_rows=False):
        head, out, radii, kept = fwd
        V, N, B, na = head[:4]
        dev = self.device
        e = kept.get if kept is not None else functools.partial(_arena_tensor, self.grad_arena or {}, dev)
        grads = {name: e(shape, name) for name, shape in (("_xyz", (N, 3)), ("_scaling", (N, 3)), ("_rotation", (N, 4)), ("_opacity", (N, 1)),
                                                           ("_features_dc", (N, 1, 3)), ("_features_rest", (N, 15, 3)))}
        st_g, st_v = e((N,), "grad2d"), e((N,), "vis")
        st_r = torch.empty(N, dtype=torch.int32, device=dev)
        d_w = e((na, B), "_skin_w") if na else None
        bits = _lib.MGR_BWD_OUTPUTS_KEPT if (kept is not None and kept.grad_ws is ws and V <= 8 and not full_rows) else 0
        self._kept.grad_ws = None
        args = (*head, ptr(radii), ptr(out), ptr(g_img), 1.0 / scale, *[ptr(g) for g in grads.values()],
                ptr(d_w), ptr(st_g), ptr(st_v), ptr(st_r), ptr(ws.buf), ws.nbytes, ws.cap, bits)
        d_T = None
        if self.pose_grad:
            d_T = torch.empty((V, B, 4, 4), dtype=torch.float32, device=dev)
            nbytes = int(lib().mgr_views_pose_workspace_bytes(V, N, B))
            if self._pose_ws is None or self._pose_ws.numel() < nbytes:
                self._pose_ws = torch.empty(nbytes, dtype=torch.uint8, device=dev)
            check(lib().mgr_views_backward_pose(*args, ptr(d_T), ptr(self._pose_ws), self._pose_ws.numel(), stream()),
                  "mgr_views_backward_pose")
        else:
            check(lib().mgr_views_backward(*args, stream()), "mgr_views_backward")
        if kept is not None:
            kept.handed_out(ws)
            if full_rows:
                kept.grad_ws = None
        return grads, d_w, st_g, st_v, st_r, d_T

    def _skin_backward(self, ws, head, xyz, d_w, d_xyz, full_rows=False):
        V, N, _, na, _, W, H = head[:7]
        active = None
        if V <= 8 and N > 0 and not full_rows:
            lst, cnt = ctypes.c_void_p(), ctypes.c_void_p()
            check(lib().mgr_views_active_list(ptr(ws.buf), V, N, W, H, ws.cap, ctypes.byref(lst), ctypes.byref(cnt)),
                  "mgr_views_active_list")
            active = (lst, cnt)
        if not na:
            return active
        s, sg = self.s, self.grid
        grid = (na, ptr(xyz), ptr(sg.data), sg.D, sg.H, sg.W, sg.B, sg.stride, ptr(s["grid_center"]), ptr(s["grid_scale"]), ptr(d_w), ptr(d_xyz))
        if active is not None:
            check(lib().mgr_skin_weights_bwd_indexed(*grid, lst, cnt, N, stream()), "mgr_skin_weights_bwd_indexed")
        else:
            check(lib().mgr_skin_weights_bwd(*grid, 1, stream()), "mgr_skin_weights_bwd")
        return active

    def _d_w_rows(self, d_w):
        na, B = d_w.shape
        L, dev = lib(), d_w.device
        r = self._sg_rows
        if r is None or r["idx"].numel() != na or r["idx"].device != dev:
            r = self._sg_rows = dict(mask=torch.empty(na, dtype=torch.uint8, device=dev), idx=torch.empty(na, dtype=torch.int32, device=dev),
                                     count=torch.zeros(1, dtype=torch.int32, device=dev),
                                     ws=torch.empty(L.mgr_exchange_index_workspace_bytes(na), dtype=torch.uint8, device=dev))
        check(L.mgr_skin_rows_mask(na, B, ptr(d_w), ptr(r["mask"]), stream()), "mgr_skin_rows_mask")
        check(L.mgr_exchange_index(na, ptr(r["mask"]), ptr(r["idx"]), ptr(r["count"]), ptr(r["ws"]), r["ws"].numel(), stream()), "mgr_exchange_index")
        return ptr(r["idx"]), ptr(r["count"])

    def _skin_grid_backward(self, head, xyz, d_w, active, rows_of_d_w=False):
        V, N, _, na = head[:4]
        s = self.s
        lst, cnt = active if active is not None else (None, None)
        self.last_skin_w_grad = d_w
        if rows_of_d_w and V <= 8 and na:
            lst, cnt = self._d_w_rows(d_w)
            return self.ops._skin_grid_grad(na, xyz, self.grid, s["grid_center"], s["grid_scale"], d_w, lst, cnt, na,
                                            kept=self._sg_kept if self.persistent_grads else None)
        return self.ops._skin_grid_grad(na, xyz, self.grid, s["grid_center"], s["grid_scale"], d_w, lst, cnt, N if active is not None else na,
                                        kept=self._sg_kept if self.persistent_grads else None)

    def __call__(self, view_ids, scale=1.0):
        if self.fused:
            return self._step_direct(view_ids, scale)
        self.last_active = None
        for v in self.params.values():
            v.grad = None
        sel = self._select(view_ids)
        T = sel["T"].detach().requires_grad_(True) if self.pose_grad else None
        map_on = self._map_terms()
        tgt = sel["targets"]
        map_out = None
        if any(map_on):
            img, radii, means2D, extras = self.forward_views(view_ids, T=T, maps=(True, map_on[1]))
            loss, g = self._image_loss(img, tgt, scale)
            masks, depths = self._map_sel(sel, view_ids, map_on[1])
            k = scale * len(view_ids)
            ml, sums = losses.map_loss(extras["alpha"], masks, self.w_mask, extras["depth"] if map_on[1] else None, depths,
                                       self.w_depth if map_on[1] else 0.0)
            torch.autograd.backward([img, ml * k], [g, None])
            map_out = (sums[2] * k, sums[0] * k, sums[1] * k)
            loss = loss + map_out[0]
        else:
            img, radii, means2D = self.forward_views(view_ids, T=T)
            loss, g = self._image_loss(img, tgt, scale)
            img.backward(g)
# ... 260 lines not shown
```

### manus_amd/fused.py

```python
import torch

from . import rasterizer as _rz
from ._lib import check, f32c, lib, ptr, stream


class ViewStats:

    def __init__(self):
        self.grad2d = self.vis = self.radii = None


class _RenderViews(torch.autograd.Function):
    @staticmethod
    def forward(ctx, xyz, log_scale, rot, opacity, f_dc, f_rest, skin_w, transforms, cams, bg, W, H, stats,
                grad2d_scale, grad_arena=None):
        xyz, log_scale, rot = f32c(xyz), f32c(log_scale), f32c(rot)
        opacity, f_dc, f_rest = f32c(opacity).reshape(-1), f32c(f_dc), f32c(f_rest)
        N, V = xyz.shape[0], cams.shape[0]
        B = n_art = 0
        if skin_w is not None:
            skin_w, transforms = f32c(skin_w), f32c(transforms)
            n_art, B = skin_w.shape
            if n_art > N:
                raise _rz._lib.ManusHipError("render_views: more skin-weight rows than Gaussians")
            if transforms.shape[0] != V or transforms.shape[1] != B:
                raise _rz._lib.ManusHipError("render_views: transforms must be (V,B,4,4), one pose per view")
        bg = f32c(bg).reshape(-1)
        dev = xyz.device
        out = torch.empty((V, 3, H, W), dtype=torch.float32, device=dev)
        radii = torch.empty((V, N), dtype=torch.int32, device=dev)

        sh_half = 0

        def launch(ws):
            check(lib().mgr_views_forward(V, N, B, n_art, sh_half, W, H, ptr(cams), ptr(bg), ptr(xyz), ptr(log_scale), ptr(rot),
                                          ptr(opacity), ptr(f_dc), ptr(f_rest), ptr(skin_w), ptr(transforms),
                                          ptr(out), ptr(radii), ptr(ws.buf), ws.nbytes, ws.cap, ws.skip_bits(), stream()),
                  "mgr_views_forward")

        ws, _ = _rz.context(dev).forward(V, N, W, H, launch)
        ctx.lease = _rz._Lease(ws)
        ctx.meta = (V, N, B, n_art, W, H, stats, float(grad2d_scale))
        ctx.arena = grad_arena
        ctx.save_for_backward(xyz, log_scale, rot, opacity, f_dc, f_rest, skin_w, transforms, cams, bg, out, radii)
        ctx.mark_non_differentiable(radii)
        return out, radii

    @staticmethod
    def backward(ctx, g_img, _g_radii):
        xyz, log_scale, rot, opacity, f_dc, f_rest, skin_w, transforms, cams, bg, out, radii = ctx.saved_tensors
        V, N, B, n_art, W, H, stats, g2s = ctx.meta
        ws = ctx.lease.ws
        dev = xyz.device
        g_img = f32c(g_img)
        arena = ctx.arena or {}

        def e(*s, name=None):
            t = arena.get(name) if name else None
            if t is not None and t.numel() == int(torch.Size(s).numel()) and t.is_contiguous() and t.dtype == torch.float32 \
                    and t.device == dev:
                return t.view(s)
            return torch.empty(s, dtype=torch.float32, device=dev)

        d_xyz, d_ls, d_rot, d_op = e(N, 3), e(N, 3, name="_scaling"), e(N, 4, name="_rotation"), e(N, name="_opacity")
        d_fdc, d_frest = e(N, 1, 3, name="_features_dc"), e(N, 15, 3, name="_features_rest")
        d_w = e(n_art, B) if skin_w is not None else None
        st_g, st_v = (e(N, name="grad2d"), e(N, name="vis")) if stats is not None else (None, None)
        st_r = torch.empty(N, dtype=torch.int32, device=dev) if stats is not None else None
        sh_half = 0
        check(lib().mgr_views_backward(V, N, B, n_art, sh_half, W, H, ptr(cams), ptr(bg), ptr(xyz), ptr(log_scale), ptr(rot),
                                       ptr(opacity), ptr(f_dc), ptr(f_rest), ptr(skin_w), ptr(transforms),
                                       ptr(radii), ptr(out), ptr(g_img), g2s, ptr(d_xyz), ptr(d_ls), ptr(d_rot),
                                       ptr(d_op), ptr(d_fdc), ptr(d_frest), ptr(d_w), ptr(st_g), ptr(st_v),
                                       ptr(st_r), ptr(ws.buf), ws.nbytes, ws.cap, 0, stream()),
              "mgr_views_backward")
        if stats is not None:
            stats.grad2d, stats.vis, stats.radii = st_g, st_v, st_r
        return (d_xyz, d_ls, d_rot, d_op.reshape(-1, 1), d_fdc, d_frest, d_w, None, None, None, None, None, None,
                None, None)


def render_views(xyz, log_scale, rot, opacity_logit, f_dc, f_rest, skin_w, transforms, cams, bg, W, H,
                 stats=None, grad2d_scale=1.0, grad_arena=None):
    return _RenderViews.apply(xyz, log_scale, rot, opacity_logit, f_dc, f_rest, skin_w, transforms, cams, bg,
                              int(W), int(H), stats, grad2d_scale, grad_arena)
```

### manus_amd/rasterizer.py

```python
from typing import NamedTuple

import ctypes
import os
import time
import weakref

import torch
import torch.nn as nn

from . import _lib
from ._lib import (check, f32c, lib, ptr, stream, MGR_FWD_RANK_LARGE, MGR_FWD_SKIP_BOX_LARGE, MGR_FWD_SKIP_BOX_MID, MGR_FWD_SKIP_SORT_BEHIND,
                   MGR_FWD_SPREAD, MGR_OVF_CUT, MGR_OVF_FLAGS_MASK, MGR_OVF_PAIRS, MGR_OVF_REPAIRED_SHIFT, MGR_OVF_TIER, MGR_TIERS_BEYOND_SMALL_MASK,
                   MGR_TIERS_BEYOND_SMALL_SHIFT, MGR_TIERS_BOX_LARGE, MGR_TIERS_BOX_MID, MGR_TIERS_NEAR_LARGE_SHIFT, MGR_TIERS_NEAR_MASK,
                   MGR_TIERS_NEAR_SMALL_SHIFT, MGR_TIERS_WIDE_RECT)
from .ops import lbs_cov, sh_colors


class GaussianRasterizationSettings(NamedTuple):
    image_height: int
    image_width: int
    tanfovx: float
    tanfovy: float
    bg: torch.Tensor
    scale_modifier: float
    viewmatrix: torch.Tensor
    projmatrix: torch.Tensor
    sh_degree: int
    campos: torch.Tensor
    prefiltered: bool
    debug: bool


class RasterWorkspace:
    SORT_BIG_MAX = int(os.environ.get("MANUS_SORT_BIG_MAX", "0"))

    def __init__(self, device, V, N, W, H, cap):
        self.key = (V, N, W, H)
        self.cap = int(cap)
        self.nbytes = int(lib().mgr_raster_workspace_bytes(V, N, W, H, self.cap))
        self.buf = torch.zeros(self.nbytes, dtype=torch.uint8, device=device)
        self.busy = False
        self.hint_key = self.prev_hint_key = None
        self.cut_block = False
        self.mirror = None
        self.tiers = None
        self.no_flagging_skips = False

    def skip_bits(self):
        t = self.tiers
        if t is None:
            return 0
        large = (t >> MGR_TIERS_BEYOND_SMALL_SHIFT) & MGR_TIERS_BEYOND_SMALL_MASK
        near = (t >> (MGR_TIERS_NEAR_LARGE_SHIFT if large else MGR_TIERS_NEAR_SMALL_SHIFT)) & MGR_TIERS_NEAR_MASK
        bits = ((MGR_FWD_RANK_LARGE if large else 0) | (MGR_FWD_SPREAD if t & MGR_TIERS_WIDE_RECT else 0))
        if not self.no_flagging_skips:
            bits |= ((0 if t & MGR_TIERS_BOX_LARGE else MGR_FWD_SKIP_BOX_LARGE) | (0 if t & MGR_TIERS_BOX_MID else MGR_FWD_SKIP_BOX_MID)
                     | (MGR_FWD_SKIP_SORT_BEHIND if near <= RasterWorkspace.SORT_BIG_MAX else 0))
        return bits


def default_pair_capacity(V, N):
    return max(4096, 8 * V * max(N, 1))


class RasterContext:

    MAX_FENCES = 64
    AUTO_FENCE_AFTER = int(os.environ.get("MANUS_AUTO_FENCE_AFTER", "8"))

    def __init__(self, device):
        self.device = torch.device(device)
        self.pool = {}
        self.cap_hint = {}
        self.sync_every_forward = True
        self.last_ws = None
        self._fences = []
        self._free_pinned = []
        self._evicted_overflow = False
        self.cut_retries = 0
        self.cut_repairs = 0
        self._clean = {}
        self._seen = {}
        self.auto_fenced = 0
        self.tier_retries = 0

    def acquire(self, V, N, W, H, min_cap):
        lst = self.pool.setdefault((V, N, W, H), [])
        for ws in lst:
            if not ws.busy and ws.cap >= min_cap:
                ws.busy = True
                return ws
        lst[:] = [w for w in lst if w.busy]
        ws = RasterWorkspace(self.device, V, N, W, H, min_cap)
        ws.busy = True
        lst.append(ws)
        return ws

    def clear(self):
        if self._fences:
            torch.cuda.synchronize(self.device)
        for ws, pinned, ev in self._fences:
            if pinned is not None:
                self._free_pinned.append(pinned)
        for lst in self.pool.values():
            for ws in lst:
                if ws.mirror is not None:
                    lib().mgr_raster_set_status_mirror(ptr(ws.buf), None)
                    self._free_pinned.append(ws.mirror)
                    ws.mirror = None
        self.pool.clear()
        self.cap_hint.clear()
        self._fences.clear()
        self._evicted_overflow = False
        self.last_ws = None
        self._clean.clear()
        self._seen.clear()

    _SYNC = (False, MGR_OVF_PAIRS, MGR_OVF_PAIRS | MGR_OVF_CUT)
    _FENCE = (True, 0, 0)
    _RECHECK = (True, MGR_OVF_PAIRS, 0)

# ... 159 lines not shown
    return context(device).check_overflow()


def poll(device=None):
    return context(device).poll()


class _Lease:

    def __init__(self, ws):
        self.ws = ws

    def __del__(self):
        self.ws.busy = False


def _run_forward(cams, V, N, W, H, bg, means3D, cov3D, colors, opacity, debug, sync_check=True, graph=True):
    dev = means3D.device
    out = torch.empty((V, 3, H, W), dtype=torch.float32, device=dev)
    radii = torch.empty((V, N), dtype=torch.int32, device=dev)
    s_m = means3D.stride(0) if means3D.dim() == 3 else 0
    s_c = cov3D.stride(0) if cov3D.dim() == 3 else 0
    s_col = colors.stride(0) if colors.dim() == 3 else 0
    s_o = opacity.stride(0) if opacity.dim() == 2 else 0

    def launch(ws):
        check(lib().mgr_raster_forward(V, N, W, H, ptr(cams), ptr(bg), ptr(means3D), s_m, ptr(cov3D), s_c,
                                       ptr(colors), s_col, ptr(opacity), s_o, ptr(out), ptr(radii),
                                       ptr(ws.buf), ws.nbytes, ws.cap, (_lib.MGR_FWD_CHECK if debug else 0) | ws.skip_bits(), stream()),
              "mgr_raster_forward")

    ws, npairs = context(dev).forward(V, N, W, H, launch, sync_check, auto_fence=graph, cams=cams)
    return out, radii, ws, npairs


def _opacity_layout(op, V, N):
    if op.dim() == 3:
        return op.reshape(V, N)
    if op.dim() == 2 and op.shape[1] == 1:
        return op.reshape(N)
    if op.dim() == 2:
        return op.reshape(V, N)
    return op.reshape(N)


class _RasterizeGaussians(torch.autograd.Function):
    @staticmethod
    def forward(ctx, means3D, means2D, colors, opacities, cov3D, cams, bg, W, H, debug, graph=True, share=None):
        V = cams.shape[0]
        means3D, colors, cov3D = f32c(means3D), f32c(colors), f32c(cov3D)
        opac = f32c(opacities)
        N = means3D.shape[-2]
        opac = _opacity_layout(opac, V, N)
        bg = f32c(bg).reshape(-1)
        out, radii, ws, npairs = _run_forward(cams, V, N, W, H, bg, means3D, cov3D, colors, opac, debug, graph=graph)
        ctx.lease = _Lease(ws)
        if share is not None:
            share.lease = ctx.lease
        ctx.meta = (V, N, W, H, bool(debug), means2D.shape, opacities.shape)
        ctx.num_rendered = npairs
        ctx.save_for_backward(means3D, colors, opac, cov3D, cams, bg, out)
        ctx.mark_non_differentiable(radii)
        return out, radii

    @staticmethod
    def backward(ctx, g_color, _g_radii):
        means3D, colors, opac, cov3D, cams, bg, out = ctx.saved_tensors
        V, N, W, H, debug, m2d_shape, op_shape = ctx.meta
        ws = ctx.lease.ws
        dev = means3D.device
        g_color = f32c(g_color)
        d_m3 = torch.empty((V, N, 3), dtype=torch.float32, device=dev)
        d_m2 = torch.empty((V, N, 3), dtype=torch.float32, device=dev)
        d_col = torch.empty((V, N, 3), dtype=torch.float32, device=dev)
        d_op = torch.empty((V, N), dtype=torch.float32, device=dev)
        d_cov = torch.empty((V, N, 6), dtype=torch.float32, device=dev)
        s_m = means3D.stride(0) if means3D.dim() == 3 else 0
        s_c = cov3D.stride(0) if cov3D.dim() == 3 else 0
        s_col = colors.stride(0) if colors.dim() == 3 else 0
        s_o = opac.stride(0) if opac.dim() == 2 else 0
        check(lib().mgr_raster_backward(V, N, W, H, ptr(cams), ptr(bg), ptr(means3D), s_m, ptr(cov3D), s_c,
                                        ptr(colors), s_col, ptr(opac), s_o, ptr(out), ptr(g_color), ptr(d_m3), ptr(d_m2),
                                        ptr(d_col), ptr(d_op), ptr(d_cov), ptr(ws.buf), ws.nbytes, ws.cap,
                                        _lib.MGR_BWD_CHECK if debug else 0, stream()), "mgr_raster_backward")

        def fold(g, shared, shape=None):
            if shared:
                g = g.sum(0) if V > 1 else g[0]
            return g.reshape(shape) if shape is not None else g

        g_m3 = fold(d_m3, means3D.dim() == 2)
        g_m2 = fold(d_m2, len(m2d_shape) == 2, m2d_shape)
        g_col = fold(d_col, colors.dim() == 2)
        g_op = fold(d_op, opac.dim() == 1, op_shape)
        g_cov = fold(d_cov, cov3D.dim() == 2)
        return g_m3, g_m2, g_col, g_op, g_cov, None, None, None, None, None, None, None


def _builds_graph(*tensors):
    return torch.is_grad_enabled() and any(torch.is_tensor(t) and t.requires_grad for t in tensors)


def rasterize_views(cams, means3D, means2D, colors, opacities, cov3D, bg, W, H, debug=False):
    return _RasterizeGaussians.apply(means3D, means2D, colors, opacities, cov3D, cams, bg, int(W), int(H), debug,
                                     _builds_graph(means3D, means2D, colors, opacities, cov3D))


MAX_FEATURE_CHANNELS = 32


def _feature_request(features, bg, depth, alpha):
    C = 0
    if features is not None:
        if not torch.is_tensor(features) or features.dim() not in (2, 3):
            raise _lib.ManusHipError("features must be a tensor (N,C), shared by the views, or (V,N,C)")
        C = int(features.shape[-1])
        if not 1 <= C <= MAX_FEATURE_CHANNELS:
            raise _lib.ManusHipError("features carry %d channels; 1 .. %d are supported" % (C, MAX_FEATURE_CHANNELS))
    if C == 0 and not depth and not alpha:
        raise _lib.ManusHipError("nothing to render: no features, no depth, no alpha")
    if bg is not None:
        bg = torch.as_tensor(bg, dtype=torch.float32).reshape(-1)
        if bg.numel() != C:
            raise _lib.ManusHipError("bg has %d values for %d feature channels" % (bg.numel(), C))
    return C, bg


def blend_features(features=None, bg=None, depth=False, alpha=False, device=None):
    C, bg = _feature_request(features, bg, depth, alpha)
    with torch.no_grad():
        ctx = context(device)
        ws = ctx.last_ws
        if ws is None:
            raise _lib.ManusHipError("blend_features: no forward has run on this context")
        V, N, W, H = ws.key
        dev = ws.buf.device
        s_f = 0
        if features is not None:
            if features.shape[-2] != N or (features.dim() == 3 and features.shape[0] != V):
                raise _lib.ManusHipError("features %s do not fit the last forward's %d views of %d Gaussians" % (tuple(features.shape), V, N))
            features = f32c(features.detach().to(dev))
            s_f = N * C if features.dim() == 3 else 0
        if bg is not None:
            bg = bg.to(dev).contiguous()
        n_out = C + (1 if depth else 0)
        out = torch.empty((V, n_out, H, W), dtype=torch.float32, device=dev) if n_out else None
        out_a = torch.empty((V, H, W), dtype=torch.float32, device=dev) if alpha else None
        check(lib().mgr_raster_blend_features(V, N, C, W, H, ptr(features), s_f, ptr(bg), int(bool(depth)), ptr(out), ptr(out_a),
                                              ptr(ws.buf), ws.nbytes, ws.cap, stream()), "mgr_raster_blend_features")
        return {"features": out[:, :C] if C else None, "depth": out[:, C] if depth else None, "alpha": out_a}


class _LeaseShare:
    lease = None


def _forward_seq(ws):
    seq = ctypes.c_uint32(0)
    check(lib().mgr_raster_forward_seq_sync(ptr(ws.buf), ctypes.byref(seq), stream()), "mgr_raster_forward_seq_sync")
    return int(seq.value)


class _BlendFeatures(torch.autograd.Function):

    @staticmethod
    def forward(ctx, means3D, means2D, opacities, cov3D, features, cams, bg, lease, depth, alpha, debug):
        ws = lease.ws
# ... 128 lines not shown
```

Measured before the change: 782.0.

## Track per-instance tile hits with 64-bit masks instead of scanning pair tags

```diff
diff --git a/include/manus_hip.h b/include/manus_hip.h
--- a/include/manus_hip.h
+++ b/include/manus_hip.h
@@ -38,6 +38,7 @@
 
 #define MGR_BWD_CHECK 1
 #define MGR_BWD_OUTPUTS_KEPT 512
+#define MGR_DEBUG_BWD_HIT_MASKS 2
 
 #define MGR_OVF_PAIRS 1u
 #define MGR_OVF_CUT 2u
@@ -147,6 +148,7 @@
 int mgr_sh_to_half(int N, const float* f_rest, void* out_half, void* stream);
 
 int mgr_raster_layout(int V, int N, int W, int H, int64_t pair_capacity, size_t* out, int n_out);
+size_t mgr_raster_hit_mask_offset(int V, int N, int W, int H, int64_t pair_capacity);
 int mgr_raster_record_bytes(void);
 
 int mgr_raster_set_cut_margin(float frac_entries, int min_entries, float depth_range_frac, float depth_rel, int interior_only);
diff --git a/manus_amd/_lib.py b/manus_amd/_lib.py
--- a/manus_amd/_lib.py
+++ b/manus_amd/_lib.py
@@ -19,6 +19,8 @@
 MGR_FWD_SKIP_BOX_LARGE, MGR_FWD_SKIP_BOX_MID, MGR_FWD_SKIP_SORT_BEHIND, MGR_FWD_RANK_LARGE = 16, 32, 128, 256
 MGR_FWD_IMAGE_KEPT, MGR_FWD_REPAIR, MGR_FWD_SPREAD = 1024, 2048, 4096
 MGR_BWD_CHECK, MGR_BWD_OUTPUTS_KEPT = 1, 512
+MGR_DEBUG_BWD_HIT_MASKS = 2
+bwd_debug_bits = 0
 MGR_OVF_PAIRS, MGR_OVF_CUT, MGR_OVF_TIER, MGR_OVF_FLAGS_MASK, MGR_OVF_REPAIRED_SHIFT = 1, 2, 4, 0xFFFF, 16
 MGR_TIERS_BOX_LARGE, MGR_TIERS_BOX_MID, MGR_TIERS_WIDE_RECT = 1, 2, 4
 MGR_TIERS_NEAR_SMALL_SHIFT, MGR_TIERS_NEAR_LARGE_SHIFT, MGR_TIERS_NEAR_MASK = 8, 16, 0xFF
@@ -62,6 +64,7 @@
     "mgr_views_maps_backward_pose": (c_int, [c_int] * 6 + [c_vp] * 11 + [c_int] + [c_vp] * 5 + [c_vp, c_sz, c_i64, c_vp, c_sz, c_int] +
                                      [c_int, c_vp, c_vp, c_sz, c_vp]),
     "mgr_raster_record_bytes": (c_int, []),
+    "mgr_raster_hit_mask_offset": (c_sz, [c_int, c_int, c_int, c_int, c_i64]),
     "mgr_raster_layout": (c_int, [c_int, c_int, c_int, c_int, c_i64, ctypes.POINTER(c_sz), c_int]),
     "mgr_raster_status_sync": (c_int, [c_vp, ctypes.POINTER(c_i64), ctypes.POINTER(ctypes.c_int32), c_vp]),
     "mgr_raster_set_status_mirror": (c_int, [c_vp, c_vp]),
diff --git a/manus_amd/csrc/instance_math.h b/manus_amd/csrc/instance_math.h
--- a/manus_amd/csrc/instance_math.h
+++ b/manus_amd/csrc/instance_math.h
@@ -403,6 +403,21 @@
     }
 }
 
+__device__ __forceinline__ void gather_pair_hits(uint32_t off, unsigned long long hit, const float4* __restrict__ pair_grad,
+                                                 float acc[9]) {
+#pragma unroll
+    for (int k = 0; k < 9; ++k) acc[k] = 0.f;
+    while (hit) {
+        const int j = __builtin_ctzll(hit);
+        hit &= hit - 1;
+        const float4* r = pair_grad + (size_t)(off + (uint32_t)j) * 3;
+        const float4 a = r[0], b = r[1], c = r[2];
+        acc[0] += a.x; acc[1] += a.y; acc[2] += a.z; acc[3] += a.w;
+        acc[4] += b.x; acc[5] += b.y; acc[6] += b.z; acc[7] += b.w;
+        acc[8] += c.x;
+    }
+}
+
 #define MGR_POSE_REC 13
 #define MGR_POSE_MAX_WG 1024
 
diff --git a/manus_amd/csrc/mgr_common.h b/manus_amd/csrc/mgr_common.h
--- a/manus_amd/csrc/mgr_common.h
+++ b/manus_amd/csrc/mgr_common.h
@@ -136,12 +136,13 @@
     float b;
     int32_t slot_base;
     int32_t rect_w;
-    int32_t pad;
+    uint32_t off_big;
 #if MGR_GREC_BYTES == 64
     int32_t pad64[4];
 #endif
 };
 
+#define MGR_GREC_BIG 0x80000000u
 #define MGR_CHUNK 64
 
 static inline uint32_t mgr_rep_units(int64_t cap) { int64_t u = cap / 16384; return (uint32_t)(u < 64 ? 64 : (u > 1024 ? 1024 : u)); }
@@ -151,7 +152,7 @@
 struct MgrLayout {
     size_t header, scan_part, scan_cls, scan_box, grec, depth, rect, alive, pair_off, tile_count, tile_start, tile_cursor, tile_done, tile_qdone,
         tile_zcut, tile_zused, tile_qend, tile_bgok, tile_queue, tile_qrec, chunk_start, items, ckpt, keys, keys2, groups, sorted_gid, final_T, n_contrib, pair_tag, pair_grad, inst_grad, inst_tag,
-        db_count, db_cursor, db_start, db_nvis, db_bbox, db_keys, db_order, db_rec, bin_mat, tile_rep, rep_unit, rep_state, rep_last, rep_cnt, rep_cand, rep_view, tile_zwin, db_zrange, db_item, total;
+        db_count, db_cursor, db_start, db_nvis, db_bbox, db_keys, db_order, db_rec, bin_mat, tile_rep, rep_unit, rep_state, rep_last, rep_cnt, rep_cand, rep_view, tile_zwin, db_zrange, db_item, hit_mask, total;
 };
 
 #ifndef MGR_DB_BUCKETS
@@ -233,6 +234,7 @@
     L.tile_zwin = o; o += mgr_align(VT * 4);
     L.db_zrange = o; o += mgr_align((size_t)V * (((size_t)(N > 0 ? N : 1) + 511) / 512) * 2 * 4);
     L.db_item = o;   o += mgr_align((size_t)V * (((size_t)(N > 0 ? N : 1) + MGR_DB_ITEM - 1) / MGR_DB_ITEM + 1) * 2 * 4);
+    L.hit_mask = o;  o += mgr_align(VN * 8);
     L.total = o;
     return L;
 }
diff --git a/manus_amd/csrc/raster_bwd.hip b/manus_amd/csrc/raster_bwd.hip
--- a/manus_amd/csrc/raster_bwd.hip
+++ b/manus_amd/csrc/raster_bwd.hip
@@ -1,4 +1,6 @@
 #include <atomic>
+#include <mutex>
+#include <unordered_set>
 
 #include "instance_math.h"
 
@@ -59,12 +61,13 @@
 #define BWD_WAVES 4
 #endif
 
+template <bool TAGS>
 __global__ __launch_bounds__(256) __attribute__((amdgpu_waves_per_eu(BWD_WAVES, BWD_WAVES))) void k_blend_bwd(
     int N, int W, int H, int gx, int gy, const uint32_t* __restrict__ sorted_gid, const MgrGRec* __restrict__ grec,
     const uint32_t* __restrict__ n_contrib, const float4* __restrict__ ckpt, const uint4* __restrict__ items,
     MgrHeader* hdr, const float* __restrict__ out_color, const float* __restrict__ dL_dpix,
-    uint32_t* __restrict__ pair_tag, float4* __restrict__ pair_grad, uint32_t* __restrict__ inst_tag, uint32_t cap,
-    uint32_t epoch) {
+    uint32_t* __restrict__ pair_tag, float4* __restrict__ pair_grad, uint32_t* __restrict__ inst_tag, unsigned long long* __restrict__ hit_mask,
+    uint32_t cap, uint32_t epoch) {
     __shared__ __align__(16) float s_pair[4][32][MGR_PAIR_FLOATS];
     __shared__ __align__(16) float s_xch[4][4 * BWD_ROW];
     __shared__ float s_acc[4][BWD_BATCH][9];
@@ -387,8 +390,16 @@
             o[0] = make_float4(mx, my, -0.5f * r[2], -0.5f * r[3]);
             o[1] = make_float4(-0.5f * r[4], r[5], r[6], r[7]);
             o[2] = make_float4(r[8], 0.f, 0.f, 0.f);
-            pair_tag[slot] = epoch;
-            inst_tag[(size_t)v * N + gid] = epoch;
+            if (TAGS) {
+                pair_tag[slot] = epoch;
+                inst_tag[(size_t)v * N + gid] = epoch;
+            } else {
+                const uint32_t ob = __float_as_uint(rcz.w);
+                unsigned long long bit = 1ull;
+                if (ob & MGR_GREC_BIG) pair_tag[slot] = epoch;
+                else bit = 1ull << (((uint32_t)slot - ob) & 63u);
+                (void)__hip_atomic_fetch_or(hit_mask + (size_t)v * N + gid, bit, __ATOMIC_RELAXED, __HIP_MEMORY_SCOPE_AGENT);
+            }
 #endif
         }
         __builtin_amdgcn_wave_barrier();
@@ -404,6 +415,7 @@
 #endif
 }
 
+template <bool TAGS>
 __global__ __launch_bounds__(256) void k_preprocess_bwd(
     int N, int W, int H, const float* __restrict__ cams, const float* __restrict__ means3D,
     int64_t s_means, const float* __restrict__ cov3D, int64_t s_cov,
@@ -411,19 +423,34 @@
     const uint32_t* __restrict__ pair_off, const uint32_t* __restrict__ pair_tag,
     const float4* __restrict__ pair_grad, float* __restrict__ dL_dmeans3D,
     float* __restrict__ dL_dmeans2D, float* __restrict__ dL_dcolors,
-    float* __restrict__ dL_dopacity, float* __restrict__ dL_dcov3D, const uint32_t* __restrict__ inst_tag,
-    uint32_t cap, uint32_t epoch, MgrHeader* hdr) {
+    float* __restrict__ dL_dopacity, float* __restrict__ dL_dcov3D, uint32_t* inst_tag,
+    unsigned long long* hit_mask, uint32_t cap, uint32_t epoch, MgrHeader* hdr) {
     if (blockIdx.x == 0 && blockIdx.y == 0 && threadIdx.x < MGR_NCTR) hdr->qctr[threadIdx.x * 64] = 0u;
     const int v = blockIdx.y;
     const int i = blockIdx.x * 256 + threadIdx.x;
     if (i >= N) return;
     const size_t vi = (size_t)v * N + i;
-    const ushort4 rc = rect[vi];
-    const uint32_t cnt = (uint32_t)((rc.z - rc.x) * (rc.w - rc.y));
     float acc[9] = {0.f, 0.f, 0.f, 0.f, 0.f, 0.f, 0.f, 0.f, 0.f};
     float dm[3] = {0.f, 0.f, 0.f}, dc6[6] = {0.f, 0.f, 0.f, 0.f, 0.f, 0.f};
-    if (cnt > 0 && inst_tag[vi] == epoch) {
-        gather_pair_grads(pair_off[vi], cnt, pair_tag, pair_grad, cap, epoch, acc);
+    unsigned long long hw = 0ull;
+    uint32_t cnt = 0u;
+    bool act;
+    if (TAGS) {
+        const ushort4 rc = rect[vi];
+        cnt = (uint32_t)((rc.z - rc.x) * (rc.w - rc.y));
+        act = cnt > 0 && inst_tag[vi] == epoch;
+    } else {
+        hw = hit_mask[vi];
+        act = hw != 0ull;
+        if (act) { hit_mask[vi] = 0ull; inst_tag[vi] = epoch; }
+        if (hw == 1ull) {
+            const ushort4 rc = rect[vi];
+            cnt = (uint32_t)((rc.z - rc.x) * (rc.w - rc.y));
+        }
+    }
+    if (act) {
+        if (TAGS || cnt > 64u) gather_pair_grads(pair_off[vi], cnt, pair_tag, pair_grad, cap, epoch, acc);
+        else gather_pair_hits(pair_off[vi], hw, pair_grad, acc);
         MgrCam cam;
         mgr_load_cam(cams, v, cam);
         const float* mp = means3D + (size_t)v * s_means + (size_t)i * 3;
@@ -508,11 +535,11 @@
 #endif
 #define IB_TSTRIDE(B) ((B) * 16 + 4)
 
-template <int G>
+template <int G, bool TAGS>
 __global__ __launch_bounds__(256) void k_inst_gather(
     int v_first, int v_count, int N, int B, int n_art, const int32_t* __restrict__ radii, const ushort4* __restrict__ rect,
     const uint32_t* __restrict__ pair_off, const uint32_t* __restrict__ pair_tag,
-    const float4* __restrict__ pair_grad, const uint32_t* __restrict__ inst_tag, uint32_t cap, uint32_t epoch,
+    const float4* __restrict__ pair_grad, uint32_t* inst_tag, unsigned long long* hit_mask, uint32_t cap, uint32_t epoch,
     int accumulate, int rounds, float4* __restrict__ iacc,
     uint32_t* __restrict__ active_list, MgrHeader* hdr, float* __restrict__ d_xyz, float* __restrict__ d_ls,
     float* __restrict__ d_rot, float* __restrict__ d_op, float* __restrict__ d_fdc, float* __restrict__ d_frest,
@@ -542,7 +569,7 @@
         for (int k = 0; k < 9; ++k) acc[k] = 0.f;
         int rad = 0;
         bool any = false;
-        {
+        if (TAGS) {
             const size_t vi = (size_t)min(v, v_first + v_count - 1) * N + i;
             const int rd = radii[vi];
             const uint32_t tg = inst_tag[vi];
@@ -551,6 +578,26 @@
             rad = mine ? rd : 0;
             if (rad > 0 && tg == epoch) {
                 gather_pair_grads(po, (uint32_t)((rc.z - rc.x) * (rc.w - rc.y)), pair_tag, pair_grad, cap, epoch, acc);
+#pragma unroll
+                for (int k = 0; k < 9; ++k) any = any || (acc[k] != 0.f);
+            }
+        } else {
+            const size_t vi = (size_t)min(v, v_first + v_count - 1) * N + i;
+            const int rd = radii[vi];
+            const unsigned long long hr = hit_mask[vi];
+            const uint32_t po = pair_off[vi];
+            rad = mine ? rd : 0;
+            const unsigned long long hw = mine ? hr : 0ull;
+            if (hw != 0ull) hit_mask[vi] = 0ull;
+            if (rad > 0 && hw != 0ull) {
+                inst_tag[vi] = epoch;
+                uint32_t tiles = 0u;
+                if (hw == 1ull) {
+                    const ushort4 rc = rect[vi];
+                    tiles = (uint32_t)((rc.z - rc.x) * (rc.w - rc.y));
+                }
+                if (tiles > 64u) gather_pair_grads(po, tiles, pair_tag, pair_grad, cap, epoch, acc);
+                else gather_pair_hits(po, hw, pair_grad, acc);
 #pragma unroll
                 for (int k = 0; k < 9; ++k) any = any || (acc[k] != 0.f);
             }
@@ -622,20 +669,24 @@
     }
 }
 
-template <int G>
+template <int G, bool TAGS>
 __global__ __launch_bounds__(256) void k_inst_gather_runs(
     int v_first, int v_count, int N, int B, int n_art, const int32_t* __restrict__ radii, const ushort4* __restrict__ rect,
     const uint32_t* __restrict__ pair_off, const uint32_t* __restrict__ pair_tag,
-    const float4* __restrict__ pair_grad, const uint32_t* __restrict__ inst_tag, uint32_t cap, uint32_t epoch,
+    const float4* __restrict__ pair_grad, uint32_t* inst_tag, unsigned long long* hit_mask, uint32_t cap, uint32_t epoch,
     int accumulate, int rounds, float4* __restrict__ iacc,
     uint32_t* __restrict__ active_list, MgrHeader* hdr, float* __restrict__ d_xyz, float* __restrict__ d_ls,
     float* __restrict__ d_rot, float* __restrict__ d_op, float* __restrict__ d_fdc, float* __restrict__ d_frest,
     float* __restrict__ d_w, float* __restrict__ st_grad2d, float* __restrict__ st_vis,
     int32_t* __restrict__ st_radii, uint32_t* __restrict__ run_list, unsigned char* __restrict__ row_state, int kept) {
     constexpr int IPB = 256 / G, NG = 256;
-    __shared__ uint32_t s_wi[NG * G], s_wo[NG * G], s_wc[NG * G];
+    __shared__ unsigned short s_wi[NG * G];
+    __shared__ uint32_t s_w32[3][NG * G];
+    uint32_t* const s_wo = s_w32[0]; uint32_t* const s_wl = s_w32[1]; uint32_t* const s_wh = s_w32[2];
     __shared__ uint32_t s_mask[NG];
-    __shared__ uint32_t s_list[NG], s_rl[3][NG];
+    uint32_t* const s_list = &s_w32[0][0];
+    static_assert(G == 1 || 3 * G >= 4, "the active list and the three run lists (4 NG words) must fit the work list's 3 NG G words");
+    uint32_t (*const s_rl)[NG] = (uint32_t (*)[NG])(&s_w32[0][0] + (G >= 2 ? NG : 0));
     __shared__ uint32_t s_nw, s_cnt, s_base, s_rc[3], s_rb[3];
     const int tid = threadIdx.x, vl = tid & (G - 1), il = tid / G, lane = tid & 63;
     if (blockIdx.x == 0 && tid < MGR_NCTR && v_first == 0) hdr->qctr[tid * 64] = 0u;
@@ -651,6 +702,7 @@
     int rd_r[G];
     uint32_t tg_r[G], po_r[G];
     ushort4 rc_r[G];
+    unsigned long long hm_r[G];
 #ifndef MGR_GATHER_PRELOAD
 #define MGR_GATHER_PRELOAD 1
 #endif
@@ -660,8 +712,8 @@
         const int i = min(i_base + min(rnd, rounds - 1) * IPB + il, N - 1);
         const size_t vi = (size_t)min(v_first + vl, v_first + v_count - 1) * N + i;
         rd_r[rnd] = radii[vi];
-        tg_r[rnd] = inst_tag[vi];
-        rc_r[rnd] = rect[vi];
+        if (TAGS) { tg_r[rnd] = inst_tag[vi]; rc_r[rnd] = rect[vi]; }
+        else hm_r[rnd] = hit_mask[vi];
         po_r[rnd] = pair_off[vi];
     }
 #pragma unroll
@@ -673,21 +725,36 @@
         const int i_raw = i_base + rnd * IPB + il;
         const int i = min(i_raw, N - 1);
         const bool ok = i_raw < N, mine = ok && vl < v_count;
+        const size_t vi = (size_t)min(v_first + vl, v_first + v_count - 1) * N + i;
 #if MGR_GATHER_PRELOAD
         const int rd = rd_r[rnd];
-        const uint32_t tg = tg_r[rnd];
-        const ushort4 rc = rc_r[rnd];
+        const uint32_t tg = TAGS ? tg_r[rnd] : 0u;
+        ushort4 rc = TAGS ? rc_r[rnd] : make_ushort4(0, 0, 0, 0);
+        const unsigned long long hr = TAGS ? 0ull : hm_r[rnd];
         const uint32_t po = po_r[rnd];
 #else
-        const size_t vi = (size_t)min(v_first + vl, v_first + v_count - 1) * N + i;
         const int rd = radii[vi];
-        const uint32_t tg = inst_tag[vi];
-        const ushort4 rc = rect[vi];
+        const uint32_t tg = TAGS ? inst_tag[vi] : 0u;
+        ushort4 rc = TAGS ? rect[vi] : make_ushort4(0, 0, 0, 0);
+        const unsigned long long hr = TAGS ? 0ull : hit_mask[vi];
         const uint32_t po = pair_off[vi];
-        (void)rd_r; (void)tg_r; (void)rc_r; (void)po_r;
+        (void)rd_r; (void)tg_r; (void)rc_r; (void)po_r; (void)hm_r;
 #endif
         const int rad = mine ? rd : 0;
-        const bool act = rad > 0 && tg == epoch;
+        const unsigned long long hw = mine ? hr : 0ull;
+        bool act, walk_tags = TAGS;
+        if (TAGS) act = rad > 0 && tg == epoch;
+        else {
+            act = rad > 0 && hw != 0ull;
+            if (hw != 0ull) hit_mask[vi] = 0ull;
+            if (act) {
+                inst_tag[vi] = epoch;
+                if (hw == 1ull) {
+                    rc = rect[vi];
+                    walk_tags = (uint32_t)((rc.z - rc.x) * (rc.w - rc.y)) > 64u;
+                }
+            }
+        }
         const float vis = grp_sum<G>(rad > 0 ? 1.0f : 0.0f);
         int maxrad = rad;
         if (G >= 2) maxrad = max(maxrad, __builtin_amdgcn_update_dpp(0, maxrad, 0xb1, 0xf, 0xf, false));
@@ -701,9 +768,10 @@
             base = (uint32_t)__shfl((int)base, first, 64);
             if (act) {
                 const uint32_t pos = base + (uint32_t)__popcll(m & ((1ull << lane) - 1ull));
-                s_wi[pos] = ((uint32_t)(rnd * IPB + il) << 3) | (uint32_t)vl;
+                s_wi[pos] = (unsigned short)(((uint32_t)(rnd * IPB + il) << 3) | (uint32_t)vl | (walk_tags ? 0x8000u : 0u));
                 s_wo[pos] = po;
-                s_wc[pos] = (uint32_t)((rc.z - rc.x) * (rc.w - rc.y));
+                s_wl[pos] = walk_tags ? (uint32_t)((rc.z - rc.x) * (rc.w - rc.y)) : (uint32_t)hw;
+                s_wh[pos] = (uint32_t)(hw >> 32);
             }
         }
         if (ok && vl == 0) {
@@ -714,9 +782,10 @@
     __syncthreads();
     const uint32_t n_work = s_nw;
     for (uint32_t k = (uint32_t)tid; k < n_work; k += 256u) {
-        const uint32_t w = s_wi[k];
+        const uint32_t wf = s_wi[k], w = wf & 0x7FFFu;
         float acc[9];
-        gather_pair_grads(s_wo[k], s_wc[k], pair_tag, pair_grad, cap, epoch, acc);
+        if (TAGS || (wf & 0x8000u)) gather_pair_grads(s_wo[k], s_wl[k], pair_tag, pair_grad, cap, epoch, acc);
+        else gather_pair_hits(s_wo[k], ((unsigned long long)s_wh[k] << 32) | s_wl[k], pair_grad, acc);
         bool any = false;
 #pragma unroll
         for (int q = 0; q < 9; ++q) any = any || (acc[q] != 0.f);
@@ -1076,6 +1145,15 @@
     return pose_part_bytes(N, B, Gv) + (size_t)N * Gv;
 }
 
+static bool hit_masks_pending(const void* workspace, bool set) {
+    static std::mutex mu;
+    static std::unordered_set<const void*> pending;
+    std::lock_guard<std::mutex> lock(mu);
+    if (set) return !pending.insert(workspace).second;
+    pending.erase(workspace);
+    return false;
+}
+
 static int raster_backward_impl(int V, int N, int W, int H, const float* cams, const float* bg,
                                    const float* means3D, int64_t s_means, const float* cov3D,
                                    int64_t s_cov, const float* colors, int64_t s_col,
@@ -1101,11 +1179,18 @@
     uint32_t epoch = g_epoch.fetch_add(1) + 1;
     if (epoch == 0) epoch = g_epoch.fetch_add(1) + 1;
 
-    { MGR_PROF("k_blend_bwd", stream); hipLaunchKernelGGL(k_blend_bwd, dim3(256 * BWD_WAVES), dim3(256), 0, stream, N, W, H, gx, gy,
-                       (const uint32_t*)(ws + L.sorted_gid), (const MgrGRec*)(ws + L.grec), (const uint32_t*)(ws + L.n_contrib),
-                       (const float4*)(ws + L.ckpt), (const uint4*)(ws + L.items), hdr, out_color,
-                       dL_dcolor, (uint32_t*)(ws + L.pair_tag), (float4*)(ws + L.pair_grad),
-                       (uint32_t*)(ws + L.inst_tag), (uint32_t)cap, epoch); }
+    const bool tags = (flags & MGR_DEBUG_BWD_HIT_MASKS) == 0;
+    unsigned long long* const hit_mask = (unsigned long long*)(ws + L.hit_mask);
+    if (!tags && hit_masks_pending(workspace, true))
+        MGR_HIP(hipMemsetAsync(hit_mask, 0, (size_t)V * N * 8, stream));
+#define MGR_BB_LAUNCH(TG)                                                                                             \
+    hipLaunchKernelGGL(k_blend_bwd<TG>, dim3(256 * BWD_WAVES), dim3(256), 0, stream, N, W, H, gx, gy,                  \
+                       (const uint32_t*)(ws + L.sorted_gid), (const MgrGRec*)(ws + L.grec), (const uint32_t*)(ws + L.n_contrib), \
+                       (const float4*)(ws + L.ckpt), (const uint4*)(ws + L.items), hdr, out_color,                    \
+                       dL_dcolor, (uint32_t*)(ws + L.pair_tag), (float4*)(ws + L.pair_grad),                          \
+                       (uint32_t*)(ws + L.inst_tag), hit_mask, (uint32_t)cap, epoch)
+    { MGR_PROF("k_blend_bwd", stream); if (tags) MGR_BB_LAUNCH(true); else MGR_BB_LAUNCH(false); }
+#undef MGR_BB_LAUNCH
     MGR_LAUNCH_CHECK("k_blend_bwd", stream, flags & MGR_BWD_CHECK);
     if (canon) {
         const int Gv = V <= 1 ? 1 : V <= 2 ? 2 : V <= 4 ? 4 : 8;
@@ -1131,11 +1216,12 @@
             uint32_t* rlist = alist + (size_t)N;
             unsigned char* row_state = V <= Gv ? (unsigned char*)(rlist + 3 * (size_t)N) : nullptr;
             const int kept = (flags & MGR_BWD_OUTPUTS_KEPT) && V <= Gv ? 1 : 0;
-#define MGR_IG_LAUNCH(GG)                                                                                             \
-    hipLaunchKernelGGL((k_inst_gather<GG>), grid_g, dim3(256), 0, stream, v0, vc, N, canon->B, canon->n_art, canon->radii, \
+#define MGR_IG_LAUNCH(GG) if (tags) MGR_IG_LAUNCH2(GG, true); else MGR_IG_LAUNCH2(GG, false)
+#define MGR_IG_LAUNCH2(GG, TG)                                                                                        \
+    hipLaunchKernelGGL((k_inst_gather<GG, TG>), grid_g, dim3(256), 0, stream, v0, vc, N, canon->B, canon->n_art, canon->radii, \
                        (const ushort4*)(ws + L.rect), (const uint32_t*)(ws + L.pair_off),                             \
                        (const uint32_t*)(ws + L.pair_tag), (const float4*)(ws + L.pair_grad),                        \
-                       (const uint32_t*)(ws + L.inst_tag), (uint32_t)cap, epoch, accm, rounds, iacc, alist, hdr, canon->d_xyz, canon->d_ls, canon->d_rot, canon->d_op, canon->d_fdc,    \
+                       (uint32_t*)(ws + L.inst_tag), hit_mask, (uint32_t)cap, epoch, accm, rounds, iacc, alist, hdr, canon->d_xyz, canon->d_ls, canon->d_rot, canon->d_op, canon->d_fdc,    \
                        canon->d_frest, canon->d_w, canon->st_grad2d, canon->st_vis, canon->st_radii, runs && GG == 8 ? rlist : (uint32_t*)nullptr)
 #define MGR_IB_LAUNCH(GG, BB)                                                                                         \
     if (mixed && canon->sh_half) MGR_IB_LAUNCH2(GG, BB, true, true);                                                  \
@@ -1150,24 +1236,28 @@
                        canon->d_frest, canon->d_w, canon->st_grad2d)
             {
                 MGR_PROF("k_inst_gather", stream);
-#define MGR_IGR_LAUNCH(GG)                                                                                            \
-    hipLaunchKernelGGL((k_inst_gather_runs<GG>), grid_gr, dim3(256), 0, stream, v0, vc, N, canon->B, canon->n_art, canon->radii, \
+#define MGR_IGR_LAUNCH(GG) if (tags) MGR_IGR_LAUNCH2(GG, true); else MGR_IGR_LAUNCH2(GG, false)
+#define MGR_IGR_LAUNCH2(GG, TG)                                                                                       \
+    hipLaunchKernelGGL((k_inst_gather_runs<GG, TG>), grid_gr, dim3(256), 0, stream, v0, vc, N, canon->B, canon->n_art, canon->radii, \
                        (const ushort4*)(ws + L.rect), (const uint32_t*)(ws + L.pair_off),                             \
                        (const uint32_t*)(ws + L.pair_tag), (const float4*)(ws + L.pair_grad),                        \
-                       (const uint32_t*)(ws + L.inst_tag), (uint32_t)cap, epoch, accm, rounds_r, iacc, alist, hdr, canon->d_xyz, canon->d_ls, canon->d_rot, canon->d_op, canon->d_fdc, \
+                       (uint32_t*)(ws + L.inst_tag), hit_mask, (uint32_t)cap, epoch, accm, rounds_r, iacc, alist, hdr, canon->d_xyz, canon->d_ls, canon->d_rot, canon->d_op, canon->d_fdc, \
                        canon->d_frest, canon->d_w, canon->st_grad2d, canon->st_vis, canon->st_radii, rlist, row_state, kept)
                 const bool old_gather = g_inst_runs.load(std::memory_order_relaxed) == 2 && Gv == 8;
                 if (runs && !old_gather) {
-                    if (Gv == 8) MGR_IGR_LAUNCH(8);
-                    else if (Gv == 4) MGR_IGR_LAUNCH(4);
-                    else if (Gv == 2) MGR_IGR_LAUNCH(2);
-                    else MGR_IGR_LAUNCH(1);
+                    if (Gv == 8) { MGR_IGR_LAUNCH(8); }
+                    else if (Gv == 4) { MGR_IGR_LAUNCH(4); }
+                    else if (Gv == 2) { MGR_IGR_LAUNCH(2); }
+                    else { MGR_IGR_LAUNCH(1); }
                 }
 #undef MGR_IGR_LAUNCH
-                else if (Gv == 8) MGR_IG_LAUNCH(8);
-                else if (Gv == 4) MGR_IG_LAUNCH(4);
-                else if (Gv == 2) MGR_IG_LAUNCH(2);
-                else MGR_IG_LAUNCH(1);
+#undef MGR_IGR_LAUNCH2
+                else if (Gv == 8) { MGR_IG_LAUNCH(8); }
+                else if (Gv == 4) { MGR_IG_LAUNCH(4); }
+                else if (Gv == 2) { MGR_IG_LAUNCH(2); }
+                else { MGR_IG_LAUNCH(1); }
+                MGR_LAUNCH_CHECK("k_inst_gather", stream, 0);
+                if (!tags && v0 + Gv >= V) hit_masks_pending(workspace, false);
             }
             MgrProfScope prof_ib(canon->d_T ? "k_inst_bwd_pose" : "k_inst_bwd", stream);
 #define MGR_IBR_LAUNCH(MX, HF)                                                                                        \
@@ -1238,14 +1328,22 @@
 #undef MGR_IB_LAUNCH
 #undef MGR_IB_LAUNCH2
 #undef MGR_IG_LAUNCH
-        }
-    } else
-    { MGR_PROF("k_preprocess_bwd", stream); hipLaunchKernelGGL(k_preprocess_bwd, dim3((N + 255) / 256, V), dim3(256), 0, stream, N, W, H, cams,
-                       means3D, s_means, cov3D, s_cov, (const int32_t*)nullptr,
-                       (const ushort4*)(ws + L.rect), (const uint32_t*)(ws + L.pair_off),
-                       (const uint32_t*)(ws + L.pair_tag), (const float4*)(ws + L.pair_grad),
-                       dL_dmeans3D, dL_dmeans2D, dL_dcolors, dL_dopacity, dL_dcov3D,
-                       (const uint32_t*)(ws + L.inst_tag), (uint32_t)cap, epoch, hdr); }
+#undef MGR_IG_LAUNCH2
+        }
+    } else {
+#define MGR_PB_LAUNCH(TG)                                                                                             \
+    hipLaunchKernelGGL(k_preprocess_bwd<TG>, dim3((N + 255) / 256, V), dim3(256), 0, stream, N, W, H, cams,            \
+                       means3D, s_means, cov3D, s_cov, (const int32_t*)nullptr,                                       \
+                       (const ushort4*)(ws + L.rect), (const uint32_t*)(ws + L.pair_off),                             \
+                       (const uint32_t*)(ws + L.pair_tag), (const float4*)(ws + L.pair_grad),                         \
+                       dL_dmeans3D, dL_dmeans2D, dL_dcolors, dL_dopacity, dL_dcov3D,                                  \
+                       (uint32_t*)(ws + L.inst_tag), hit_mask, (uint32_t)cap, epoch, hdr)
+        MGR_PROF("k_preprocess_bwd", stream);
+        if (tags) MGR_PB_LAUNCH(true); else MGR_PB_LAUNCH(false);
+#undef MGR_PB_LAUNCH
+        MGR_LAUNCH_CHECK("k_preprocess_bwd", stream, 0);
+        if (!tags) hit_masks_pending(workspace, false);
+    }
     MGR_LAUNCH_CHECK("k_preprocess_bwd", stream, flags & MGR_BWD_CHECK);
     return MGR_OK;
 }
diff --git a/manus_amd/csrc/raster_fwd.hip b/manus_amd/csrc/raster_fwd.hip
--- a/manus_amd/csrc/raster_fwd.hip
+++ b/manus_amd/csrc/raster_fwd.hip
@@ -235,7 +235,7 @@
         r.r = col[0]; r.g = col[1]; r.b = col[2];
         r.rect_w = x1 - x0;
         r.slot_base = (int32_t)off - y0 * (x1 - x0) - x0;
-        r.pad = 0;
+        r.off_big = (off & ~MGR_GREC_BIG) | (tiles > 64u ? MGR_GREC_BIG : 0u);
         grec[vi] = r;
         depth[vi] = po.zv;
         rect[vi] = make_ushort4((unsigned short)x0, (unsigned short)y0, (unsigned short)x1, (unsigned short)y1);
@@ -2724,8 +2724,10 @@
     const bool repair = use_cut && (flags & MGR_FWD_REPAIR) && W < 65536 && H < 65536 &&
                         (int64_t)((W + 15) / 16) * ((H + 15) / 16) <= (int64_t)MGR_REP_MAX_TILES;
     const int debug = flags & MGR_FWD_CHECK;
-    if (V <= 0 || N < 0 || W <= 0 || H <= 0 || cap < 0 || cap > 0xFFFFFFF0ll)
+    if (V <= 0 || N < 0 || W <= 0 || H <= 0 || cap < 0)
         return mgr_fail(MGR_EINVAL, "mgr_raster_forward: bad sizes");
+    if (cap >= 0x80000000ll)
+        return mgr_fail(MGR_EINVAL, "mgr_raster_forward: pair capacities of 2^31 or more are not supported");
     if (!cams || !bg || !out_color || !workspace ||
         (N > 0 && !canon && (!means3D || !cov3D || !colors || !opacity)) || (N > 0 && !radii))
         return mgr_fail(MGR_EINVAL, "mgr_raster_forward: null pointer");
@@ -2988,6 +2990,7 @@
     return 0;
 }
 #endif
+extern "C" size_t mgr_raster_hit_mask_offset(int V, int N, int W, int H, int64_t cap) { return mgr_layout(V, N, W, H, cap).hit_mask; }
 extern "C" int mgr_raster_layout(int V, int N, int W, int H, int64_t cap, size_t* out, int n_out) {
     const MgrLayout L = mgr_layout(V, N, W, H, cap);
     const size_t v[] = {L.header, L.grec, L.depth, L.rect, L.alive, L.pair_off, L.tile_count, L.tile_start,
diff --git a/manus_amd/engine.py b/manus_amd/engine.py
--- a/manus_amd/engine.py
+++ b/manus_amd/engine.py
@@ -865,7 +865,7 @@
         bits = _lib.MGR_BWD_OUTPUTS_KEPT if (kept is not None and kept.grad_ws is ws and V <= 8 and not full_rows) else 0
         self._kept.grad_ws = None
         args = (*head, ptr(radii), ptr(out), ptr(g_img), 1.0 / scale, *[ptr(g) for g in grads.values()],
-                ptr(d_w), ptr(st_g), ptr(st_v), ptr(st_r), ptr(ws.buf), ws.nbytes, ws.cap, bits)
+                ptr(d_w), ptr(st_g), ptr(st_v), ptr(st_r), ptr(ws.buf), ws.nbytes, ws.cap, bits | _lib.bwd_debug_bits)
         d_T = None
         if self.pose_grad:
             d_T = torch.empty((V, B, 4, 4), dtype=torch.float32, device=dev)
diff --git a/manus_amd/fused.py b/manus_amd/fused.py
--- a/manus_amd/fused.py
+++ b/manus_amd/fused.py
@@ -72,7 +72,7 @@
                                        ptr(opacity), ptr(f_dc), ptr(f_rest), ptr(skin_w), ptr(transforms),
                                        ptr(radii), ptr(out), ptr(g_img), g2s, ptr(d_xyz), ptr(d_ls), ptr(d_rot),
                                        ptr(d_op), ptr(d_fdc), ptr(d_frest), ptr(d_w), ptr(st_g), ptr(st_v),
-                                       ptr(st_r), ptr(ws.buf), ws.nbytes, ws.cap, 0, stream()),
+                                       ptr(st_r), ptr(ws.buf), ws.nbytes, ws.cap, _rz._lib.bwd_debug_bits, stream()),
               "mgr_views_backward")
         if stats is not None:
             stats.grad2d, stats.vis, stats.radii = st_g, st_v, st_r
diff --git a/manus_amd/rasterizer.py b/manus_amd/rasterizer.py
--- a/manus_amd/rasterizer.py
+++ b/manus_amd/rasterizer.py
@@ -37,6 +37,8 @@
     def __init__(self, device, V, N, W, H, cap):
         self.key = (V, N, W, H)
         self.cap = int(cap)
+        if self.cap >= 1 << 31:
+            raise _lib.ManusHipError("pair capacity %d: 2^31 pairs or more are not supported" % self.cap)
         self.nbytes = int(lib().mgr_raster_workspace_bytes(V, N, W, H, self.cap))
         self.buf = torch.zeros(self.nbytes, dtype=torch.uint8, device=device)
         self.busy = False
@@ -362,7 +364,7 @@
         check(lib().mgr_raster_backward(V, N, W, H, ptr(cams), ptr(bg), ptr(means3D), s_m, ptr(cov3D), s_c,
                                         ptr(colors), s_col, ptr(opac), s_o, ptr(out), ptr(g_color), ptr(d_m3), ptr(d_m2),
                                         ptr(d_col), ptr(d_op), ptr(d_cov), ptr(ws.buf), ws.nbytes, ws.cap,
-                                        _lib.MGR_BWD_CHECK if debug else 0, stream()), "mgr_raster_backward")
+                                        (_lib.MGR_BWD_CHECK if debug else 0) | _lib.bwd_debug_bits, stream()), "mgr_raster_backward")
 
         def fold(g, shared, shape=None):
             if shared:
```

New measurement: 781.8 (median of 3 runs). No clear change (-0.0%).
